# Stylish-TTS/stylish-tts

Measured on AMD Instinct MI355X. Metric: audio frames/sec/GPU (24 kHz) forward+backward; DDP scaling 1/2/4/8 MI355X, higher is better.
Workload: dtype bf16 GEMM operands, f32 accumulation/storage; 1 GPU; c3: B=32/GPU T=520 frames (6.5 s) L=100

## Files before the change

### include/stylish_hip.h

```cpp
#ifndef STYLISH_HIP_H
#define STYLISH_HIP_H

#include <stddef.h>
#include <stdint.h>

#ifdef __cplusplus
extern "C" {
#endif

typedef enum {
  STY_OK = 0,
  STY_EINVAL = -1,
  STY_ESHAPE = -2,
  STY_EHIP = -3,
  STY_ENOMEM = -4,
  STY_ESTATE = -5
} sty_status;

typedef struct sty_model sty_model;

int sty_version(void);
const char *sty_last_error(void);

int sty_model_create(const char *kind, sty_model **out);
// ... 30 lines not shown
  float *audio;
  float *tap_text_encoding;
  float *tap_decoder_out;
  sty_vocoder_io voc_taps;
  void *style_stream;
} sty_speech_io;
int sty_speech_workspace_bytes(const sty_model *m, int B, int L, int T, size_t *bytes);
int sty_speech_fwd(sty_model *m, const sty_speech_io *io, void *workspace, size_t ws_bytes, void *stream);

int sty_style_workspace_bytes(const sty_model *m, int B, int T, size_t *bytes);
int sty_style_fwd(sty_model *m, int B, int T, const float *mel, float *style, void *workspace, size_t ws_bytes,
                  void *stream);

int sty_mel_workspace_bytes(int B, int N, int n_fft, int hop, size_t *bytes);
int sty_mel_fwd(int B, int N, const float *audio, int n_fft, int win_length, int hop, float mean, float std,
                float *mel, float *energy, void *workspace, size_t ws_bytes, void *stream);

int sty_multispec_workspace_bytes(int B, int N, size_t *bytes);
int sty_multispec_fwd(int B, int N, const float *audio, float *const *mag, float *const *phase,
                      float *const *fft_mag, void *workspace, size_t ws_bytes, void *stream);

int sty_alignment_fwd(int B, int L, int T, const float *durations, float *alignment, void *stream);

int sty_duration_workspace_bytes(const sty_model *m, int B, int L, size_t *bytes);
int sty_duration_fwd(sty_model *m, int B, int L, const int64_t *texts, const int64_t *text_lengths, const float *style,
                     float *dur_pred, void *workspace, size_t ws_bytes, void *stream);
int sty_pitch_energy_workspace_bytes(const sty_model *m, int B, int L, int T, size_t *bytes);
int sty_pitch_energy_fwd(sty_model *m, int B, int L, int T, const int64_t *texts, const int64_t *text_lengths,
                         const float *alignment, const float *style, float *pitch, float *energy, void *workspace,
                         size_t ws_bytes, void *stream);

int sty_pitch_style_workspace_bytes(const sty_model *m, int B, int T, size_t *bytes);
int sty_pitch_style_fwd(sty_model *m, int B, int T, const float *mel, const float *pitch, const float *energy,
                        float *style, void *workspace, size_t ws_bytes, void *stream);

int sty_aligner_workspace_bytes(const sty_model *m, int B, int T, size_t *bytes);
int sty_aligner_fwd(sty_model *m, int B, int T, const float *mel, const int64_t *mel_lengths, float *log_probs,
                    void *workspace, size_t ws_bytes, void *stream);
int sty_forced_align_workspace_bytes(int B, int T, int U, size_t *bytes);
int sty_forced_align(int B, int T, int V1, int U, const float *log_probs, const int64_t *targets,
                     const int64_t *input_lengths, const int64_t *target_lengths, int blank, int32_t *labels,
                     float *scores, int32_t *status, void *workspace, size_t ws_bytes, void *stream);

void sty_rmvpe_resample_kernel_host(float *out);
void sty_rmvpe_mel_basis_host(float *out);
int sty_rmvpe_mel_workspace_bytes(int B, int N, size_t *bytes);
int sty_rmvpe_mel_fwd(int B, int N, const float *audio, float *logmel, void *workspace, size_t ws_bytes, void *stream);
int sty_rmvpe_workspace_bytes(const sty_model *m, int B, int n, size_t *bytes);
int sty_rmvpe_fwd(sty_model *m, int B, int n, const float *logmel, float *salience, void *workspace, size_t ws_bytes,
                  void *stream);
int sty_rmvpe_decode(int B, int n, const float *salience, float thred, float *f0, void *stream);

int sty_aligner_train_workspace_bytes(sty_model *m, int B, int T, size_t *bytes);
int sty_aligner_fwd_train(sty_model *m, int B, int T, const float *mel, const int64_t *mel_lengths, float drop_p,
                          unsigned drop_seed, float *log_probs, void *workspace, size_t ws_bytes, void *stream);
int sty_aligner_bwd(sty_model *m, const float *d_logits, void *stream);
int sty_ctc_loss_workspace_bytes(int B, int T, int V1, int U, size_t *bytes);
int sty_ctc_loss_fwd_bwd(int B, int T, int V1, int U, const float *log_probs, const float *log_priors, float prior_scale,
                         const int64_t *targets, const int64_t *input_lengths, const int64_t *target_lengths, int blank,
                         float weight, double *nll, float *loss, int32_t *status, float *d_logits, void *workspace,
                         size_t ws_bytes, void *stream);

int sty_convnext_fwd(sty_model *m, const char *prefix, int B, int C, int T, const float *x, const float *style,
                     float *y, void *workspace, size_t ws_bytes, void *stream);
int sty_resblock_fwd(sty_model *m, const char *prefix, int B, int T, const float *x, const float *style, float *y,
                     void *workspace, size_t ws_bytes, void *stream);
int sty_block_train_workspace_bytes(sty_model *m, const char *kind, const char *prefix, int B, int C, int T,
                                    size_t *bytes);
int sty_block_fwd_bwd(sty_model *m, const char *kind, const char *prefix, int B, int C, int T, const float *x,
                      const float *style, const float *gy, float *y, float *gx, float *d_style, void *workspace,
                      size_t ws_bytes, void *stream);
int sty_attention_workspace_bytes(int B, int H, int T, size_t *bytes);
int sty_attention_fwd_bwd(int B, int H, int DH, int T, const float *q, const float *k, const float *v,
                          const int64_t *lengths, const float *d_o, float *o, float *dq, float *dk, float *dv,
                          void *workspace, size_t ws_bytes, void *stream);
int sty_stft64_fwd(int B, int N, const float *wave, float *spec, float *phase, void *stream);
void sty_stft64_bases_host(float *out);
int sty_istft64_fwd(int B, int F, const float *logamp, const float *real, const float *imag, float *audio,
                    void *stream);
int sty_source_fwd(int B, int T, const float *pitch, const float *voiced, const float *noise, uint64_t seed,
                   const float *lin_w, const float *lin_b, float *prior, void *workspace, size_t ws_bytes,
                   void *stream);
int sty_source_workspace_bytes(int B, int T, size_t *bytes);
int sty_grn_bwd_workspace_bytes(int B, int C4, int T, size_t *bytes);
int sty_grn_bwd(int B, int C4, int T, const float *h, const float *ds, const float *gamma, int from_gx, float *coef,
                float *dgamma, void *workspace, size_t ws_bytes, void *stream);
int sty_act_bwd(int kind, int B, int C, int T, const float *x, float *dy, const float *alpha, const float *h,
                const float *coef, int fused, float *dx, int accumulate, float *dalpha, void *stream);
int sty_adain_finalize(int B, int C, int T, int nseg, const double *part, const float *gb, float eps, float *a, float *s,
                       float *mean, float *rstd, void *stream);

int sty_model_enable_training(sty_model *m);
typedef struct {
  int bn_batch_stats;
  int sn_power_iter;
  int f0_smooth;
  int energy_smooth;
  float bn_momentum;
  unsigned dropout_seed;
  float text_dropout;
  int compute_bf16;
  int frozen;
  float block_dropout;
} sty_train_opts;
int sty_model_set_train_opts(sty_model *m, const sty_train_opts *opts);

typedef void (*sty_grad_hook)(void *user, int segment);
int sty_model_set_grad_hook(sty_model *m, sty_grad_hook hook, void *user);
int sty_model_bind_grad(sty_model *m, const char *key, float *grad);
int sty_vocoder_train_workspace_bytes(sty_model *m, int B, int T, size_t *bytes);
int sty_vocoder_fwd_train(sty_model *m, const sty_vocoder_io *io, void *workspace, size_t ws_bytes, void *stream);
int sty_vocoder_bwd(sty_model *m, const float *d_audio, float *d_mel, float *d_style, void *stream);
int sty_speech_train_workspace_bytes(sty_model *m, int B, int L, int T, size_t *bytes);
int sty_speech_fwd_train(sty_model *m, const sty_speech_io *io, void *workspace, size_t ws_bytes, void *stream);
int sty_speech_bwd(sty_model *m, const float *d_audio, float *d_style, float *d_energy, void *stream);
int sty_speech_prepare_train(sty_model *m, void *stream);
int sty_speech_bwd_pe(sty_model *m, const float *d_audio, float *d_style, float *d_pitch, float *d_energy, void *stream);
int sty_speech_d_style_ready(sty_model *m, void *stream);
int sty_speech_branch_stream(sty_model *m, void **stream);
int sty_style_train_workspace_bytes(sty_model *m, int B, int T, size_t *bytes);
int sty_style_fwd_train(sty_model *m, int B, int T, const float *mel, float *style, void *workspace, size_t ws_bytes,
                        void *stream);
int sty_style_bwd(sty_model *m, const float *d_style, void *stream);
int sty_style_prepare_train(sty_model *m, void *stream);
int sty_style_tap(sty_model *m, int index, int grad, float *dst, int *C, int *H, int *W, void *stream);
int sty_pitch_loss_fwd_bwd(int B, int T, const float *target, const float *pred, float weight, int normalize,
                           float *loss, float *d_pred, void *workspace, size_t ws_bytes, void *stream);
int sty_prediction_to_duration(int B, int L, int NC, const float *pred, const int64_t *text_lengths,
                               const float *class_table, float *duration, void *stream);
int sty_duration_loss_fwd_bwd(int B, int L, int NC, const float *pred, const int64_t *text_lengths,
                              const float *target_dur, const int64_t *target_class, const float *class_table,
                              const float *ce_weight, float w_duration, float w_ce, const float *d_duration_extra,
                              float *losses, float *d_pred, void *workspace, size_t ws_bytes, void *stream);
int sty_duration_train_workspace_bytes(sty_model *m, int B, int L, size_t *bytes);
int sty_duration_fwd_train(sty_model *m, int B, int L, const int64_t *texts, const int64_t *text_lengths,
                           const float *style, float *out, void *workspace, size_t ws_bytes, void *stream);
int sty_duration_bwd(sty_model *m, const float *d_out, float *d_style, void *stream);
int sty_pitch_energy_train_workspace_bytes(sty_model *m, int B, int L, int T, size_t *bytes);
int sty_pitch_energy_fwd_train(sty_model *m, int B, int L, int T, const int64_t *texts, const int64_t *text_lengths,
                               const float *alignment, const float *style, float *pitch, float *energy, void *workspace,
                               size_t ws_bytes, void *stream);
int sty_pitch_energy_bwd(sty_model *m, const float *d_pitch, const float *d_energy, float *d_style, void *stream);
int sty_pitch_style_train_workspace_bytes(sty_model *m, int B, int T, size_t *bytes);
int sty_pitch_style_fwd_train(sty_model *m, int B, int T, const float *mel, const float *pitch, const float *energy,
                              float *style, void *workspace, size_t ws_bytes, void *stream);

int sty_conv1d_workspace_bytes(int Cout, int Cin, int K, size_t *bytes);
int sty_conv1d_fwd(int B, int Cin, int Cout, int K, int dil, int T, const float *x, const float *w, const float *bias,
                   float *y, void *workspace, size_t ws_bytes, int compute_bf16, void *stream);
int sty_conv1d_fwd_ex(int B, int Cin, int Cout, int K, int dil, int T, const float *x, const float *w, const float *bias,
                      const float *in_mask, const float *residual, const float *out_mask, int out_mask_post, int relu,
                      float *y, void *workspace, size_t ws_bytes, int compute_bf16, void *stream);
enum { STY_ROUTE_IN_MASK = 1, STY_ROUTE_RESIDUAL = 2, STY_ROUTE_OUT_MASK = 4, STY_ROUTE_RELU = 8, STY_ROUTE_TWO_BYTE_X = 16,
       STY_ROUTE_STATS = 32, STY_ROUTE_Y16 = 64, STY_ROUTE_X16 = 128 };
enum { STY_CONV_STEM2D = 0, STY_CONV_32P, STY_CONV_SC, STY_CONV_K1, STY_CONV_Q, STY_CONV_P16, STY_CONV_TILED };
int sty_conv1d_route(int B, int Cin, int Cout, int K, int dil, int T, int compute_bf16, int flags, int *kernel);
int sty_conv1d_bwd_workspace_bytes(int B, int Cin, int Cout, int K, int T, size_t *bytes);
int sty_conv1d_bwd(int B, int Cin, int Cout, int K, int dil, int T, const float *x, const float *w, const float *gy,
                   float *dw, float *dbias, float *dx, void *workspace, size_t ws_bytes, int compute_bf16,
                   void *stream);
int sty_partial_sum(int dw_form, const float *part, int C, int K, int nblk, float *dw, float *db, void *stream);

int sty_adamw_step(size_t n, float *p, const float *g, float *m, float *v, float lr, float beta1, float beta2,
                   float eps, float weight_decay, int step, float grad_scale, void *stream);
int sty_adamw_step_scaled(size_t n, float *p, const float *g, float *m, float *v, double lr, const double *lr_mult,
                          float beta1, float beta2, float eps, float weight_decay, int step, float grad_scale,
                          void *stream);
int sty_disc_lr_track(double *state, const float *loss, double ideal_loss, double f_max, double h_min, double x_max,
                      double x_min, void *stream);

int sty_acoustic_loss_workspace_bytes(int B, int N, size_t *bytes);
int sty_acoustic_loss_target(int B, int N, const float *audio_gt, void *workspace, size_t ws_bytes, void *stream);
int sty_acoustic_loss_fwd_bwd(int B, int N, const float *audio_gt, const float *audio_pred, float w_mel,
                              float w_phase, float *losses, float *d_audio_pred, void *workspace, size_t ws_bytes,
                              void *stream);

typedef struct {
  const float *g[10];
  const float *v[10];
  const float *bias[10];
} sty_specdisc_params;
typedef struct {
  float *g[10];
  float *v[10];
  float *bias[10];
} sty_specdisc_grads;
int sty_specdisc_workspace_bytes(int B, int H, int W, int with_grads, size_t *bytes);
int sty_specdisc_forward(const sty_specdisc_params *p, int B, int H, int W, const float *x, float *scores,
                         int compute_bf16, void *workspace, size_t ws_bytes, void *stream);
int sty_specdisc_losses(const sty_specdisc_params *p, int B, int H, int W, const float *target, const float *pred,
                        float gen_scale, float *gen_loss, float *d_pred, float disc_scale, float *disc_loss,
                        const sty_specdisc_grads *grads, int compute_bf16, void *workspace, size_t ws_bytes,
                        void *stream);

int sty_pitchdisc_workspace_bytes(int B, int dim_in, int kernel, int T, int with_grads, size_t *bytes);
int sty_pitchdisc_forward(const sty_specdisc_params *p, int B, int dim_in, int kernel, int T, const float *x,
                          float *scores, void *workspace, size_t ws_bytes, void *stream);
int sty_pitchdisc_losses(const sty_specdisc_params *p, int B, int dim_in, int kernel, int T, const float *target,
                         const float *pred, float gen_scale, float *gen_loss, float *d_pred, float disc_scale,
                         float *disc_loss, const sty_specdisc_grads *grads, void *workspace, size_t ws_bytes,
                         void *stream);

typedef struct {
  const float *conv_w[12];
  const float *conv_b[12];
  const float *bn_w[9];
  const float *bn_b[9];
  float *bn_rm[9];
  float *bn_rv[9];
} sty_cfdisc_params;
typedef struct {
  float *conv_w[12];
  float *conv_b[12];
  float *bn_w[9];
  float *bn_b[9];
} sty_cfdisc_grads;
int sty_cfdisc_workspace_bytes(int B, int N, int with_grads, size_t *bytes);
int sty_cfdisc_forward(const sty_cfdisc_params *p, int B, int N, const float *x, float *scores, float bn_momentum,
                       int compute_bf16, void *workspace, size_t ws_bytes, void *stream);
int sty_cfdisc_losses(const sty_cfdisc_params *p, int B, int N, const float *target, const float *pred, float gen_scale,
                      float *gen_loss, float *d_pred, float disc_scale, float *disc_loss, const sty_cfdisc_grads *grads,
                      float bn_momentum, int compute_bf16, void *workspace, size_t ws_bytes, void *stream);

int sty_acoustic_gan_workspace_bytes(int B, int N, int with_grads, size_t *bytes);
int sty_acoustic_gan_loss_fwd_bwd(int B, int N, const float *audio_gt, const float *audio_pred, float w_mel,
                                  float w_phase, float w_gen, const sty_specdisc_params *mrd, float disc_scale,
                                  const sty_specdisc_grads *mrd_grads, int step_mask, float *losses, float *gan_losses,
                                  float *d_audio_pred, void *workspace, size_t ws_bytes, void *gan_workspace,
                                  size_t gan_ws_bytes, int compute_bf16, void *stream);

typedef struct sty_comm sty_comm;
int sty_comm_unique_id(void *id128);
int sty_comm_init(const void *id128, int rank, int world, int stream_priority, sty_comm **out);
int sty_comm_allreduce_bucket(sty_comm *c, float *buf, size_t n, void *producer_stream);
int sty_comm_wait(sty_comm *c, void *consumer_stream);
int sty_comm_set_stream(sty_comm *c, void *stream);
int sty_comm_stats(sty_comm *c, uint64_t *buckets, uint64_t *reduce_scatter_all_gather, double *bytes);
int sty_comm_destroy(sty_comm *c);

int sty_pack_accumulate(int n, int D, int rows, const float *styles, const int64_t *text_lengths, double *sums,
                        int64_t *counts, void *stream);
int sty_pack_finalize(int rows, int D, const double *sums, const int64_t *counts, const int32_t *lo, const int32_t *hi,
                      float *pack, void *stream);

typedef struct {
  char name[48];
  char inst[144];
  uint64_t launches;
  double ms;
  double flops;
  double bytes;
} sty_prof_row;
int sty_prof_enable(int on);
int sty_prof_only(const char *family);
int sty_set_single_stream(int on);
int sty_prof_report(sty_prof_row *rows, int cap);

#ifdef __cplusplus
}
#endif
#endif
```

### stylish_tts_amd/csrc/api.hip

```cpp
#include <math.h>
#include <stdarg.h>
#include <string.h>
#include <stdlib.h>
#include <cxxabi.h>

#include <map>
#include <string>

#include "model.h"

namespace sty {

static thread_local char g_err[1024] = "";
void set_error(const char* fmt, ...) {
  va_list ap;
  va_start(ap, fmt);
  vsnprintf(g_err, sizeof(g_err), fmt, ap);
  va_end(ap);
}
int hip_fail(hipError_t e, const char* what) {
  set_error("HIP error %d (%s) at %s", (int)e, hipGetErrorString(e), what);
  return STY_EHIP;
}

// ... 2666 lines not shown
}
int sty_style_tap(sty_model* m, int index, int grad, float* dst, int* C, int* H, int* W, void* stream) {
  int rc = model_ready(m, "mel_style_encoder", "pitch_style_encoder");
  if (rc) return rc;
  if (!m->trainer) {
    set_error("sty_style_tap: no recorded forward");
    return STY_ESTATE;
  }
  return trainer_style_tap(m->trainer, index, grad, dst, C, H, W, S(stream));
}
int sty_conv1d_workspace_bytes(int Cout, int Cin, int K, size_t* bytes) {
  if (!bytes || Cout <= 0 || Cin <= 0 || K <= 0) {
    set_error("sty_conv1d_workspace_bytes: bad argument");
    return STY_EINVAL;
  }
  *bytes = ((size_t)K * align_up(Cin, CI_CHUNK) * align_up(Cout, 128) + align_up(Cout, 128)) * sizeof(float) + 512;
  return STY_OK;
}
int sty_conv1d_fwd(int B, int Cin, int Cout, int K, int dil, int T, const float* x, const float* w, const float* bias,
                   float* y, void* workspace, size_t ws_bytes, int compute_bf16, void* stream) {
  size_t need = 0;
  int rc = sty_conv1d_workspace_bytes(Cout, Cin, K, &need);
  if (rc) return rc;
  if (!x || !w || !y || !workspace || B <= 0 || T <= 0 || dil <= 0 || (K - 1) * dil > 128 || ws_bytes < need) {
    set_error("sty_conv1d_fwd: bad argument, halo > 128 or workspace too small");
    return STY_EINVAL;
  }
  PackedConv pc;
  pc.Cin = Cin;
  pc.Cout = Cout;
  pc.K = K;
  pc.CinP = (int)align_up(Cin, CI_CHUNK);
  pc.CoutP = (int)align_up(Cout, 32);
  float* wp = reinterpret_cast<float*>(align_up(reinterpret_cast<size_t>(workspace), 256));
  float* bp = wp + (size_t)K * pc.CinP * pc.CoutP;
  STY_HIP(hipMemsetAsync(wp, 0, ((size_t)K * pc.CinP * pc.CoutP + pc.CoutP) * sizeof(float), S(stream)));
  rc = launch_pack_conv(w, nullptr, nullptr, bias, Cout, Cin, K, wp, bp, pc.CinP, pc.CoutP, S(stream));
  if (rc) return rc;
  pc.wp = wp;
  pc.bias = bias ? bp : nullptr;
  ConvArgs a;
  a.x[0] = x;
  a.xc[0] = Cin;
  a.nsrc = 1;
  a.B = B;
  a.T = T;
  a.w = pc;
  a.dil = dil;
  a.pad = (K - 1) * dil / 2;
  a.y = y;
  a.bf16 = compute_bf16 != 0;
  if (compute_bf16 == 2) {
    const size_t tw = ((size_t)B * (Cin + Cout) * T) * sizeof(__bf16) + 512;
    if (ws_bytes < need + tw) {
      set_error("sty_conv1d_fwd: compute_bf16 = 2 needs %zu more workspace bytes for the operand twins", tw);
      return STY_EINVAL;
    }
    __bf16* x16 = reinterpret_cast<__bf16*>(align_up(reinterpret_cast<size_t>(static_cast<char*>(workspace) + need), 256));
    if ((rc = launch_twin_cast(x, nullptr, PRO_NONE, B, Cin, T, x16, S(stream)))) return rc;
    a.x16 = x16;
    a.y16 = x16 + (size_t)B * Cin * T;
    a.y16_act = PRO_LRELU;
  }
  return launch_conv1d(a, S(stream));
}
static PackedConv unit_conv_dims(int Cin, int Cout, int K) {
  PackedConv pc;
  pc.Cin = Cin;
  pc.Cout = Cout;
  pc.K = K;
  pc.CinP = (int)align_up(Cin, CI_CHUNK);
  pc.CoutP = (int)align_up(Cout, 32);
  return pc;
}
int sty_conv1d_fwd_ex(int B, int Cin, int Cout, int K, int dil, int T, const float* x, const float* w, const float* bias,
                      const float* in_mask, const float* residual, const float* out_mask, int out_mask_post, int relu, float* y,
                      void* workspace, size_t ws_bytes, int compute_bf16, void* stream) {
  size_t need = 0;
  int rc = sty_conv1d_workspace_bytes(Cout, Cin, K, &need);
  if (rc) return rc;
  if (!x || !w || !y || !workspace || B <= 0 || T <= 0 || dil <= 0 || (K - 1) * dil > 128 || ws_bytes < need ||
      !(compute_bf16 == 0 || compute_bf16 == 1)) {
    set_error("sty_conv1d_fwd_ex: bad argument, halo > 128, a compute mode other than 0 / 1 or workspace too small");
    return STY_EINVAL;
  }
  PackedConv pc;
  pc.Cin = Cin;
  pc.Cout = Cout;
  pc.K = K;
  pc.CinP = (int)align_up(Cin, CI_CHUNK);
  pc.CoutP = (int)align_up(Cout, 32);
  float* wp = reinterpret_cast<float*>(align_up(reinterpret_cast<size_t>(workspace), 256));
  float* bp = wp + (size_t)K * pc.CinP * pc.CoutP;
  STY_HIP(hipMemsetAsync(wp, 0, ((size_t)K * pc.CinP * pc.CoutP + pc.CoutP) * sizeof(float), S(stream)));
  rc = launch_pack_conv(w, nullptr, nullptr, bias, Cout, Cin, K, wp, bp, pc.CinP, pc.CoutP, S(stream));
  if (rc) return rc;
  pc.wp = wp;
  pc.bias = bias ? bp : nullptr;
  ConvArgs a;
  a.x[0] = x;
  a.xc[0] = Cin;
  a.nsrc = 1;
  a.B = B;
  a.T = T;
  a.w = pc;
  a.dil = dil;
  a.pad = (K - 1) * dil / 2;
  a.y = y;
  a.bf16 = compute_bf16;
  if (in_mask) {
    a.pro = PRO_MASK;
    a.mask = in_mask;
  }
  a.act = relu ? ACT_RELU : ACT_NONE;
  a.residual = residual;
  a.out_mask = out_mask;
  a.out_mask_post = out_mask ? out_mask_post : 0;
  return launch_conv1d(a, S(stream));
}
int sty_conv1d_route(int B, int Cin, int Cout, int K, int dil, int T, int compute_bf16, int flags, int* kernel) {
  if (!kernel || B <= 0 || Cin <= 0 || Cout <= 0 || K <= 0 || T <= 0 || dil <= 0) {
    set_error("sty_conv1d_route: bad argument");
    return STY_EINVAL;
  }
  static_assert(STY_CONV_STEM2D == CONV_STEM2D && STY_CONV_32P == CONV_32P && STY_CONV_SC == CONV_SC && STY_CONV_K1 == CONV_K1 &&
                    STY_CONV_Q == CONV_Q && STY_CONV_P16 == CONV_P16 && STY_CONV_TILED == CONV_TILED,
                "stylish_hip.h lists the families in the order of ConvKernel");
  static float dummy_f[4];
  static double dummy_d[4];
  static __bf16 dummy_h[4];
  ConvArgs a;
  a.x[0] = dummy_f;
  a.xc[0] = Cin;
  a.nsrc = 1;
  a.B = B;
  a.T = T;
  a.w = unit_conv_dims(Cin, Cout, K);
  a.w.wp = dummy_f;
  a.dil = dil;
  a.pad = (K - 1) * dil / 2;
  a.y = dummy_f;
  a.bf16 = compute_bf16 != 0;
  if (flags & STY_ROUTE_IN_MASK) {
    a.pro = PRO_MASK;
    a.mask = dummy_f;
  }
  if (flags & STY_ROUTE_RESIDUAL) a.residual = dummy_f;
  if (flags & STY_ROUTE_OUT_MASK) a.out_mask = dummy_f;
  if (flags & STY_ROUTE_RELU) a.act = ACT_RELU;
  if (flags & STY_ROUTE_TWO_BYTE_X) a.xh = 1;
  if (flags & STY_ROUTE_STATS) a.stat_part = dummy_d;
  if (flags & STY_ROUTE_Y16) a.y16 = dummy_h;
  if (flags & STY_ROUTE_X16) a.x16 = dummy_h;
  const ConvRoute r = conv1d_route(a);
  *kernel = r.refusal == CONV_OK ? (int)r.kernel : -1;
  return STY_OK;
}
int sty_conv1d_bwd_workspace_bytes(int B, int Cin, int Cout, int K, int T, size_t* bytes) {
  if (!bytes || B <= 0 || Cin <= 0 || Cout <= 0 || K <= 0 || T <= 0) {
    set_error("sty_conv1d_bwd_workspace_bytes: bad argument");
    return STY_EINVAL;
  }
  const PackedConv pc = unit_conv_dims(Cin, Cout, K);
  const size_t plane = (size_t)K * pc.CinP * pc.CoutP + pc.CoutP;
  *bytes = (3 * plane + wgrad_partial_floats(pc, B, T)) * sizeof(float) + 1024;
  *bytes += (size_t)B * (Cin + Cout) * T * sizeof(__bf16) + 512;
  return STY_OK;
}
int sty_conv1d_bwd(int B, int Cin, int Cout, int K, int dil, int T, const float* x, const float* w, const float* gy,
                   float* dw, float* dbias, float* dx, void* workspace, size_t ws_bytes, int compute_bf16,
                   void* stream) {
  size_t need = 0;
  int rc = sty_conv1d_bwd_workspace_bytes(B, Cin, Cout, K, T, &need);
  if (rc) return rc;
  if (!x || !w || !gy || !dw || !workspace || dil <= 0 || (K - 1) * dil > 128 || ws_bytes < need) {
    set_error("sty_conv1d_bwd: bad argument, halo > 128 or workspace too small");
    return STY_EINVAL;
  }
  hipStream_t st = S(stream);
  PackedConv pc = unit_conv_dims(Cin, Cout, K);
  const size_t plane = (size_t)K * pc.CinP * pc.CoutP;
  float* wp = reinterpret_cast<float*>(align_up(reinterpret_cast<size_t>(workspace), 256));
  float* bp = wp + plane;
  float* gwp = bp + pc.CoutP;
  float* gbp = gwp + plane;
  PackedConv pd;
  pd.Cin = Cout;
  pd.Cout = Cin;
  pd.K = K;
  pd.CinP = pc.CoutP;
  pd.CoutP = pc.CinP;
  float* wd = gbp + pc.CoutP;
  float* partial = wd + plane + pc.CoutP;
  STY_HIP(hipMemsetAsync(wp, 0, (size_t)(partial - wp) * sizeof(float), st));
  rc = launch_pack_conv(w, nullptr, nullptr, nullptr, Cout, Cin, K, wp, bp, pc.CinP, pc.CoutP, st);
  if (rc) return rc;
  pc.wp = wp;
  pc.bias = dbias ? bp : nullptr;
  ConvArgs a;
  a.x[0] = x;
  a.xc[0] = Cin;
  a.nsrc = 1;
  a.B = B;
  a.T = T;
  a.w = pc;
  a.dil = dil;
  a.pad = (K - 1) * dil / 2;
  a.bf16 = compute_bf16 != 0;
  if (compute_bf16 == 3) {
    if (dx || T % 2) {
      set_error("sty_conv1d_bwd: a two-byte x (compute_bf16 = 3) is for dw / dbias only (dx == NULL), T even");
      return STY_EINVAL;
    }
    a.xh = 1;
  }
  if (compute_bf16 == 2) {
    __bf16* x16 = reinterpret_cast<__bf16*>(align_up(reinterpret_cast<size_t>(partial + wgrad_partial_floats(pc, B, T)), 256));
    __bf16* g16 = x16 + (size_t)B * Cin * T;
    if ((rc = launch_twin_cast(x, nullptr, PRO_NONE, B, Cin, T, x16, st))) return rc;
    if ((rc = launch_twin_cast(gy, nullptr, PRO_NONE, B, Cout, T, g16, st))) return rc;
    a.x16 = x16;
    a.g16 = g16;
  }
  bool bias_done = false;
  rc = launch_conv1d_wgrad(a, gy, nullptr, 1.0f, gwp, partial, dbias ? gbp : nullptr, &bias_done, st);
  if (rc) return rc;
  if (dbias && !bias_done) {
    set_error("sty_conv1d_bwd: this conv's bias gradient is a separate pass (launch_bias_grad), not wired here");
    return STY_EINVAL;
  }
  STY_HIP(hipMemsetAsync(dw, 0, (size_t)Cout * Cin * K * sizeof(float), st));
  rc = launch_unpack_grad(gwp, nullptr, nullptr, Cout, Cin, K, pc.CinP, pc.CoutP, dw, nullptr, nullptr, st);
  if (rc) return rc;
  if (dbias) STY_HIP(hipMemcpyAsync(dbias, gbp, (size_t)Cout * sizeof(float), hipMemcpyDeviceToDevice, st));
  if (dx) {
    PackedConv pdm = pd;
    rc = launch_pack_dgrad(wp, K, pc.CinP, pc.CoutP, wd, st);
    if (rc) return rc;
    pdm.wp = wd;
    pdm.bias = nullptr;
    ConvArgs d;
    d.x[0] = gy;
    d.xc[0] = Cout;
    d.nsrc = 1;
    d.B = B;
    d.T = T;
    d.w = pdm;
    d.dil = dil;
    d.pad = (K - 1) * dil - a.pad;
    d.bf16 = a.bf16;
    d.y = dx;
    d.x16 = a.g16;
    rc = launch_conv1d(d, st);
  }
  return rc;
}
int sty_partial_sum(int dw_form, const float* part, int C, int K, int nblk, float* dw, float* db, void* stream) {
  if (!part || !db || C <= 0 || nblk <= 0 || (dw_form && (!dw || K <= 0))) {
    set_error("sty_partial_sum: bad argument");
    return STY_EINVAL;
  }
  return launch_partial_sum(dw_form, part, C, K, nblk, dw, db, S(stream));
}
static size_t grn_bwd_ws_bytes(int B, int C4, int T) {
  return (size_t)B * C4 * row_stats_nseg(T) * 2 * sizeof(double) + (size_t)2 * B * C4 * sizeof(float);
}
int sty_grn_bwd_workspace_bytes(int B, int C4, int T, size_t* bytes) {
  if (!bytes || B <= 0 || C4 <= 0 || T <= 0) {
    set_error("sty_grn_bwd_workspace_bytes: bad argument");
    return STY_EINVAL;
  }
  *bytes = grn_bwd_ws_bytes(B, C4, T);
  return STY_OK;
}
int sty_grn_bwd(int B, int C4, int T, const float* h, const float* ds, const float* gamma, int from_gx, float* coef,
                float* dgamma, void* workspace, size_t ws_bytes, void* stream) {
  if (!h || !ds || !gamma || !coef || !dgamma || !workspace || B <= 0 || C4 <= 0 || T <= 0) {
    set_error("sty_grn_bwd: bad argument");
    return STY_EINVAL;
  }
  if (ws_bytes < grn_bwd_ws_bytes(B, C4, T)) {
    set_error("sty_grn_bwd: workspace too small");
    return STY_ENOMEM;
  }
  hipStream_t st = S(stream);
  const int nseg = row_stats_nseg(T);
  double* part = (double*)workspace;
  float* scale = (float*)(part + (size_t)B * C4 * nseg * 2);
  float* gx = scale + (size_t)B * C4;
  int rc = launch_row_stats(h, B * C4, T, part, st);
  if (rc) return rc;
  if ((rc = launch_grn_finalize(part, nseg, gamma, B, C4, scale, st, gx))) return rc;
  return launch_grn_bwd(from_gx ? gx : nullptr, part, nseg, gamma, ds, B, C4, coef, dgamma, st);
}
int sty_act_bwd(int kind, int B, int C, int T, const float* x, float* dy, const float* alpha, const float* h,
                const float* coef, int fused, float* dx, int accumulate, float* dalpha, void* stream) {
  if (!x || !dy || !dx || B <= 0 || C <= 0 || T <= 0 || (kind == ACT_SNAKE && !alpha) || ((h != nullptr) != (coef != nullptr))) {
    set_error("sty_act_bwd: bad argument");
    return STY_EINVAL;
  }
  hipStream_t st = S(stream);
  if (h && !fused) {
    const int rc = launch_row_scale_add(h, coef, 0.f, B * C, T, dy, st);
    if (rc) return rc;
    h = coef = nullptr;
  }
  return launch_act_bwd(kind, x, dy, alpha, B, C, T, dx, accumulate, dalpha, st, h, coef);
}
int sty_adain_finalize(int B, int C, int T, int nseg, const double* part, const float* gb, float eps, float* a, float* s,
// ... 145 lines not shown
```

### stylish_tts_amd/csrc/bwd.hip

```cpp
#include "sty_common.h"

namespace sty {

__device__ __forceinline__ double wave_sum(double v) {
  for (int o = 32; o > 0; o >>= 1) v += __shfl_xor(v, o);
  return v;
}

template <int N>
__device__ __forceinline__ void block_sum(double (&v)[N], double (*red)[4]) {
  const int lane = threadIdx.x & 63, wave = threadIdx.x >> 6;
#pragma unroll
  for (int i = 0; i < N; ++i) {
    v[i] = wave_sum(v[i]);
    if (lane == 0) red[i][wave] = v[i];
  }
  __syncthreads();
  if (threadIdx.x == 0) {
#pragma unroll
    for (int i = 0; i < N; ++i) v[i] = red[i][0] + red[i][1] + red[i][2] + red[i][3];
  }
}

__global__ __launch_bounds__(256) void pro_bwd_kernel(int mode_, const float* __restrict__ u, int Cu, int cu0,
// ... 592 lines not shown
  STY_LAUNCH_CHECK();
  return STY_OK;
}
bool chan_ln32_eligible(int B, int C, int T, int relu) {
  return C == 32 && !relu && (size_t)B * T >= 65536 && getenv("STY_NO_LN32_BWD") == nullptr;
}
int launch_chan_ln_bwd(const float* x, const float* dy, const float* y, int B, int C, int T, float eps, int ada,
                       const float* w, const float* gb, int relu, const float* out_mask, float* dx, int accumulate,
                       float* mu_tmp, float* r_tmp, float* dgb, float* dw, float* db, hipStream_t st, int h16) {
  const bool no32 = getenv("STY_NO_LN32_BWD") != nullptr;
  if (C == 32 && !relu && (size_t)B * T >= 65536 && !no32) {
    const int nblk = cdiv(T, 256);
    if ((h16 & 4) && accumulate) {
      set_error("chan_ln_bwd: a two-byte dx cannot be accumulated into");
      return STY_EINVAL;
    }
    hipLaunchKernelGGL(chan_ln32_bwd_kernel, dim3(nblk, B), dim3(256), 0, st, x, dy, T, eps, ada, w, gb, out_mask, dx, accumulate,
                       mu_tmp, h16);
    hipLaunchKernelGGL(chan_ln32_param_sum_kernel, dim3(ada ? B * 64 : 64), dim3(64), 0, st, mu_tmp, B, nblk, ada, dgb, dw, db);
    STY_LAUNCH_CHECK();
    return STY_OK;
  }
  if (h16) {
    set_error("chan_ln_bwd: two-byte tensors only on the C = 32 long-row kernel (chan_ln32_eligible)");
    return STY_EINVAL;
  }
  if ((size_t)B * T < 65536 && C <= 256)
    hipLaunchKernelGGL((chan_ln_bwd_dx_reg_kernel<16, 16>), dim3(cdiv(T, 16), B), dim3(256), 0, st, x, dy, y, C, T, eps, ada, w,
                       gb, relu, out_mask, dx, accumulate, mu_tmp, r_tmp);
  else if ((size_t)B * T >= 65536)
    hipLaunchKernelGGL(chan_ln_bwd_dx_kernel<64>, dim3(cdiv(T, 64), B), dim3(256), 0, st, x, dy, y, C, T, eps, ada, w, gb,
                       relu, out_mask, dx, accumulate, mu_tmp, r_tmp);
  else
    hipLaunchKernelGGL(chan_ln_bwd_dx_kernel<16>, dim3(cdiv(T, 16), B), dim3(256), 0, st, x, dy, y, C, T, eps, ada, w, gb,
                       relu, out_mask, dx, accumulate, mu_tmp, r_tmp);
  hipLaunchKernelGGL(chan_ln_bwd_param_kernel, dim3(C, B), dim3(256), 0, st, x, dy, y, mu_tmp, r_tmp, C, T, ada, relu,
                     out_mask, dgb, dw, db);
  STY_LAUNCH_CHECK();
  return STY_OK;
}

__global__ __launch_bounds__(256) void grn_bwd_kernel(const float* __restrict__ gx, const double* __restrict__ part, int nseg,
                                                      const float* __restrict__ gamma,
                                                      const float* __restrict__ ds, int C4,
                                                      float* __restrict__ coef, float* __restrict__ dgamma) {
  __shared__ float gxs[1024];
  __shared__ double red[2][4];
  const int b = blockIdx.x;
  if (gx) {
    for (int c = threadIdx.x; c < C4; c += 256) gxs[c] = gx[(size_t)b * C4 + c];
  } else if (nseg < 32) {
    for (int c = threadIdx.x; c < C4; c += 256) {
      double sq = 0.0;
      for (int k = 0; k < nseg; ++k) sq += part[(((size_t)b * C4 + c) * nseg + k) * 2 + 1];
      gxs[c] = (float)sqrt(sq);
    }
  } else {
    const int lane = threadIdx.x & 63, wave = threadIdx.x >> 6;
    for (int c = wave; c < C4; c += 4) {
      const double* pp = part + ((size_t)b * C4 + c) * nseg * 2 + 1;
      double sq = 0.0;
      for (int k = lane; k < nseg; k += 64) sq += pp[(size_t)k * 2];
      for (int o = 32; o > 0; o >>= 1) sq += __shfl_xor(sq, o);
      if (lane == 0) gxs[c] = (float)sqrt(sq);
    }
  }
  __syncthreads();
  double acc[1] = {0.0};
  for (int c = threadIdx.x; c < C4; c += 256) acc[0] += gxs[c];
  __shared__ float mean_s, dot_s;
  block_sum<1>(acc, red);
  if (threadIdx.x == 0) mean_s = (float)(acc[0] / C4);
  __syncthreads();
  const float m = mean_s + 1e-6f;
  double d2[1] = {0.0};
  for (int c = threadIdx.x; c < C4; c += 256) {
    const float dnx = ds[(size_t)b * C4 + c] * gamma[c];
    d2[0] += (double)dnx * gxs[c];
    atomicAdd(&dgamma[c], ds[(size_t)b * C4 + c] * (gxs[c] / m));
  }
  __syncthreads();
  block_sum<1>(d2, red);
  if (threadIdx.x == 0) dot_s = (float)d2[0];
  __syncthreads();
  for (int c = threadIdx.x; c < C4; c += 256) {
    const float dnx = ds[(size_t)b * C4 + c] * gamma[c];
    const float dgx = dnx / m - dot_s / (m * m) / (float)C4;
    coef[(size_t)b * C4 + c] = gxs[c] > 0.f ? dgx / gxs[c] : 0.f;
  }
}
int launch_grn_bwd(const float* gx, const double* part, int nseg, const float* gamma, const float* ds, int B, int C4,
                   float* coef, float* dgamma, hipStream_t st) {
  if (C4 > 1024) {
    set_error("grn_bwd: 4C > 1024");
    return STY_EINVAL;
  }
  if (!gx && !part) {
    set_error("grn_bwd: neither the forward's norms nor its partials");
    return STY_EINVAL;
  }
  ProfScope prof("grn_bwd_kernel", 0.0, 4.0 * B * C4 * 4, st, gx ? "gx" : "part");
  hipLaunchKernelGGL(grn_bwd_kernel, dim3(B), dim3(256), 0, st, gx, part, nseg, gamma, ds, C4, coef, dgamma);
  STY_LAUNCH_CHECK();
  return STY_OK;
}

__global__ void act_fwd_kernel(int kind, const float* __restrict__ x, const float* __restrict__ alpha, int C, int T,
                               float* __restrict__ y) {
  const int t = blockIdx.x * 256 + threadIdx.x, c = blockIdx.y, b = blockIdx.z;
  if (t >= T) return;
  if (kind == ACT_GLU) {
    const float a = x[((size_t)b * 2 * C + c) * T + t], g = x[((size_t)b * 2 * C + C + c) * T + t];
    y[((size_t)b * C + c) * T + t] = a / (1.f + expf(-g));
    return;
  }
  const size_t o = ((size_t)b * C + c) * T + t;
  const float v = x[o];
  float r = v;
  if (kind == ACT_RELU) r = fmaxf(v, 0.f);
  else if (kind == ACT_SWISH) r = v / (1.f + expf(-v));
  else if (kind == ACT_SNAKE) r = sty_snake(v, alpha[c], 1.f / alpha[c]);
  else if (kind == 100) r = tanhf(v);
  else if (kind == ACT_GELU) r = 0.5f * v * (1.0f + erff(v * 0.70710678118654752f));
  y[o] = r;
}
__device__ __forceinline__ float act_apply1(int kind, float v, float al, float ral) {
  float r = v;
  if (kind == ACT_RELU) r = fmaxf(v, 0.f);
  else if (kind == ACT_SWISH) r = v / (1.f + expf(-v));
  else if (kind == ACT_SNAKE) r = sty_snake(v, al, ral);
  else if (kind == 100) r = tanhf(v);
  else if (kind == ACT_GELU) r = 0.5f * v * (1.0f + erff(v * 0.70710678118654752f));
  return r;
}
__global__ __launch_bounds__(256) void act_fwd4_kernel(int kind, const float* __restrict__ x, const float* __restrict__ alpha,
                                                       unsigned C, unsigned T4, unsigned n4, float* __restrict__ y) {
  const unsigned idx = blockIdx.x * 256u + threadIdx.x;
  if (idx >= n4) return;
  float al = 1.f, ral = 1.f;
  if (kind == ACT_SNAKE) {
    al = alpha[(idx / T4) % C];
    ral = 1.f / al;
  }
  const float4 v = reinterpret_cast<const float4*>(x)[idx];
  float4 r;
  r.x = act_apply1(kind, v.x, al, ral);
  r.y = act_apply1(kind, v.y, al, ral);
  r.z = act_apply1(kind, v.z, al, ral);
  r.w = act_apply1(kind, v.w, al, ral);
  reinterpret_cast<float4*>(y)[idx] = r;
}
int launch_act_fwd(int kind, const float* x, const float* alpha, int B, int C, int T, float* y, hipStream_t st) {
  const size_t n4 = (size_t)B * C * (T / 4);
  if (kind != ACT_GLU && T % 4 == 0 && n4 < ((size_t)1 << 31) && ((((size_t)x | (size_t)y) & 15) == 0)) {
    hipLaunchKernelGGL(act_fwd4_kernel, dim3((unsigned)((n4 + 255) / 256)), dim3(256), 0, st, kind, x, alpha, (unsigned)C,
                       (unsigned)(T / 4), (unsigned)n4, y);
    STY_LAUNCH_CHECK();
    return STY_OK;
  }
  hipLaunchKernelGGL(act_fwd_kernel, dim3(cdiv(T, 256), C, B), dim3(256), 0, st, kind, x, alpha, C, T, y);
  STY_LAUNCH_CHECK();
  return STY_OK;
}
__global__ __launch_bounds__(256) void act_bwd_kernel(int kind, const float* __restrict__ x,
                                                      const float* __restrict__ dy, const float* __restrict__ alpha,
                                                      int C, int T, float* __restrict__ dx, int accumulate,
                                                      float* __restrict__ dalpha, const float* __restrict__ h,
                                                      const float* __restrict__ coef) {
  __shared__ double red[1][4];
  const int c = blockIdx.x, b = blockIdx.y;
  double acc[1] = {0.0};
  if (kind == ACT_GLU) {
    const size_t ra = ((size_t)b * 2 * C + c) * T, rg = ((size_t)b * 2 * C + C + c) * T, ro = ((size_t)b * C + c) * T;
    for (int t = threadIdx.x; t < T; t += 256) {
      const float a = x[ra + t], g = x[rg + t], d = dy[ro + t];
      const float sg = 1.f / (1.f + expf(-g));
      const float da = d * sg, dg = d * a * sg * (1.f - sg);
      dx[ra + t] = accumulate ? dx[ra + t] + da : da;
      dx[rg + t] = accumulate ? dx[rg + t] + dg : dg;
    }
    return;
  }
  const size_t row = ((size_t)b * C + c) * T;
  const float al = kind == ACT_SNAKE ? alpha[c] : 1.f;
  const float cf = h ? coef[(size_t)b * C + c] : 0.f;
  auto one = [&](float v, float d) -> float {
    float g = d;
    if (kind == ACT_RELU) g = v > 0.f ? d : 0.f;
    else if (kind == ACT_SWISH) {
      const float sg = 1.f / (1.f + expf(-v));
      g = d * (sg + v * sg * (1.f - sg));
    } else if (kind == ACT_SNAKE) {
      float sn, cs;
      sty_sincos(al * v, sn, cs);
      const float s2 = sn * sn, s2a = 2.f * sn * cs;
      g = d * (1.f + s2a);
      acc[0] += (double)(d * (v * s2a - s2 / al) / al);
    } else if (kind == 100) {
      const float th = tanhf(v);
      g = d * (1.f - th * th);
    } else if (kind == ACT_GELU) {
      g = d * (0.5f * (1.0f + erff(v * 0.70710678118654752f)) + v * 0.3989422804014327f * expf(-0.5f * v * v));
    }
    return g;
  };
  if ((T & 3) == 0 && ((((size_t)(x + row) | (size_t)(dy + row) | (size_t)(dx + row) | (size_t)(h ? h + row : nullptr)) & 15) == 0)) {
    const float4* x4 = reinterpret_cast<const float4*>(x + row);
    const float4* d4 = reinterpret_cast<const float4*>(dy + row);
    float4* o4 = reinterpret_cast<float4*>(dx + row);
    const float4* h4 = h ? reinterpret_cast<const float4*>(h + row) : nullptr;
    for (int t = threadIdx.x; t < T / 4; t += 256) {
      const float4 v = x4[t];
      float4 d = d4[t];
      if (h) {
        const float4 hv = h4[t];
        d = make_float4(fmaf(hv.x, cf, d.x), fmaf(hv.y, cf, d.y), fmaf(hv.z, cf, d.z), fmaf(hv.w, cf, d.w));
      }
      float4 g;
      g.x = one(v.x, d.x);
      g.y = one(v.y, d.y);
      g.z = one(v.z, d.z);
      g.w = one(v.w, d.w);
      if (accumulate) {
        const float4 o = o4[t];
        g = make_float4(o.x + g.x, o.y + g.y, o.z + g.z, o.w + g.w);
      }
      o4[t] = g;
    }
  } else
  for (int t = threadIdx.x; t < T; t += 256) {
    const float v = x[row + t];
    float d = dy[row + t];
    if (h) d = fmaf(h[row + t], cf, d);
    float g = d;
    if (kind == ACT_RELU) g = v > 0.f ? d : 0.f;
    else if (kind == ACT_SWISH) {
      const float sg = 1.f / (1.f + expf(-v));
      g = d * (sg + v * sg * (1.f - sg));
    } else if (kind == ACT_SNAKE) {
      float sn, cs;
      sty_sincos(al * v, sn, cs);
      const float s2 = sn * sn, s2a = 2.f * sn * cs;
      g = d * (1.f + s2a);
      acc[0] += (double)(d * (v * s2a - s2 / al) / al);
    } else if (kind == 100) {
      const float th = tanhf(v);
      g = d * (1.f - th * th);
    } else if (kind == ACT_GELU) {
      g = d * (0.5f * (1.0f + erff(v * 0.70710678118654752f)) + v * 0.3989422804014327f * expf(-0.5f * v * v));
    }
    dx[row + t] = accumulate ? dx[row + t] + g : g;
  }
  if (kind == ACT_SNAKE && dalpha) {
    block_sum<1>(acc, red);
    if (threadIdx.x == 0) atomicAdd(&dalpha[c], (float)acc[0]);
  }
}
int launch_act_bwd(int kind, const float* x, const float* dy, const float* alpha, int B, int C, int T, float* dx,
                   int accumulate, float* dalpha, hipStream_t st, const float* h, const float* coef) {
  if (h && (kind == ACT_GLU || !coef)) {
    set_error("act_bwd: a row term needs its coefficients and a one-to-one activation");
    return STY_EINVAL;
  }
  ProfScope prof("act_bwd_kernel", 0.0, 4.0 * B * C * T * (3.0 + (accumulate ? 1 : 0) + (h ? 1 : 0)), st, h ? "row term" : nullptr);
  hipLaunchKernelGGL(act_bwd_kernel, dim3(C, B), dim3(256), 0, st, kind, x, dy, alpha, C, T, dx, accumulate, dalpha, h, coef);
  STY_LAUNCH_CHECK();
  return STY_OK;
}

__global__ void row_scale_add_kernel(const float* __restrict__ src, const float* __restrict__ coef, float k, int T,
                                     float* __restrict__ dst) {
  const int t = blockIdx.x * 256 + threadIdx.x, row = blockIdx.y;
  if (t >= T) return;
  const size_t o = (size_t)row * T + t;
  dst[o] += src[o] * (coef ? coef[row] : k);
}
__global__ __launch_bounds__(256) void row_scale_add4_kernel(const float* __restrict__ src, const float* __restrict__ coef,
                                                             float k, unsigned T4, unsigned n4, float* __restrict__ dst) {
  const unsigned idx = blockIdx.x * 256u + threadIdx.x;
  if (idx >= n4) return;
  const float f = coef ? coef[idx / T4] : k;
  const float4 sv = reinterpret_cast<const float4*>(src)[idx];
  float4 d = reinterpret_cast<float4*>(dst)[idx];
  d.x += sv.x * f;
  d.y += sv.y * f;
  d.z += sv.z * f;
  d.w += sv.w * f;
  reinterpret_cast<float4*>(dst)[idx] = d;
}
int launch_row_scale_add(const float* src, const float* coef, float k, int rows, int T, float* dst, hipStream_t st) {
  ProfScope prof(coef ? "row_scale_add_kernel[coef]" : "row_scale_add_kernel", 0.0, 12.0 * rows * T, st);
  const size_t n4 = (size_t)rows * (T / 4);
  if (vec4_ok(n4, T, src, dst)) {
    hipLaunchKernelGGL(row_scale_add4_kernel, dim3((unsigned)((n4 + 255) / 256)), dim3(256), 0, st, src, coef, k,
                       (unsigned)(T / 4), (unsigned)n4, dst);
    STY_LAUNCH_CHECK();
    return STY_OK;
  }
  hipLaunchKernelGGL(row_scale_add_kernel, dim3(cdiv(T, 256), rows), dim3(256), 0, st, src, coef, k, T, dst);
  STY_LAUNCH_CHECK();
  return STY_OK;
}

__global__ void dwconv_fwd_kernel(const float* __restrict__ x, const float* __restrict__ w,
                                  const float* __restrict__ bias, int C, int T, int K, int pad,
                                  float* __restrict__ y) {
// ... 640 lines not shown
```

### stylish_tts_amd/csrc/conv1d.hip

```cpp
#include <stdlib.h>

#include "sty_common.h"

namespace sty {

__device__ __forceinline__ float sigmoidf_(float v) { return 1.0f / (1.0f + expf(-v)); }

}

#include "conv_stage.h"

namespace sty {

template <int ACT>
__device__ __forceinline__ float act_apply(float x, float alpha) {
  if constexpr (ACT == ACT_RELU) return fmaxf(x, 0.f);
  if constexpr (ACT == ACT_SWISH) return x * sigmoidf_(x);
  if constexpr (ACT == ACT_SNAKE) return sty_snake(x, alpha, 1.0f / alpha);
  if constexpr (ACT == ACT_GELU) return 0.5f * x * (1.0f + erff(x * 0.70710678118654752f));
  return x;
}

constexpr int STY_MINW = 2;
template <int WM, int WN, int MT, int NT, int KS = 1, bool BF = false>
// ... 213 lines not shown
    }
    return;
  }
#define STY_EPI_ACT(ACT)                                                                 \
  _Pragma("clang loop unroll(full)") for (int m = 0; m < MT; ++m)                        \
  _Pragma("clang loop unroll(full)") for (int n = 0; n < NT; ++n)                        \
  _Pragma("unroll") for (int r = 0; r < 16; ++r) {                                       \
    const int co = co0 + m * 32 + (r & 3) + 8 * (r >> 2) + 4 * hi;                       \
    float x = acc[m][n][r] + (a.w.bias ? a.w.bias[co] : 0.f);                            \
    float al = 1.f;                                                                      \
    if constexpr (ACT == ACT_SNAKE) al = a.act_alpha[co < Cout ? co : 0];                \
    acc[m][n][r] = act_apply<ACT>(x, al) * a.out_scale;                                  \
  }
  switch (a.act) {
    case ACT_RELU: { STY_EPI_ACT(ACT_RELU) } break;
    case ACT_SWISH: { STY_EPI_ACT(ACT_SWISH) } break;
    case ACT_SNAKE: { STY_EPI_ACT(ACT_SNAKE) } break;
    case ACT_GELU: { STY_EPI_ACT(ACT_GELU) } break;
    default: { STY_EPI_ACT(ACT_NONE) } break;
  }
#undef STY_EPI_ACT
#pragma clang loop unroll(full)
  for (int m = 0; m < MT; ++m) {
#pragma clang loop unroll(full)
    for (int n = 0; n < NT; ++n) {
      const int t = t0 + tw + n * 32 + l31;
      const bool tin = t < T;
      float v[16];
      const float om_pre = (a.out_mask && !a.out_mask_post && tin) ? a.out_mask[(size_t)b * T + t] : 1.f;
#pragma unroll
      for (int r = 0; r < 16; ++r) {
        const int co = co0 + m * 32 + (r & 3) + 8 * (r >> 2) + 4 * hi;
        float x = acc[m][n][r] * om_pre;
        if (a.residual && co < Cout && tin) x += a.residual[((size_t)b * Cout + co) * T + t];
        v[r] = x;
      }
      if (a.ln_out) {
        float s = 0.f;
#pragma unroll
        for (int r = 0; r < 16; ++r) s += v[r];
        s += __shfl_xor(s, 32);
        const float mean = s * (1.0f / 32.0f);
        float q = 0.f;
#pragma unroll
        for (int r = 0; r < 16; ++r) {
          float d = v[r] - mean;
          q += d * d;
        }
        q += __shfl_xor(q, 32);
        const float rstd = 1.0f / sqrtf(q * (1.0f / 32.0f) + a.ln_eps);
#pragma unroll
        for (int r = 0; r < 16; ++r) {
          const int co = co0 + m * 32 + (r & 3) + 8 * (r >> 2) + 4 * hi;
          v[r] = (v[r] - mean) * rstd * a.ln_w[co] + a.ln_b[co];
        }
      }
      if (tin) {
        const float om = (a.out_mask && a.out_mask_post) ? a.out_mask[(size_t)b * T + t] : 1.f;
        if (a.shuffle == 1) {
#pragma unroll
          for (int r = 0; r < 16; ++r) {
            const int co = co0 + m * 32 + (r & 3) + 8 * (r >> 2) + 4 * hi;
            if (co < Cout) a.y[((size_t)b * Cout + co) * T + t] = v[r] * om;
          }
        } else {
          const int s = a.shuffle;
#pragma unroll
          for (int r = 0; r < 16; ++r) {
            const int co = co0 + m * 32 + (r & 3) + 8 * (r >> 2) + 4 * hi;
            if (co < Cout)
              a.y[((size_t)b * (Cout / s) + co / s) * ((size_t)T * s) + (size_t)t * s + co % s] = v[r] * om;
          }
        }
      }
    }
  }
}

template <int WM, int WN, int MT, int NT, int KS = 1, bool BF = false>
static int launch_cfg(const ConvArgs& a, hipStream_t st) {
  if constexpr (!BF) {
    if (a.bf16) return launch_cfg<WM, WN, MT, NT, KS, true>(a, st);
  }
  constexpr int CO_BLK = 32 * MT * WM;
  constexpr int TT_BLK = 32 * NT * WN;
  const int halo = (a.w.K - 1) * a.dil;
  size_t lds = (size_t)KS * CI_CHUNK * (TT_BLK + halo) * sizeof(float);
  if (KS > 1 && lds < (size_t)MT * NT * 16 * 64 * WM * WN * sizeof(float)) lds = (size_t)MT * NT * 16 * 64 * WM * WN * sizeof(float);
  if (halo > 128) {
    set_error("conv1d: receptive-field halo %d > 128 not built", halo);
    return STY_EINVAL;
  }
  if (lds > 64 * 1024) {
    static bool raised = false;
    if (!raised) {
      STY_HIP(hipFuncSetAttribute(reinterpret_cast<const void*>(&conv1d_mfma_kernel<WM, WN, MT, NT, KS, BF>),
                                  hipFuncAttributeMaxDynamicSharedMemorySize, 80 * 1024));
      raised = true;
    }
    if (lds > 80 * 1024) {
      set_error("conv1d: LDS tile %zu B exceeds 80 KiB (K=%d dil=%d)", lds, a.w.K, a.dil);
      return STY_EINVAL;
    }
  }
  if (a.w.CoutP % CO_BLK != 0) {
    set_error("conv1d: CoutP %d not a multiple of block tile %d", a.w.CoutP, CO_BLK);
    return STY_EINVAL;
  }
  dim3 grid(cdiv(a.T, TT_BLK), a.w.CoutP / CO_BLK, a.B);
  const double outs = (double)a.B * a.w.Cout * a.T;
  const double flops = 2.0 * a.w.Cin * a.w.K * outs;
  const double in_elems = (double)a.B * (a.flatW ? a.Cin2d : a.w.Cin) * a.T;
  const double bytes = 4.0 * (in_elems + outs * (a.residual ? 2.0 : 1.0) + (double)a.w.Cout * a.w.Cin * a.w.K);
  char fam[48];
  snprintf(fam, sizeof(fam), BF ? "conv1d_mfma_kernel<%d,%d,%d,%d,%d,true>" : "conv1d_mfma_kernel<%d,%d,%d,%d,%d,false>", WM,
           WN, MT, NT, KS);
  char detail[40];
  snprintf(detail, sizeof(detail), "ci%d co%d k%d T%d W%d", a.w.Cin, a.w.Cout, a.w.K, a.T, a.flatW);
  ProfScope prof(fam, flops, bytes, st, detail);
  hipLaunchKernelGGL((conv1d_mfma_kernel<WM, WN, MT, NT, KS, BF>), grid, dim3(64 * WM * WN * KS), lds, st, a);
  STY_LAUNCH_CHECK();
  return STY_OK;
}

static int launch_tiled(const ConvArgs& a, hipStream_t st) {
  const long tiles128 = (long)cdiv(a.T, 128) * (a.w.CoutP / 128) * a.B;
  const long t128_min = a.bf16 ? 256 : 512;
  const long t64_min = a.bf16 ? 256 : 512;
  constexpr long t32_min = 512;
  if (a.act == ACT_GLU) {
    if (a.w.CoutP % 128 == 0 && tiles128 >= t128_min) return launch_cfg<2, 2, 2, 2>(a, st);
    return launch_cfg<1, 4, 2, 1>(a, st);
  }
  if (a.w.CoutP % 128 == 0 && tiles128 >= t128_min) return launch_cfg<2, 2, 2, 2>(a, st);
  if (a.w.CoutP % 64 == 0) {
    const long tiles64 = (long)cdiv(a.T, 256) * (a.w.CoutP / 64) * a.B;
    if (tiles64 >= t64_min) return launch_cfg<1, 4, 2, 2>(a, st);
    const long wgs = (long)cdiv(a.T, 64) * (a.w.CoutP / 64) * a.B;
    constexpr int ks4_wgs = 64;
    if (wgs <= ks4_wgs && a.ksplit_max >= 4 && a.w.CinP >= 8 * CI_CHUNK && a.pro != PRO_LN_AFFINE)
      return launch_cfg<2, 2, 1, 1, 4>(a, st);
    constexpr int ks2_wgs = 256;
    if (wgs <= ks2_wgs && a.w.CinP >= 4 * CI_CHUNK && a.pro != PRO_LN_AFFINE) return launch_cfg<2, 2, 1, 1, 2>(a, st);
    return launch_cfg<2, 2, 1, 1>(a, st);
  }
  if ((long)cdiv(a.T, 512) * (a.w.CoutP / 32) * a.B >= t32_min) return launch_cfg<1, 8, 1, 2>(a, st);
  return launch_cfg<1, 4, 1, 2>(a, st);
}

bool stem2d_eligible(const ConvArgs& a);
bool conv32p_eligible(const ConvArgs& a);
bool convsc_eligible(const ConvArgs& a);
bool convk1_eligible(const ConvArgs& a);
bool convp16_eligible(const ConvArgs& a);
bool convq_eligible(const ConvArgs& a);
int launch_stem2d(const ConvArgs& a, hipStream_t st);
int launch_conv32p(const ConvArgs& a, hipStream_t st);
int launch_convsc(const ConvArgs& a, hipStream_t st);
int launch_convk1(const ConvArgs& a, hipStream_t st);
int launch_convq(const ConvArgs& a, hipStream_t st);
int launch_convp16(const ConvArgs& a, hipStream_t st);

ConvRoute conv1d_route(const ConvArgs& a) {
  ConvRoute r;
  if (stem2d_eligible(a))
    r.kernel = CONV_STEM2D;
  else if (conv32p_eligible(a))
    r.kernel = CONV_32P;
  else if (a.xh || a.yh || a.rh)
    r.refusal = CONV_NO_TWO_BYTE;
  else if (a.stat_part)
    r.refusal = CONV_NO_STATS;
  else if (convsc_eligible(a))
    r.kernel = CONV_SC;
  else if (convk1_eligible(a))
    r.kernel = CONV_K1;
  else if (convp16_eligible(a))
    r.kernel = a.x16 && convq_eligible(a) ? CONV_Q : CONV_P16;
  r.x16_only = (r.kernel == CONV_Q || r.kernel == CONV_P16) && a.x16 && a.act != ACT_LRELU01;
  r.up_stage = r.kernel == CONV_Q && a.flatW && a.act == ACT_NONE && !a.out_mask && !a.residual &&
               !(a.up_g && (!a.up_gate16 || !a.up_mask || a.up_H <= 0 || a.up_H * a.flatW != a.T)) &&
               (long)a.w.Cout * a.T < (1l << 26);
  if (a.up_g && !r.up_stage) r.refusal = CONV_NO_UP_STAGE;
  return r;
}

int launch_conv1d(const ConvArgs& a, hipStream_t st) {
  const ConvRoute r = conv1d_route(a);
  if (r.refusal == CONV_NO_UP_STAGE) {
    set_error("conv1d: up-sample + gate output stage asked of a conv that does not run on convq_kernel");
    return STY_EINVAL;
  }
  int cin = 0;
  for (int i = 0; i < a.nsrc; ++i) cin += a.xc[i];
  if (a.flatW) cin = a.w.Cin;
  if (cin != a.w.Cin) {
    set_error("conv1d: input channels %d != weight Cin %d", cin, a.w.Cin);
    return STY_ESHAPE;
  }
  if (a.pro == PRO_LN_AFFINE && a.w.CinP != CI_CHUNK) {
    set_error("conv1d: LN prologue needs Cin <= %d", CI_CHUNK);
    return STY_EINVAL;
  }
  if (a.ln_out && a.w.Cout != 32) {
    set_error("conv1d: LN epilogue needs Cout == 32");
    return STY_EINVAL;
  }
  if (r.refusal == CONV_NO_TWO_BYTE) {
    set_error("conv1d: bf16-stored operand (xh %d yh %d rh %d) on a conv the persistent 32-channel kernel does not take", a.xh,
              a.yh, a.rh);
    return STY_EINVAL;
  }
  if (r.refusal == CONV_NO_STATS) {
    set_error("conv1d: output statistics requested for a conv the persistent 32-channel kernel does not take");
    return STY_EINVAL;
  }
  int rc = STY_OK;
  switch (r.kernel) {
    case CONV_STEM2D: rc = launch_stem2d(a, st); break;
    case CONV_32P: rc = launch_conv32p(a, st); break;
    case CONV_SC: rc = launch_convsc(a, st); break;
    case CONV_K1: rc = launch_convk1(a, st); break;
    case CONV_Q: rc = launch_convq(a, st); break;
    case CONV_P16: rc = launch_convp16(a, st); break;
    case CONV_TILED: rc = launch_tiled(a, st); break;
  }
  if (rc == STY_OK && a.y16 && !r.writes_y16()) {
    if (a.shuffle > 1) {
      set_error("conv1d: no output twin for a pixel-shuffled store");
      return STY_EINVAL;
    }
    rc = launch_twin_cast(a.y, nullptr, a.y16_act, a.B, a.w.Cout, a.T, a.y16, st);
  }
  return rc;
}

}
```

### stylish_tts_amd/csrc/convk1.hip

```cpp
#include <stdlib.h>

#include "sty_common.h"
#include "conv_stage.h"

namespace sty {

constexpr int G_KC = 64;
constexpr int G_PITCH = 160;

typedef short g_s4 __attribute__((ext_vector_type(4)));

__device__ __forceinline__ unsigned g_pk(float a, float b) {
  typedef __bf16 b2 __attribute__((ext_vector_type(2)));
  b2 r;
  r[0] = (__bf16)a;
  r[1] = (__bf16)b;
  return __builtin_bit_cast(unsigned, r);
}

template <int PRO, int RELU>
__global__ __launch_bounds__(256, 2) void convk1_kernel(ConvArgs a, int tiles_per_row, int ncot, int ntiles, int per_xcd) {
  extern __shared__ __attribute__((aligned(16))) __bf16 g_lds[];
  const int tid = threadIdx.x, lane = tid & 63, wave = __builtin_amdgcn_readfirstlane(tid >> 6), l31 = lane & 31, hi = lane >> 5;
  const int wm = wave >> 1, wn = wave & 1;
  const int tile = ((int)blockIdx.x & 7) * per_xcd + ((int)blockIdx.x >> 3);
  if (tile >= ntiles) return;
  const int cot = tile % ncot, n0 = (tile / ncot) * 128;
  const int T = a.T, Cin = a.w.Cin, Cout = a.w.Cout;
  const int NT = a.B * T;
  const int nch = a.w.CinP / G_KC;
  const int NMB = a.w.CoutP / 32;

  const int cg = tid & 31, r0 = tid >> 5;
  const __amdgpu_buffer_rsrc_t rx =
      __builtin_amdgcn_make_buffer_rsrc(const_cast<float*>(a.x[0]), 0, (unsigned)((size_t)a.B * Cin * T * 4), 0x00020000);
  const int ns = n0 + 4 * cg;
  const int b = ns < NT ? ns / T : 0, ts = ns - b * T;
  const __amdgpu_buffer_rsrc_t rw = __builtin_amdgcn_make_buffer_rsrc(
      const_cast<void*>(a.w.wf), 0, a.w.CinP * a.w.CoutP * 2, 0x00020000);
  const int xoff = ns < NT ? ((b * Cin + r0) * T + ts) * 4 : 0x7FFFFF00;
  float mk[4] = {1.f, 1.f, 1.f, 1.f};
  if constexpr (PRO == PRO_MASK) {
#pragma unroll
    for (int e = 0; e < 4; ++e) mk[e] = ns < NT ? a.mask[(size_t)ns + e] : 0.f;
  }
  float4 xv[8];
  float pa[8];
  bf16x8 av[2][2][2];
  auto issue = [&](int c) {
#pragma unroll
    for (int i = 0; i < 8; ++i) {
      xv[i] = c * G_KC + r0 + 8 * i < Cin
                  ? __builtin_bit_cast(float4, __builtin_amdgcn_raw_buffer_load_b128(rx, xoff + (c * G_KC + 8 * i) * T * 4, 0, 0))
                  : make_float4(0.f, 0.f, 0.f, 0.f);
      if constexpr (PRO == PRO_SCALE) {
        const int ci = c * G_KC + r0 + 8 * i;
        pa[i] = ci < Cin ? a.pa[(size_t)b * Cin + ci] : 0.f;
      }
    }
#pragma unroll
    for (int h = 0; h < 2; ++h)
#pragma unroll
      for (int s_ = 0; s_ < 2; ++s_)
#pragma unroll
        for (int m = 0; m < 2; ++m) {
          const int f = ((2 * c + h) * 2 + s_) * NMB + cot * 4 + wm * 2 + m;
          av[h][s_][m] = __builtin_bit_cast(bf16x8, __builtin_bit_cast(float4, __builtin_amdgcn_raw_buffer_load_b128(
                                                        rw, cot * 4 + wm * 2 + m < NMB ? lane * 16 : 0x7FFFFF00, f * 1024, 0)));
        }
  };
  auto commit = [&](int buf) {
    __bf16* dst = g_lds + buf * G_KC * G_PITCH + r0 * G_PITCH + 4 * cg;
#pragma unroll
    for (int i = 0; i < 8; ++i) {
      float v[4] = {xv[i].x, xv[i].y, xv[i].z, xv[i].w};
#pragma unroll
      for (int e = 0; e < 4; ++e) {
        if constexpr (PRO == PRO_MASK) v[e] *= mk[e];
        if constexpr (PRO == PRO_SCALE) v[e] *= pa[i];
      }
      uint2 pk;
      pk.x = g_pk(v[0], v[1]);
      pk.y = g_pk(v[2], v[3]);
      *reinterpret_cast<uint2*>(dst + 8 * i * G_PITCH) = pk;
    }
  };

  f32x16 acc[2][2];
#pragma unroll
  for (int m = 0; m < 2; ++m)
#pragma unroll
    for (int n = 0; n < 2; ++n)
#pragma unroll
      for (int r = 0; r < 16; ++r) acc[m][n][r] = 0.f;

  const int i16 = lane & 15, nh = (lane >> 4) & 1;
  const int trow = 8 * hi + (i16 >> 2), tcol = wn * 64 + 16 * nh + 4 * (i16 & 3);

  issue(0);
  for (int c = 0; c < nch; ++c) {
    const int buf = c & 1;
    commit(buf);
    bf16x8 ac[2][2][2];
#pragma unroll
    for (int h = 0; h < 2; ++h)
#pragma unroll
      for (int s_ = 0; s_ < 2; ++s_)
#pragma unroll
        for (int m = 0; m < 2; ++m) ac[h][s_][m] = av[h][s_][m];
    __syncthreads();
    if (c + 1 < nch) issue(c + 1);
    const __bf16* xb = g_lds + buf * G_KC * G_PITCH;
#pragma unroll
    for (int ks = 0; ks < 4; ++ks) {
      bf16x8 bfrag[2];
#pragma unroll
      for (int n = 0; n < 2; ++n) {
        const __bf16* p = xb + (ks * 16 + trow) * G_PITCH + tcol + n * 32;
        const g_s4 lo = __builtin_amdgcn_ds_read_tr16_b64_v4i16((__attribute__((address_space(3))) g_s4*)(p));
        const g_s4 hi4 = __builtin_amdgcn_ds_read_tr16_b64_v4i16((__attribute__((address_space(3))) g_s4*)(p + 4 * G_PITCH));
        typedef short s8 __attribute__((ext_vector_type(8)));
        s8 q;
        q[0] = lo[0];
        q[1] = lo[1];
        q[2] = lo[2];
        q[3] = lo[3];
        q[4] = hi4[0];
        q[5] = hi4[1];
        q[6] = hi4[2];
        q[7] = hi4[3];
        bfrag[n] = __builtin_bit_cast(bf16x8, q);
      }
#pragma unroll
      for (int m = 0; m < 2; ++m)
#pragma unroll
        for (int n = 0; n < 2; ++n)
          acc[m][n] = __builtin_amdgcn_mfma_f32_32x32x16_bf16(ac[ks >> 1][ks & 1][m], bfrag[n], acc[m][n], 0, 0, 0);
    }
  }

  __syncthreads();
  float* stg = reinterpret_cast<float*>(g_lds) + wave * 32 * 68;
  const unsigned ybytes = (unsigned)((size_t)a.B * Cout * T * 4);
  const __amdgpu_buffer_rsrc_t ry = __builtin_amdgcn_make_buffer_rsrc(a.y, 0, ybytes, 0x00020000);
  const __amdgpu_buffer_rsrc_t rres = __builtin_amdgcn_make_buffer_rsrc(
      const_cast<float*>(a.residual ? a.residual : a.y), 0, a.residual ? ybytes : 0, 0x00020000);
  const bool post = a.out_mask && a.out_mask_post;
  const int c4 = lane & 15, rq = lane >> 4;
  const int nq = n0 + wn * 64 + 4 * c4;
  const bool qin = nq < NT;
  const int bq = qin ? nq / T : 0, tq = nq - bq * T;
  float om[4] = {1.f, 1.f, 1.f, 1.f};
  if (a.out_mask && qin) {
#pragma unroll
    for (int e = 0; e < 4; ++e) om[e] = a.out_mask[(size_t)nq + e];
  }
#pragma unroll
  for (int m = 0; m < 2; ++m) {
#pragma unroll
    for (int n = 0; n < 2; ++n)
#pragma unroll
      for (int r = 0; r < 16; ++r) stg[((r & 3) + 8 * (r >> 2) + 4 * hi) * 68 + n * 32 + l31] = acc[m][n][r];
    __syncthreads();
    const int cobase = cot * 128 + (wm * 2 + m) * 32;
#pragma unroll
    for (int i = 0; i < 8; ++i) {
      const int row = rq + 4 * i, co = cobase + row;
      if (co < Cout && qin) {
        const int yo = ((bq * Cout + co) * T + tq) * 4;
        const float4 sv = *reinterpret_cast<const float4*>(stg + row * 68 + 4 * c4);
        const float bi = a.w.bias ? a.w.bias[co] : 0.f;
        float v[4] = {sv.x + bi, sv.y + bi, sv.z + bi, sv.w + bi};
        float al = 1.f, ral = 1.f;
        if (RELU == 2) {
          al = a.act_alpha[co];
          ral = 1.0f / al;
        }
        float4 res = make_float4(0.f, 0.f, 0.f, 0.f);
        if (a.residual) res = __builtin_bit_cast(float4, __builtin_amdgcn_raw_buffer_load_b128(rres, yo, 0, 0));
        const float rr[4] = {res.x, res.y, res.z, res.w};
#pragma unroll
        for (int e = 0; e < 4; ++e) {
          if (RELU == 1) v[e] = fmaxf(v[e], 0.f);
          if (RELU == 2) v[e] = sty_snake(v[e], al, ral);
          if (RELU == 3) v[e] = 0.5f * v[e] * (1.0f + erff(v[e] * 0.70710678118654752f));
          v[e] *= a.out_scale;
          if (a.out_mask && !post) v[e] *= om[e];
          v[e] += rr[e];
          if (post) v[e] *= om[e];
        }
        const float4 o4 = make_float4(v[0], v[1], v[2], v[3]);
        __builtin_amdgcn_raw_buffer_store_b128(
            __builtin_bit_cast(__attribute__((__vector_size__(4 * sizeof(unsigned)))) unsigned, o4), ry, yo, 0, 0);
      }
    }
    __syncthreads();
  }
}

int convp16_frags(const ConvArgs& a, hipStream_t st, const void** out);

bool convk1_eligible(const ConvArgs& a) {
  if (!a.bf16 || getenv("STY_NO_CONVK1")) return false;
  if (a.w.K != 1 || a.flatW || a.nsrc != 1 || a.in_shuffle > 1 || a.shuffle != 1 || a.ln_out || a.Tin || a.y_split) return false;
  if (!(a.act == ACT_NONE || a.act == ACT_RELU || (a.act == ACT_SNAKE && a.act_alpha) || a.act == ACT_GELU)) return false;
  if (!(a.pro == PRO_NONE || a.pro == PRO_MASK || a.pro == PRO_SCALE)) return false;
  if (a.T % 4 || a.w.CinP % G_KC || a.w.CinP < 64 || a.w.CoutP < 64) return false;
  if ((size_t)a.B * a.w.CinP * a.T * 4 >= (size_t)1 << 31 || (size_t)a.B * a.w.CoutP * a.T * 4 >= (size_t)1 << 31) return false;
  const char* mt = getenv("STY_CONVK1_MIN_TILES");
  return (long)cdiv(a.B * a.T, 128) * cdiv(a.w.CoutP, 128) >= (mt ? atoi(mt) : 24);
}

template <int PRO>
static void g_launch(const ConvArgs& a, dim3 grid, size_t lds, int tpr, int ncot, int ntiles, int per, hipStream_t st) {
  if (a.act == ACT_RELU)
    hipLaunchKernelGGL((convk1_kernel<PRO, 1>), grid, dim3(256), lds, st, a, tpr, ncot, ntiles, per);
  else if (a.act == ACT_SNAKE)
    hipLaunchKernelGGL((convk1_kernel<PRO, 2>), grid, dim3(256), lds, st, a, tpr, ncot, ntiles, per);
  else if (a.act == ACT_GELU)
    hipLaunchKernelGGL((convk1_kernel<PRO, 3>), grid, dim3(256), lds, st, a, tpr, ncot, ntiles, per);
  else
    hipLaunchKernelGGL((convk1_kernel<PRO, 0>), grid, dim3(256), lds, st, a, tpr, ncot, ntiles, per);
}

int launch_convk1(const ConvArgs& a0, hipStream_t st) {
  ConvArgs a = a0;
  int rc = convp16_frags(a0, st, &a.w.wf);
  if (rc) return rc;
  const int tpr = cdiv(a.B * a.T, 128), ncot = cdiv(a.w.CoutP, 128);
  const int ntiles = tpr * ncot, per = cdiv(ntiles, 8);
  const size_t lds = (size_t)2 * G_KC * G_PITCH * sizeof(__bf16);
  const double outs = (double)a.B * a.w.Cout * a.T;
  char detail[40];
  snprintf(detail, sizeof(detail), "ci%d co%d k1 T%d", a.w.Cin, a.w.Cout, a.T);
  ProfScope prof("convk1_kernel<true>", 2.0 * a.w.Cin * outs,
                 4.0 * ((double)a.B * a.w.Cin * a.T + outs * (a.residual ? 2.0 : 1.0)) + 2.0 * a.w.Cout * a.w.Cin, st, detail);
  const dim3 grid(per * 8);
  switch (a.pro) {
    case PRO_MASK: g_launch<PRO_MASK>(a, grid, lds, tpr, ncot, ntiles, per, st); break;
    case PRO_SCALE: g_launch<PRO_SCALE>(a, grid, lds, tpr, ncot, ntiles, per, st); break;
    default: g_launch<PRO_NONE>(a, grid, lds, tpr, ncot, ntiles, per, st); break;
  }
  STY_LAUNCH_CHECK();
  return STY_OK;
}

}
```

### stylish_tts_amd/csrc/norms.hip

```cpp
#include "sty_common.h"

namespace sty {

__global__ __launch_bounds__(256) void style_fc_kernel(const StyleFcDesc* __restrict__ descs, int style_dim,
                                                       const float* __restrict__ style, float* __restrict__ gb_base,
                                                       int B) {
  __shared__ float s[256];
  const StyleFcDesc d = descs[blockIdx.x];
  const int b = blockIdx.y;
  for (int i = threadIdx.x; i < style_dim; i += 256) s[i] = style[(size_t)b * style_dim + i];
  __syncthreads();
  for (int j = threadIdx.x; j < d.n; j += 256) {
    const float* w = d.W + (size_t)j * style_dim;
    float acc = 0.f;
    for (int k = 0; k < style_dim; ++k) acc = fmaf(s[k], w[k], acc);
    gb_base[d.off * B + (size_t)b * d.n + j] = acc + d.b[j];
  }
}

int launch_style_fc(const StyleFcDesc* descs_dev, int nlayers, int B, int style_dim, const float* style,
                    float* gb_base, hipStream_t st) {
  if (style_dim > 256) {
    set_error("style_fc: style_dim %d > 256", style_dim);
    return STY_EINVAL;
  }
  hipLaunchKernelGGL(style_fc_kernel, dim3(nlayers, B), dim3(256), 0, st, descs_dev, style_dim, style, gb_base, B);
  STY_LAUNCH_CHECK();
  return STY_OK;
}

constexpr int SEG = 4096;
int row_stats_nseg(int T) { return cdiv(T, SEG); }

__global__ __launch_bounds__(256) void row_stats_kernel(const float* __restrict__ x, int T, int nseg,
                                                        double* __restrict__ part) {
  __shared__ double rs[8], rq[8];
  const int seg = blockIdx.x, row = blockIdx.y;
  const float* p = x + (size_t)row * T;
  const int beg = seg * SEG, end = min(beg + SEG, T);
  double s = 0.0, q = 0.0;
  for (int i = beg + threadIdx.x; i < end; i += 256) {
    const double v = (double)p[i];
    s += v;
    q += v * v;
  }
  for (int o = 32; o > 0; o >>= 1) {
    s += __shfl_xor(s, o);
    q += __shfl_xor(q, o);
  }
  const int wave = threadIdx.x >> 6;
  if ((threadIdx.x & 63) == 0) {
    rs[wave] = s;
    rq[wave] = q;
  }
  __syncthreads();
  if (threadIdx.x == 0) {
    double ts = rs[0] + rs[1] + rs[2] + rs[3], tq = rq[0] + rq[1] + rq[2] + rq[3];
    part[((size_t)row * nseg + seg) * 2 + 0] = ts;
    part[((size_t)row * nseg + seg) * 2 + 1] = tq;
  }
}

int launch_row_stats(const float* x, int rows, int T, double* part, hipStream_t st) {
  const int nseg = row_stats_nseg(T);
  hipLaunchKernelGGL(row_stats_kernel, dim3(nseg, rows), dim3(256), 0, st, x, T, nseg, part);
  STY_LAUNCH_CHECK();
  return STY_OK;
}

__global__ __launch_bounds__(256) void adain_finalize_kernel(const double* __restrict__ part, int nseg,
                                                             const float* __restrict__ gb, int B, int C, int T, float eps,
                                                             float* __restrict__ a, float* __restrict__ s,
                                                             float* __restrict__ mean_out, float* __restrict__ rstd_out) {
  const int i = blockIdx.x * 4 + (threadIdx.x >> 6), lane = threadIdx.x & 63;
  if (i >= B * C) return;
  const int b = i / C, c = i % C;
  double sum = 0.0, sq = 0.0;
  for (int k = lane; k < nseg; k += 64) {
    sum += part[((size_t)i * nseg + k) * 2];
    sq += part[((size_t)i * nseg + k) * 2 + 1];
  }
  for (int o = 32; o > 0; o >>= 1) {
    sum += __shfl_xor(sum, o);
    sq += __shfl_xor(sq, o);
  }
  if (lane) return;
  const double mean = sum / T;
  double var = sq / T - mean * mean;
  if (var < 0.0) var = 0.0;
  const float rstd = (float)(1.0 / sqrt(var + (double)eps));
  const float g = 1.f + gb[(size_t)b * 2 * C + c], be = gb[(size_t)b * 2 * C + C + c];
  const float av = g * rstd;
  a[i] = av;
  s[i] = be - av * (float)mean;
  if (mean_out) {
    mean_out[i] = (float)mean;
    rstd_out[i] = rstd;
  }
}

int launch_adain_finalize(const double* part, int nseg, const float* gb, int B, int C, int T, float eps, float* a,
                          float* s, hipStream_t st, float* mean, float* rstd) {
  hipLaunchKernelGGL(adain_finalize_kernel, dim3(cdiv(B * C, 4)), dim3(256), 0, st, part, nseg, gb, B, C, T, eps, a, s, mean,
                     rstd);
  STY_LAUNCH_CHECK();
  return STY_OK;
}

__global__ __launch_bounds__(1024) void grn_finalize_kernel(const double* __restrict__ part, int nseg, int G,
                                                            const float* __restrict__ gamma, int C4,
                                                            float* __restrict__ scale, float* __restrict__ gx_out) {
  __shared__ float red[16];
  __shared__ float gxs[1024];
  const int b = blockIdx.x, wave = threadIdx.x >> 6, lane = threadIdx.x & 63;
  const int cpw = 64 / G, sub = lane / G, gl = lane % G;
  float loc = 0.f;
  for (int c0 = wave * cpw; c0 < C4; c0 += 16 * cpw) {
    const int c = c0 + sub;
    double sq = 0.0;
    if (c < C4) {
      const double* p = part + ((size_t)b * C4 + c) * nseg * 2 + 1;
      for (int k = gl; k < nseg; k += G) sq += p[(size_t)k * 2];
    }
    for (int o = G >> 1; o > 0; o >>= 1) sq += __shfl_xor(sq, o);
    if (gl == 0 && c < C4) {
      const float gx = (float)sqrt(sq);
      gxs[c] = gx;
      if (gx_out) gx_out[(size_t)b * C4 + c] = gx;
      loc += gx;
    }
  }
  for (int o = 32; o > 0; o >>= 1) loc += __shfl_xor(loc, o);
  if (lane == 0) red[wave] = loc;
  __syncthreads();
  float tot = 0.f;
#pragma unroll
  for (int i = 0; i < 16; ++i) tot += red[i];
  const float mean = tot / (float)C4;
  for (int c = threadIdx.x; c < C4; c += 1024) scale[(size_t)b * C4 + c] = 1.f + gamma[c] * (gxs[c] / (mean + 1e-6f));
}

int launch_grn_finalize(const double* part, int nseg, const float* gamma, int B, int C4, float* scale,
                        hipStream_t st, float* gx) {
  if (C4 > 1024) {
    set_error("grn_finalize: 4C = %d > 1024", C4);
    return STY_EINVAL;
  }
  int G = 1;
  while (G < 64 && G < nseg) G <<= 1;
  hipLaunchKernelGGL(grn_finalize_kernel, dim3(B), dim3(1024), 0, st, part, nseg, G, gamma, C4, scale, gx);
  STY_LAUNCH_CHECK();
  return STY_OK;
}

__global__ __launch_bounds__(64) void chan_layernorm_kernel(const float* __restrict__ x, float* __restrict__ y, int C,
                                                            int T, float eps, int ada, const float* __restrict__ w,
                                                            const float* __restrict__ bvec,
                                                            const float* __restrict__ gb, int relu,
                                                            const float* __restrict__ out_mask) {
  const int t = blockIdx.x * 64 + threadIdx.x;
  const int b = blockIdx.y;
  if (t >= T) return;
  const float* p = x + (size_t)b * C * T + t;
  float mean = 0.f;
  for (int c = 0; c < C; ++c) mean += p[(size_t)c * T];
  mean /= (float)C;
  float var = 0.f;
  for (int c = 0; c < C; ++c) {
    const float d = p[(size_t)c * T] - mean;
    var += d * d;
  }
  const float rstd = 1.0f / sqrtf(var / (float)C + eps);
  float* q = y + (size_t)b * C * T + t;
  for (int c = 0; c < C; ++c) {
    const float n = (p[(size_t)c * T] - mean) * rstd;
    float sc, sh;
    if (ada) {
      sc = 1.f + gb[(size_t)b * 2 * C + c];
      sh = gb[(size_t)b * 2 * C + C + c];
    } else {
      sc = w[c];
      sh = bvec[c];
    }
    float o = n * sc + sh;
    if (relu) o = fmaxf(o, 0.f);
    if (out_mask) o *= out_mask[(size_t)b * T + t];
    q[(size_t)c * T] = o;
  }
}

template <int CPT>
__global__ __launch_bounds__(256) void chan_layernorm_reg_kernel(const float* __restrict__ x, float* __restrict__ y,
                                                                 int T, float eps, int ada,
                                                                 const float* __restrict__ w,
                                                                 const float* __restrict__ bvec,
                                                                 const float* __restrict__ gb, int relu,
                                                                 const float* __restrict__ out_mask) {
  constexpr int C = 4 * CPT;
  __shared__ float red[4][64];
  const int lane = threadIdx.x & 63, wave = threadIdx.x >> 6;
  const int t = blockIdx.x * 64 + lane, b = blockIdx.y;
  const bool in = t < T;
  const float* p = x + (size_t)b * C * T + t;
  float v[CPT];
  float s = 0.f;
#pragma unroll
  for (int i = 0; i < CPT; ++i) {
    v[i] = in ? p[(size_t)(wave + 4 * i) * T] : 0.f;
    s += v[i];
  }
  red[wave][lane] = s;
  __syncthreads();
  const float mean = (red[0][lane] + red[1][lane] + red[2][lane] + red[3][lane]) * (1.0f / C);
  __syncthreads();
  float q = 0.f;
#pragma unroll
  for (int i = 0; i < CPT; ++i) {
    const float d = v[i] - mean;
    q += d * d;
  }
  red[wave][lane] = q;
  __syncthreads();
  const float rstd = 1.0f / sqrtf((red[0][lane] + red[1][lane] + red[2][lane] + red[3][lane]) * (1.0f / C) + eps);
  if (!in) return;
  const float om = out_mask ? out_mask[(size_t)b * T + t] : 1.f;
  float* o = y + (size_t)b * C * T + t;
#pragma unroll
  for (int i = 0; i < CPT; ++i) {
    const int c = wave + 4 * i;
    float sc, sh;
    if (ada) {
      sc = 1.f + gb[(size_t)b * 2 * C + c];
      sh = gb[(size_t)b * 2 * C + C + c];
    } else {
      sc = w[c];
      sh = bvec[c];
    }
    float r = (v[i] - mean) * rstd * sc + sh;
    if (relu) r = fmaxf(r, 0.f);
    o[(size_t)c * T] = r * om;
  }
}

int launch_chan_layernorm(const float* x, float* y, int B, int C, int T, float eps, int ada, const float* w,
                          const float* bvec, const float* gb, int relu, const float* out_mask, hipStream_t st) {
  const dim3 grid(cdiv(T, 64), B);
#define STY_LN_CASE(CPT)                                                                                          \
  case 4 * CPT:                                                                                                    \
    hipLaunchKernelGGL(chan_layernorm_reg_kernel<CPT>, grid, dim3(256), 0, st, x, y, T, eps, ada, w, bvec, gb, relu, \
                       out_mask);                                                                                  \
    break;
  switch (C) {
    STY_LN_CASE(8)
    STY_LN_CASE(16)
    STY_LN_CASE(32)
    STY_LN_CASE(64)
    STY_LN_CASE(80)
    STY_LN_CASE(96)
    STY_LN_CASE(128)
    default:
      hipLaunchKernelGGL(chan_layernorm_kernel, grid, dim3(64), 0, st, x, y, C, T, eps, ada, w, bvec, gb, relu,
                         out_mask);
  }
#undef STY_LN_CASE
  STY_LAUNCH_CHECK();
  return STY_OK;
}

template <int KT>
__global__ __launch_bounds__(256) void dwconv_adaln_kernel(const float* __restrict__ x, const float* __restrict__ w,
                                                           const float* __restrict__ bias, int C, int T, int K,
                                                           float eps, const float* __restrict__ gb,
                                                           float* __restrict__ y, int TT) {
  extern __shared__ __attribute__((aligned(16))) float u[];
  float* smean = u + (size_t)C * TT;
  float* srstd = smean + TT;
  float* part = srstd + TT;
  const int b = blockIdx.y, t0 = blockIdx.x * TT;
  const int pad = K / 2;
  const int tid = threadIdx.x;
  const int lane = tid % TT, grp = tid / TT, ngrp = 256 / TT;
  const int t = t0 + lane;
  float psum = 0.f;
  for (int c = grp; c < C; c += ngrp) {
    const float* p = x + ((size_t)b * C + c) * T;
    float acc = bias[c];
    if constexpr (KT > 0) {
      float xv[KT];
#pragma unroll
      for (int k = 0; k < KT; ++k) {
        const int tt = t - KT / 2 + k;
        xv[k] = (tt >= 0 && tt < T) ? p[tt] : 0.f;
      }
#pragma unroll
      for (int k = 0; k < KT; ++k) acc = fmaf(w[c * KT + k], xv[k], acc);
    } else {
      for (int k = 0; k < K; ++k) {
        const int tt = t - pad + k;
        if (tt >= 0 && tt < T) acc = fmaf(w[c * K + k], p[tt], acc);
      }
    }
    u[c * TT + lane] = acc;
    psum += acc;
// ... 90 lines not shown
```

### stylish_tts_amd/csrc/sty_common.h

```cpp
#pragma once
#include <hip/hip_runtime.h>
#include <stdint.h>
#include <stdio.h>

#include "../../include/stylish_hip.h"

namespace sty {

void set_error(const char* fmt, ...);
int hip_fail(hipError_t e, const char* what);

#define STY_HIP(expr)                                      \
  do {                                                     \
    hipError_t _e = (expr);                                \
    if (_e != hipSuccess) return sty::hip_fail(_e, #expr); \
  } while (0)

#define STY_LAUNCH_CHECK() STY_HIP(hipGetLastError())

extern thread_local const void* g_last_kernel;
template <class R, class... A>
inline const void* kernel_handle(R (*f)(A...)) {
  return reinterpret_cast<const void*>(f);
}
#undef hipLaunchKernelGGL
#define hipLaunchKernelGGL(kernelName, numBlocks, numThreads, memPerBlock, streamId, ...)        \
  do {                                                                                             \
    sty::g_last_kernel = sty::kernel_handle(kernelName);                                           \
    (kernelName)<<<(numBlocks), (numThreads), (memPerBlock), (streamId)>>>(__VA_ARGS__);           \
  } while (0)

struct ProfScope {
  int slot = -1;
  hipStream_t st;
  ProfScope(const char* family, double flops, double bytes, hipStream_t s, const char* detail = nullptr);
  ~ProfScope();
};

typedef float f32x16 __attribute__((ext_vector_type(16)));
typedef float f32x4 __attribute__((ext_vector_type(4)));
typedef __bf16 bf16x8 __attribute__((ext_vector_type(8)));

constexpr int WAVE = 64;

#ifdef __HIPCC__
__device__ __forceinline__ bf16x8 sty_pack_bf16(float v0, float v1, float v2, float v3, float v4, float v5, float v6,
                                                float v7) {
  bf16x8 r;
  r[0] = (__bf16)v0;
  r[1] = (__bf16)v1;
  r[2] = (__bf16)v2;
  r[3] = (__bf16)v3;
  r[4] = (__bf16)v4;
  r[5] = (__bf16)v5;
  r[6] = (__bf16)v6;
  r[7] = (__bf16)v7;
  return r;
}
#endif

#ifdef __HIPCC__
typedef __bf16 bf16x2 __attribute__((ext_vector_type(2)));
__device__ __forceinline__ float sty_bf_lo(unsigned u) { return __builtin_bit_cast(float, u << 16); }
__device__ __forceinline__ float sty_bf_hi(unsigned u) { return __builtin_bit_cast(float, u & 0xffff0000u); }
__device__ __forceinline__ unsigned sty_pack2_bf16(float lo, float hi) {
  bf16x2 r;
  r[0] = (__bf16)lo;
  r[1] = (__bf16)hi;
  return __builtin_bit_cast(unsigned, r);
}
__device__ __forceinline__ float sty_round_bf16(float v) {
  return __builtin_bit_cast(float, (unsigned)__builtin_bit_cast(unsigned short, (__bf16)v) << 16);
}
__device__ __forceinline__ float sty_ld_any(const void* p, size_t i, bool h) {
  return h ? sty_bf_lo(reinterpret_cast<const unsigned short*>(p)[i]) : reinterpret_cast<const float*>(p)[i];
}
__device__ __forceinline__ void sty_st_any(void* p, size_t i, float v, bool h) {
  if (h)
    reinterpret_cast<unsigned short*>(p)[i] = __builtin_bit_cast(unsigned short, (__bf16)v);
  else
    reinterpret_cast<float*>(p)[i] = v;
}
__device__ __forceinline__ float4 sty_ld4_any(const void* p, size_t i4, bool h) {
  if (h) {
    const uint2 u = reinterpret_cast<const uint2*>(p)[i4];
    return make_float4(sty_bf_lo(u.x), sty_bf_hi(u.x), sty_bf_lo(u.y), sty_bf_hi(u.y));
  }
  return reinterpret_cast<const float4*>(p)[i4];
}
__device__ __forceinline__ void sty_st4_any(void* p, size_t i4, float4 v, bool h) {
  if (h)
    reinterpret_cast<uint2*>(p)[i4] = make_uint2(sty_pack2_bf16(v.x, v.y), sty_pack2_bf16(v.z, v.w));
  else
    reinterpret_cast<float4*>(p)[i4] = v;
}
#endif

static inline int cdiv(int a, int b) { return (a + b - 1) / b; }
#ifdef __HIPCC__
__device__ __forceinline__ int wg_chunks(int mode, int split, int nsplit, int total, int& first, int& end) {
  if (mode == 1) {
    first = (int)(((long long)split * total) / nsplit);
    end = (int)(((long long)(split + 1) * total) / nsplit);
    return 1;
  }
  end = total;
  if (mode == 2) {
    const int k = split & 7, q = nsplit >> 3, r = nsplit & 7;
    first = k * q + (k < r ? k : r) + (split >> 3);
  } else {
    first = split;
  }
  return nsplit;
}
#endif

static inline size_t align_up(size_t v, size_t a) { return (v + a - 1) / a * a; }

struct PackedConv {
  const float* wp = nullptr;
  const float* bias = nullptr;
  int Cin = 0, Cout = 0, K = 1, CinP = 0, CoutP = 0;
  const void* wf = nullptr;
};

constexpr int CI_CHUNK = 32;

enum ConvPro : int {
  PRO_NONE = 0,
  PRO_AFFINE = 1,
  PRO_AFFINE_SNAKE = 2,
  PRO_AFFINE_LRELU = 3,
  PRO_LN_AFFINE = 4,
  PRO_MASK = 5,
  PRO_SCALE = 6,
  PRO_LRELU = 7,
};
enum ConvAct : int { ACT_NONE = 0, ACT_RELU = 1, ACT_SWISH = 2, ACT_SNAKE = 3, ACT_GLU = 4, ACT_GELU = 5,
                     ACT_LRELU01 = 6 };

struct ConvArgs {
  const float* x[3] = {nullptr, nullptr, nullptr};
  int xc[3] = {0, 0, 0};
  int nsrc = 1;
  int B = 0, T = 0;
  int Tin = 0;
  int dil = 1, pad = 0;
  int hpad = 0, Cin2d = 0;
  int flatW = 0;
  int ksplit_max = 4;
  int bf16 = 0;
  int in_shuffle = 0;
  PackedConv w;
  int pro = PRO_NONE;
  const float* pa = nullptr;
  const float* ps = nullptr;
  const float* palpha = nullptr;
  const float* pbeta = nullptr;
  float ln_eps = 1e-6f;
  const float* mask = nullptr;
  int act = ACT_NONE;
  const float* act_alpha = nullptr;
  float out_scale = 1.f;
  const float* residual = nullptr;
  const float* out_mask = nullptr;
  int out_mask_post = 0;
  int shuffle = 1;
  int ln_out = 0;
  const float* ln_w = nullptr;
  const float* ln_b = nullptr;
  float* y = nullptr;
  float* y_split = nullptr;
  double* stat_part = nullptr;
  const __bf16* x16 = nullptr;
  const __bf16* g16 = nullptr;
  __bf16* y16 = nullptr;
  int y16_act = PRO_NONE;
  const float* up_g = nullptr;
  const __bf16* up_gate16 = nullptr;
  const float* up_mask = nullptr;
  float up_scale = 1.f;
  int up_H = 0;
  int xh = 0, yh = 0, rh = 0, gh = 0;
  int w_row = 0, w_tap = 0;
};
int launch_twin_cast(const float* x, const float* mask, int pro, int B, int C, int T, __bf16* y16, hipStream_t st);
int launch_wgradb16(const ConvArgs& fwd, int nsplit, float* partial, int want_bias, hipStream_t st);

enum ConvKernel : int {
  CONV_STEM2D,
  CONV_32P,
  CONV_SC,
  CONV_K1,
  CONV_Q,
  CONV_P16,
  CONV_TILED,
};
enum ConvRefusal : int { CONV_OK = 0, CONV_NO_UP_STAGE, CONV_NO_TWO_BYTE, CONV_NO_STATS };
struct ConvRoute {
  ConvKernel kernel = CONV_TILED;
  ConvRefusal refusal = CONV_OK;
  bool x16_only = false;
  bool up_stage = false;
  bool writes_y16() const { return kernel == CONV_STEM2D || kernel == CONV_Q || kernel == CONV_P16; }
  bool stats() const { return kernel == CONV_32P; }
  bool two_byte() const { return kernel == CONV_32P; }
};
ConvRoute conv1d_route(const ConvArgs& a);
int launch_conv1d(const ConvArgs& a, hipStream_t st);
int conv32p_stat_nseg(int T);
inline int num_cus() {
  static int n = 0;
  if (!n) {
    int dev = 0;
    if (hipGetDevice(&dev) != hipSuccess || hipDeviceGetAttribute(&n, hipDeviceAttributeMultiprocessorCount, dev) != hipSuccess || n <= 0)
      n = 256;
  }
  return n;
}
enum WgradKernel : int {
  WGRAD_B,
  WGRAD_B16,
  WGRAD_K1,
  WGRAD_64,
  WGRAD_ROWS32,
  WGRAD_STEM,
  WGRAD_P32,
  WGRAD_TILED,
};
struct WgradRoute {
  WgradKernel kernel = WGRAD_TILED;
  int nsplit = 1;
  size_t plane = 0;
  bool fuses_bias = true;
  bool twins_only = false;
  bool refused = false;
};
WgradRoute conv1d_wgrad_route(const ConvArgs& fwd, const float* g, const float* gmask);
bool wgrad_fuses_bias(const ConvArgs& fwd);
int launch_conv1d_wgrad(const ConvArgs& fwd, const float* g, const float* gmask, float scale, float* gwp,
                        float* partial, float* gbias, bool* bias_done, hipStream_t st);
int launch_wgradb(const ConvArgs& ax, const ConvArgs& ag, int nsplit, float* partial, int want_bias, hipStream_t st);
int wgradb_chunks(const PackedConv& w, int B, int T, int dil);
int wgradp32_chunks(const ConvArgs& fwd);
int launch_wgradp32(const ConvArgs& ax, const ConvArgs& ag, int nsplit, float* partial, int want_bias, hipStream_t st);
int wgrad_cnx_nsplit(int B, int T);
int launch_conv_wgrad_cnx(int x_wide, const void* wide, const float* narrow, int B, int T, float* gwp, float* partial,
                          float* gbias, hipStream_t st, int narrow16 = 0);
int wgrad_cnx_per_b(int B, int T);
int launch_wgrad_cnx(int x_wide, const void* wide, const float* narrow, int B, int T, float* partial, int want_bias,
                     hipStream_t st, int per_b = 0, int narrow16 = 0);
int convp16_repack_range(const void* lo, const void* hi, hipStream_t st);
void convp16_forget_range(const void* lo, const void* hi);


struct StyleFcDesc {
  const float* W;
  const float* b;
  size_t off;
  int n;
  int pad;
};
int launch_style_fc(const StyleFcDesc* descs_dev, int nlayers, int B, int style_dim, const float* style,
                    float* gb_base, hipStream_t st);
struct StyleFcBwdDesc {
  const float* W;
  float* dW;
  float* db;
  size_t off;
  int n;
  int pad;
};
int row_stats_nseg(int T);
int launch_row_stats(const float* x, int rows, int T, double* part, hipStream_t st);
int launch_adain_finalize(const double* part, int nseg, const float* gb, int B, int C, int T, float eps, float* a,
                          float* s, hipStream_t st, float* mean = nullptr, float* rstd = nullptr);
int launch_grn_finalize(const double* part, int nseg, const float* gamma, int B, int C4, float* scale, hipStream_t st,
                        float* gx = nullptr);
int launch_chan_layernorm(const float* x, float* y, int B, int C, int T, float eps, int ada, const float* w,
                          const float* bvec, const float* gb, int relu, const float* out_mask, hipStream_t st);
int launch_embedding(const int64_t* tokens, const float* emb, int B, int L, int H, int ntok, float scale, float* y,
                     hipStream_t st);
int launch_length_mask(const int64_t* lengths, int B, int L, float* mask, hipStream_t st);
int launch_bmm_ct(const float* enc, const float* ali, int B, int C, int L, int T, float* y, hipStream_t st);
int launch_concat(const float* const* src, const int* ch, int nsrc, int B, int T, float* y, hipStream_t st);
int launch_fnv(const float* pitch, const float* energy, const float* voiced, const float* w34, int B, int T, float* y,
               hipStream_t st);
int launch_prep_fnv(const float* g0, const float* v0, const float* b0, const float* g1, const float* v1,
                    const float* b1, const float* g2, const float* v2, const float* b2, float* w34, hipStream_t st);
int launch_alignment(const float* dur, int B, int L, int T, float* ali, hipStream_t st);
int launch_axpy(const float* x, float a, float* y, size_t n, hipStream_t st);
int launch_dwconv_adaln(const float* x, const float* w, const float* bias, int B, int C, int T, int K, float eps,
                        const float* gb, float* y, hipStream_t st);
int launch_dwconv_bn_swish(const float* x, const float* w, const float* bias, const float* bn_w, const float* bn_b,
                           const float* bn_rm, const float* bn_rv, float bn_eps, int B, int C, int T, int K,
                           float* y, hipStream_t st);
}

namespace sty {
struct Cnx32Args {
  const float* x;
  const float* dw_w;
  const float* dw_b;
  const float* gb;
  const float* w1p;
  const float* b1;
  const float* alpha;
  const float* w2a;
  const float* b2eff;
  const float* scale;
  double* part;
  float* y;
  int T, ntiles;
  int bf16 = 0;
  void* h16 = nullptr;
};

struct Cnx32BwdArgs {
  const float* x;
  const float* gy;
  const float *dw_w, *dw_b;
  const float* gb;
  const float* w1p;
  const float* w1;
  const float* w2;
  const float *b1, *alpha;
  const float* scale;
  const float* coef;
  double* part;
  double* part_gb;
  float *hs, *gh0;
  float *xn, *gu;
  int T, ntiles;
  int bf16 = 0;
  int out_bf16 = 0;
  int lean = 0;
  const void* wfrag = nullptr;
  float* gx = nullptr;
  int xn16 = 0;
  int gy16 = 0, gx16 = 0, gu16 = 0;
  int x16 = 0;
};
constexpr int CNX_BWD_FUSED_STRIDE = 248;
int convnext32_bwd_ntiles(int T, int fused);
constexpr size_t CNX_FRAG_HALFS = 3 * 4 * 2 * 64 * 8;
int launch_cnx_frag_pack(const float* w1p, const float* w2raw, const float* w1raw, void* wfrag, hipStream_t st);
int launch_cnx_m_finish(float* partial, int B, int SB, const float* w2raw, const float* scale, float* ds, float* gw2,
                        float* gb2, hipStream_t st);
int launch_cnx_dalpha(const float* w1raw, const float* b1, const float* alpha, const float* gw1, const float* gb1,
                      const float* scale, const float* ds, const float* coef, const double* part, int nseg, int B,
                      float* dalpha, hipStream_t st);
int launch_convnext32_bwd(const Cnx32BwdArgs& a, int B, int pass, hipStream_t st);
int launch_cnx_partial_sum(const double* part, int B, int C, int ntiles, int mode, float* out, hipStream_t st);

constexpr int W2A_MAXJ = 16;
struct W2aJobs {
  const float* w2[W2A_MAXJ];
  const float* b2[W2A_MAXJ];
  const float* gb[W2A_MAXJ];
  float* w2a[W2A_MAXJ];
  float* b2eff[W2A_MAXJ];
  int C[W2A_MAXJ];
  int n = 0;
};
int launch_pack_w2a_multi(const W2aJobs& jobs, hipStream_t st);
struct AttnArgs {
  const float* q;
  const float* k;
  const float* v;
  float* o;
  size_t qbs, kbs, vbs, obs;
  int T, H;
  float scale;
  const int64_t* lengths;
  float drop_p = 0.f;
  unsigned drop_seed = 0, drop_site = 0;
  float* lse = nullptr;
  int bf16 = 0;
};
bool attention16_eligible(const AttnArgs& a, int DH);
int launch_attention16(const AttnArgs& a, int B, hipStream_t st);
int launch_attention16_bwd(const AttnArgs& a, const float* dO, float* dQ, float* dK, float* dV, size_t dqbs, size_t dkbs,
                           size_t dvbs, size_t dobs, int B, float* ws, hipStream_t st);
}

#ifdef __HIPCC__
namespace sty {
__device__ __forceinline__ float sty_hash_u(unsigned seed, unsigned site, unsigned idx) {
  unsigned x = idx * 0x9E3779B1u + site * 0x85EBCA77u + seed * 0xC2B2AE3Du;
  x ^= x >> 16;
  x *= 0x7FEB352Du;
  x ^= x >> 15;
  x *= 0x846CA68Bu;
  x ^= x >> 16;
  return (float)(x >> 8) * (1.0f / 16777216.0f);
}
__device__ __forceinline__ void sty_unit_vec(float re, float im, float& c, float& s) {
  const float h2 = re * re + im * im;
  if (h2 > 0.f && h2 < 3.0e38f) {
    const float r = 1.0f / sqrtf(h2);
    c = re * r;
    s = im * r;
  } else {
    const float ph = atan2f(im, re);
    c = cosf(ph);
    s = sinf(ph);
  }
}
static __device__ __attribute__((noinline)) float sty_sinf_slow(float x) { return sinf(x); }
__device__ __forceinline__ float sty_sinf(float x) {
  if (__builtin_expect(fabsf(x) > 8192.0f, 0)) return sty_sinf_slow(x);
  const float kf = rintf(x * 0.636619772f);
  const int k = (int)kf;
  float r = fmaf(-kf, 1.57079637050628662109375f, x);
  r = fmaf(-kf, -4.37113900018624283e-8f, r);
  r = fmaf(-kf, -1.71512449e-15f, r);
  const float r2 = r * r;
  const float ps = fmaf(r2, fmaf(r2, -1.9515295891e-4f, 8.3321608736e-3f), -1.6666654611e-1f);
  const float s = fmaf(r * r2, ps, r);
  const float pc = fmaf(r2, fmaf(r2, 2.443315711809948e-5f, -1.388731625493765e-3f), 4.166664568298827e-2f);
  const float c = fmaf(r2 * r2, pc, fmaf(r2, -0.5f, 1.0f));
  const float res = (k & 1) ? c : s;
  return (k & 2) ? -res : res;
}
__device__ __forceinline__ float sty_sin2_fast(float x) {
  const float kf = rintf(x * 0.636619772f);
  float r = fmaf(-kf, 1.57079637050628662109375f, x);
  r = fmaf(-kf, -4.37113900018624283e-8f, r);
  const float z = r * r;
  float p = fmaf(z, -4.27556050e-6f, 1.41093474e-4f);
  p = fmaf(p, z, -3.17460317e-3f);
// ... 110 lines not shown
```

### stylish_tts_amd/csrc/train.hip

```cpp
#include <stdlib.h>
#include <string.h>

#include <map>
#include <memory>
#include <unordered_map>

#include "model.h"

namespace sty {

struct Trainer {
  sty_model* m = nullptr;
  hipStream_t st = nullptr;
  int B = 0, T = 0;
  Bump ws;
  int rc = STY_OK;
  float* gb = nullptr;
  float* dgb = nullptr;
  const float* style = nullptr;
  float* audio = nullptr;
  std::vector<std::function<void()>> tape;
  std::unordered_map<const float*, float*> gmap;
  std::unordered_set<const float*> nograd;
  float* scratch_param = nullptr;
// ... 303 lines not shown
    gmap[act] = g;
    return true;
  }
  const float* gbp(const AdaFc& a) const { return gb ? gb + a.off * B : nullptr; }
  float* dgbp(const AdaFc& a) const { return dgb ? dgb + a.off * B : nullptr; }

  template <typename Tp>
  Tp* take(size_t n) {
    Tp* p = ws.take<Tp>(n);
    peak = ws.off > peak ? ws.off : peak;
    return p;
  }
  bool keep_temps = false;
  void release(size_t mark) {
    if (!keep_temps) ws.off = mark;
  }
  std::unordered_set<const void*> half_;
  bool act16_env = getenv("STY_NO_ACT16") == nullptr;
  bool act16_on() const { return act16_env && m->topts.compute_bf16 != 0; }
  bool is16(const void* p) const { return p && !half_.empty() && half_.count(p) != 0; }
  float* take_act(size_t n, bool h) {
    if (!h) return take<float>(n);
    float* p = reinterpret_cast<float*>(take<__bf16>((n + 7) & ~size_t(7)));
    half_.insert(p);
    return p;
  }
  std::unordered_set<const float*> g16_ok;
  bool grad16_env = getenv("STY_NO_GRAD16") == nullptr && getenv("STY_NO_CNX_GX") == nullptr;
  bool grad16_on() const { return grad16_env && act16_on(); }
  bool grad16_stream_env = getenv("STY_GRAD16_STREAM") != nullptr && atoi(getenv("STY_GRAD16_STREAM")) != 0;
  bool grad16_stream_on() const { return grad16_stream_env && grad16_on(); }
  float* G16(const float* act, size_t n) {
    auto it = gmap.find(act);
    if (it != gmap.end() && is16(it->second)) return it->second;
    return G(act, n);
  }
  std::map<const float*, std::pair<int, int>> ungated;
  bool gate_pending(const float* act) const { return !ungated.empty() && ungated.count(act) != 0; }
  void gate_flush(const float* act) {
    auto it = ungated.find(act);
    if (it == ungated.end()) return;
    const int C = it->second.first, n = it->second.second;
    ungated.erase(it);
    auto gi = gmap.find(act);
    if (gi == gmap.end() || !live()) return;
    float* g = gi->second;
    chk(launch_pro_bwd(PRO_LRELU, g, C, 0, act, B, C, n, nullptr, nullptr, C, 0, nullptr, nullptr, g, 0, nullptr, nullptr,
                       nullptr, st));
  }
  struct PendRow {
    const float* coef;
    int rows, T;
  };
  std::unordered_map<const float*, PendRow> pend_row;
  void row_flush(const float* act) {
    auto it = pend_row.find(act);
    if (it == pend_row.end()) return;
    const PendRow p = it->second;
    pend_row.erase(it);
    float* g = G(act, (size_t)p.rows * p.T);
    if (live()) chk(launch_row_scale_add(act, p.coef, 0.f, p.rows, p.T, g, st));
  }
  const float* take_row(const float* act) {
    auto it = pend_row.find(act);
    if (it == pend_row.end()) return nullptr;
    const float* coef = it->second.coef;
    pend_row.erase(it);
    return coef;
  }
  float* G(const float* act, size_t n, bool raw = false, bool keep_lazy = false, bool keep_row = false) {
    if (!pend_up.empty()) up_flush(act);
    if (!keep_row && !pend_row.empty()) row_flush(act);
    if (!raw && !ungated.empty()) gate_flush(act);
    if (!keep_lazy && !lazy_mask.empty()) mask_flush(act);
    auto it = gmap.find(act);
    if (it != gmap.end() && is16(it->second)) {
      set_error("a two-byte gradient buffer reached a consumer without a two-byte form");
      rc = STY_ESTATE;
    }
    if (it != gmap.end()) return side_cow(act, it->second, n);
    float* g = take<float>(n);
    if (live()) {
      hipError_t e = hipMemsetAsync(g, 0, n * sizeof(float), st);
      if (e != hipSuccess) rc = hip_fail(e, "grad memset");
    }
    gmap[act] = g;
    return g;
  }
  float* Gw(const float* act, size_t n, int& acc) {
    if (!pend_up.empty()) up_flush(act);
    if (!pend_row.empty()) row_flush(act);
    if (!ungated.empty()) gate_flush(act);
    if (mask_pending(act)) {
      tw_g.erase(lazy_mask[act].dst);
      mask_flush(act);
    }
    auto it = gmap.find(act);
    if (it != gmap.end() && is16(it->second)) {
      set_error("a two-byte gradient buffer reached a second writer");
      rc = STY_ESTATE;
    }
    if (it != gmap.end()) {
      acc = 1;
      return side_cow(act, it->second, n);
    }
    float* g = take<float>(n);
    gmap[act] = g;
    acc = 0;
    return g;
  }
  bool wants(const float* act) const { return !nograd.count(act); }
  float* PGpacked(const float* packed) const {
    if (!packed || !m->garena) return nullptr;
    return reinterpret_cast<float*>(m->garena + (reinterpret_cast<const char*>(packed) - m->arena));
  }
  float* PG(const float* param, size_t n) {
    auto it = m->pgrad.find(param);
    if (it != m->pgrad.end()) return it->second;
    if (n > scratch_param_n) return nullptr;
    return scratch_param;
  }

  ConvArgs base(const PackedConv& w, const float* x, int Tt, float* y) {
    ConvArgs a;
    a.x[0] = x;
    a.xc[0] = w.Cin;
    a.nsrc = 1;
    a.B = B;
    a.T = Tt;
    a.w = w;
    a.pad = (w.K - 1) / 2;
    a.y = y;
    a.bf16 = m->topts.compute_bf16;
    return a;
  }

  void conv(const ConvArgs& a0) {
    ConvArgs a = a0;
    a.bf16 = m->topts.compute_bf16;
    a.xh = is16(a.x[0]);
    a.yh = is16(a.y);
    a.rh = is16(a.residual);
    if (a.nsrc > 1 && (is16(a.x[1]) || is16(a.x[2]))) {
      set_error("training: a bf16-stored tensor as source 1 / 2 of a channel-concatenated conv");
      rc = STY_ESTATE;
      return;
    }
    const size_t pn = wgrad_partial_floats(a.w, B, a.T);
    side_need = pn > side_need ? pn : side_need;
    wg_need(pn);
    bias_pass_sizing(a);
    if (live()) chk(launch_conv1d(a, st));
    ConvArgs f = a;
    tape.push_back([this, f]() { conv_bwd(f); });
  }
  void bias_pass_sizing(const ConvArgs& a) {
    if (!a.w.bias || wgrad_fuses_bias(a)) return;
    const size_t bn = bias_grad_scratch_floats(B, a.w.Cout, a.T);
    side_need = bn > side_need ? bn : side_need;
    wg_need(bn);
  }
  void conv_wgrad(const ConvArgs& f, float* gY, const float* gmask, int shuffle) {
    const PackedConv& w = f.w;
    const int Tt = f.T;
    bool bias_done = false;
    float* gbias = w.bias ? PGpacked(w.bias) : nullptr;
    if (m->topts.frozen) {
      bias_done = true;
    } else if (side_ready()) {
      float* sp = deferring() ? wg_take(wgrad_partial_floats(w, B, Tt)) : side_partial;
      float* gwp = PGpacked(w.wp);
      const float osc = f.out_scale;
      side_push(gY, [=](hipStream_t s) { chk(launch_conv1d_wgrad(f, gY, gmask, osc, gwp, sp, gbias, nullptr, s)); });
      bias_done = wgrad_fuses_bias(f);
      if (w.bias && !bias_done) {
        float* bs = deferring() ? wg_take(bias_grad_scratch_floats(B, w.Cout, Tt)) : side_partial;
        side_push(gY, [=](hipStream_t s) { chk(launch_bias_grad(gY, gmask, B, w.Cout, Tt, shuffle, osc, gbias, bs, s)); });
        bias_done = true;
      }
    } else {
      const size_t pn = wgrad_partial_floats(w, B, Tt);
      float* partial = deferring() ? wg_take(pn) : take<float>(pn);
      DeferScope ds(this);
      if (live()) chk(launch_conv1d_wgrad(f, gY, gmask, f.out_scale, PGpacked(w.wp), partial, gbias, &bias_done, st));
    }
    if (w.bias && !bias_done) {
      float* bs = take<float>(bias_grad_scratch_floats(B, w.Cout, Tt));
      if (live()) chk(launch_bias_grad(gY, gmask, B, w.Cout, Tt, shuffle, f.out_scale, PGpacked(w.bias), bs, st));
    }
  }
  void conv_bwd(const ConvArgs& f) {
    const PackedConv& w = f.w;
    const int Tt = f.T;
    const size_t ny = (size_t)B * w.Cout * Tt;
    float* gY = G(f.y, ny);
    float* gR = nullptr;
    if (f.residual && wants(f.residual)) {
      if (!gmap.count(f.residual) && !(f.out_mask && f.out_mask_post) && f.shuffle <= 1)
        gmap[f.residual] = gY;
      else
        gR = G(f.residual, ny);
    }
    float* gX[3] = {nullptr, nullptr, nullptr};
    int accX[3] = {1, 1, 1};
    bool any = false;
    const float* gX_src = nullptr;
    if (f.nsrc == 1 && f.pro == PRO_AFFINE_SNAKE && Tt % 8 == 0 && wants(f.x[0]) && !side_reads.empty()) {
      auto ia = adain_of.find(f.pa);
      auto ig = gmap.find(f.x[0]);
      if (ia != adain_of.end() && ia->second.x == f.x[0] && ia->second.s == f.ps && !*ia->second.done && ig != gmap.end() &&
          side_reads.count(ig->second) && !is16(ig->second) && (ungated.empty() || !ungated.count(f.x[0]))) {
        gX_src = ig->second;
        gX[0] = take<float>((size_t)B * f.xc[0] * Tt);
        gmap[f.x[0]] = gX[0];
        accX[0] = 1;
        any = true;
      }
    }
    for (int i = 0; i < f.nsrc; ++i)
      if (wants(f.x[i]) && !(i == 0 && gX_src)) {
        gX[i] = Gw(f.x[i], (size_t)B * f.xc[i] * Tt, accX[i]);
        any = true;
      }
    for (int i = 1; i < f.nsrc; ++i)
      for (int j = 0; j < i; ++j)
        if (gX[i] && gX[i] == gX[j]) accX[i] = 1;
    if (side_ready())
      for (int i = 0; i < f.nsrc; ++i)
        if (gX[i] && gX[i] == gY) gX[i] = fresh_copy(f.x[i], gY, (size_t)B * f.xc[i] * Tt);
    float* dpa = nullptr;
    float* dps = nullptr;
    float* dal = nullptr;
    AdainInfo* fuse = nullptr;
    if (any && f.pro == PRO_AFFINE_SNAKE && f.nsrc == 1 && Tt % 8 == 0) {
      auto it = adain_of.find(f.pa);
      if (it != adain_of.end() && it->second.x == f.x[0] && it->second.s == f.ps && !*it->second.done) fuse = &it->second;
    }
    if (any && fuse) {
      dal = PG(f.palpha, w.Cin);
    } else if (any) {
      if (f.pro == PRO_AFFINE_SNAKE || f.pro == PRO_AFFINE_LRELU || f.pro == PRO_AFFINE) {
        int dummy;
        dpa = Gw(f.pa, (size_t)B * w.Cin, dummy);
        dps = Gw(f.ps, (size_t)B * w.Cin, dummy);
      } else if (f.pro == PRO_SCALE) {
        int dummy;
        dpa = Gw(f.pa, (size_t)B * w.Cin, dummy);
      }
      if (f.pro == PRO_AFFINE_SNAKE) dal = PG(f.palpha, w.Cin);
    }
    const size_t mark = ws.off;
    const float* gmask = f.out_mask;
    if (gR && live()) {
      if (f.out_mask && f.out_mask_post)
        chk(launch_pro_bwd(PRO_MASK, gY, w.Cout, 0, gY, B, w.Cout, Tt, nullptr, nullptr, w.Cout, 0, nullptr, f.out_mask,
                           gR, 1, nullptr, nullptr, nullptr, st));
      else
        chk(launch_row_scale_add(gY, nullptr, 1.0f, B * w.Cout, Tt, gR, st));
    }
    conv_wgrad(f, gY, gmask, f.shuffle);
    if (any) {
      auto it = m->dgrad.find(w.wp);
      if (it == m->dgrad.end()) {
        set_error("training: no input-gradient weights for a conv (model not finalized for training?)");
        rc = STY_ESTATE;
        return;
      }
      const bool u16 = f.xh && f.nsrc == 1 && act16_on();
      float* U = take_act((size_t)B * w.Cin * Tt, u16);
      struct UGuard {
        Trainer* t;
        float* U;
        size_t mark;
        ~UGuard() {
          t->half_.erase(U);
          t->release(mark);
        }
      } u_guard{this, U, mark};
      ConvArgs d;
      d.x[0] = gY;
      d.xc[0] = w.Cout;
      d.nsrc = 1;
      d.B = B;
      d.T = Tt;
      d.w = it->second;
      d.dil = f.dil;
      d.bf16 = f.bf16;
      d.pad = (w.K - 1) * f.dil - f.pad;
      d.out_scale = f.out_scale;
      d.in_shuffle = f.shuffle > 1 ? f.shuffle : 0;
      if (gmask) {
        d.pro = PRO_MASK;
        d.mask = gmask;
      }
      d.y = U;
      d.yh = u16;
      d.xh = is16(gY);
      if (f.nsrc == 1 && (f.pro == PRO_NONE || f.pro == PRO_MASK) && gX[0] != gY) {
        d.y = gX[0];
        d.yh = is16(gX[0]);
        d.rh = d.yh;
        d.residual = accX[0] ? gX[0] : nullptr;
        if (f.pro == PRO_MASK) {
          d.out_mask = f.mask;
          d.out_mask_post = 0;
        }
        if (live()) chk(launch_conv1d(d, st));
        release(mark);
        return;
      }
      if (live()) chk(launch_conv1d(d, st));
      if (fuse) {
        *fuse->done = true;
        if (live())
          chk(launch_pro_bwd_adain(U, u16, f.x[0], f.xh, B, w.Cin, Tt, f.pa, f.ps, f.palpha, fuse->mean, fuse->rstd, fuse->gbl,
                                   gX[0], is16(gX[0]), accX[0], fuse->dgl, dal, f.bf16 ? 1 : 0, st, gX_src));
        half_.erase(U);
        release(mark);
        return;
      }
      if (gX_src) {
        set_error("training: out-of-place prologue backward planned without the fused kernel");
        rc = STY_ESTATE;
        return;
      }
      if (u16 || f.xh) {
        half_.erase(U);
        set_error("training: bf16-stored conv input without the fused prologue backward");
        rc = STY_ESTATE;
        return;
      }
      int c0 = 0;
      for (int i = 0; i < f.nsrc; ++i) {
        if (gX[i] && live())
          chk(launch_pro_bwd(f.pro | (f.bf16 ? 0x100 : 0), U, w.Cin, c0, f.x[i], B, f.xc[i], Tt, f.pa, f.ps, w.Cin, c0, f.palpha, f.mask, gX[i],
                             accX[i], dpa, dps, dal, st));
        c0 += f.xc[i];
      }
    }
    release(mark);
  }

  float* act(int kind, const float* x, const float* alpha, int C, int Tt) {
    float* y = take<float>((size_t)B * C * Tt);
    if (live()) chk(launch_act_fwd(kind, x, alpha, B, C, Tt, y, st));
    tape.push_back([=]() {
      const int Cin = kind == ACT_GLU ? 2 * C : C;
      float* gY = G(y, (size_t)B * C * Tt, false, false, kind != ACT_GLU);
      const float* row = take_row(y);
      int acc = 1;
      float* gX = Gw(x, (size_t)B * Cin * Tt, acc);
      float* dal = kind == ACT_SNAKE ? PG(alpha, C) : nullptr;
      if (live()) chk(launch_act_bwd(kind, x, gY, alpha, B, C, Tt, gX, acc, dal, st, row ? y : nullptr, row));
    });
    return y;
  }

  unsigned drop_site = 0;
  const unsigned* drop_seed_arg = nullptr;
  unsigned drop_seed_val = 0;
  bool dropout_on() const { return m->topts.dropout_seed != 0; }
  float* dropout(const float* x, float p, int C, int Tt, const float* residual, size_t group = 1) {
    const size_t n = (size_t)B * C * Tt;
    float* y = take<float>(n);
    const unsigned seed = drop_seed_arg ? *drop_seed_arg : m->topts.dropout_seed, site = drop_site++;
    if (live()) chk(launch_dropout(x, residual, n, p, seed, site, y, 0, st, group));
    tape.push_back([=]() {
      float* gY = G(y, n);
      if (residual && wants(residual)) {
        if (!gmap.count(residual)) {
          gmap[residual] = gY;
        } else {
          float* gR = G(residual, n);
          if (live()) chk(launch_row_scale_add(gY, nullptr, 1.0f, 1, (int)n, gR, st));
        }
      }
      int acc = 1;
      float* gX = Gw(x, n, acc);
      if (gX == gY) {
        set_error("dropout backward: aliased gradient buffers");
        rc = STY_ESTATE;
        return;
      }
      if (live()) chk(launch_dropout(gY, nullptr, n, p, seed, site, gX, acc, st, group));
    });
    return y;
  }

  float* layernorm(const float* x, int C, int Tt, float eps, const AdaFc* fc, const float* w, const float* bvec,
                   int relu = 0, const float* omask = nullptr) {
    float* y = take<float>((size_t)B * C * Tt);
    const float* gbl = fc ? gbp(*fc) : nullptr;
    float* dgl = fc ? dgbp(*fc) : nullptr;
    if (live()) chk(launch_chan_layernorm(x, y, B, C, Tt, eps, fc ? 1 : 0, w, bvec, gbl, relu, omask, st));
    const bool ln32 = grad16_on() && chan_ln32_eligible(B, C, Tt, relu);
    if (ln32 && grad16_stream_on()) g16_ok.insert(y);
    tape.push_back([=]() {
      const size_t nel = (size_t)B * C * Tt;
      float* gY = ln32 ? G16(y, nel) : G(y, nel);
      int acc = 1, h16 = is16(gY) ? 2 : 0;
      float* gX;
      if (ln32 && g16_ok.count(x) && !gmap.count(x)) {
        gX = take_act(nel, true);
        gmap[x] = gX;
        acc = 0;
        h16 |= 4;
      } else {
        gX = Gw(x, nel, acc);
      }
      const size_t mark = ws.off;
      float* mu = take<float>((size_t)B * Tt);
      float* r = take<float>((size_t)B * Tt);
      float* dw = fc ? nullptr : PG(w, C);
      float* db = fc ? nullptr : PG(bvec, C);
      if (live())
        chk(launch_chan_ln_bwd(x, gY, y, B, C, Tt, eps, fc ? 1 : 0, w, gbl, relu, omask, gX, acc, mu, r, dgl, dw, db, st, h16));
      ws.off = mark;
    });
    return y;
  }

  struct AdainInfo {
    const float *x, *s, *mean, *rstd, *gbl;
    float* dgl;
    std::shared_ptr<bool> done;
  };
  std::unordered_map<const float*, AdainInfo> adain_of;
  void adain(const float* x, int C, int Tt, const AdaFc& fc, float*& a, float*& s, const double* have_part = nullptr,
             int have_nseg = 0) {
    a = take<float>((size_t)B * C);
    s = take<float>((size_t)B * C);
    float* mean = take<float>((size_t)B * C);
    float* rstd = take<float>((size_t)B * C);
    const int nseg = have_part ? have_nseg : row_stats_nseg(Tt);
    const double* part = have_part;
    if (!have_part) {
      double* p2 = take<double>((size_t)B * C * nseg * 2);
      if (live()) chk(launch_row_stats(x, B * C, Tt, p2, st));
      part = p2;
    }
    if (live()) chk(launch_adain_finalize(part, nseg, gbp(fc), B, C, Tt, 1e-5f, a, s, st, mean, rstd));
    const float* gbl = gbp(fc);
    float* dgl = dgbp(fc);
    float* aa = a;
    float* ss = s;
    auto done = std::make_shared<bool>(false);
    adain_of[aa] = AdainInfo{x, ss, mean, rstd, gbl, dgl, done};
    if (!have_part && is16(x)) {
      set_error("training: instance-norm statistics pass over a bf16-stored tensor (the producing conv leaves them behind)");
      rc = STY_ESTATE;
    }
    tape.push_back([=]() {
      if (*done) return;
      if (is16(x)) {
        set_error("training: AdaIN backward over a bf16-stored tensor outside the fused prologue backward");
        rc = STY_ESTATE;
        return;
      }
      float* da = G(aa, (size_t)B * C);
      float* ds = G(ss, (size_t)B * C);
      float* gX = G(x, (size_t)B * C * Tt);
      const size_t mark = ws.off;
      float* c0 = take<float>((size_t)B * C);
      float* c1 = take<float>((size_t)B * C);
      if (live()) {
        chk(launch_adain_fold_bwd(da, ds, mean, rstd, gbl, B, C, Tt, dgl, c0, c1, st));
        chk(launch_row_axpb(x, c0, c1, B * C, Tt, gX, st));
      }
      release(mark);
    });
  }

  float* dwconv(const float* x, const float* w, const float* bias, int C, int Tt, int K, int pad) {
    float* y = take<float>((size_t)B * C * Tt);
    if (live()) chk(launch_dwconv_fwd(x, w, bias, B, C, Tt, K, pad, y, st));
    tape.push_back([=]() {
      float* gY = G(y, (size_t)B * C * Tt);
      int acc = 1;
      float* gX = wants(x) ? Gw(x, (size_t)B * C * Tt, acc) : nullptr;
      float* gw = PG(w, (size_t)C * K);
      float* gb = PG(bias, C);
      if (side_ready() && gX != gY) {
        float* sc = take<float>(dwconv_bwd_scratch_floats(B, C, Tt, K));
        side_push(gY, [=](hipStream_t s2) {
          chk(launch_dwconv_bwd(x, gY, w, B, C, Tt, K, pad, nullptr, 0, gw, gb, sc, s2));
        });
        if (live() && gX) chk(launch_dwconv_bwd(x, gY, w, B, C, Tt, K, pad, gX, acc, nullptr, nullptr, nullptr, st));
        return;
      }
      const size_t mark = ws.off;
      float* sc = take<float>(dwconv_bwd_scratch_floats(B, C, Tt, K));
      if (live()) chk(launch_dwconv_bwd(x, gY, w, B, C, Tt, K, pad, gX, acc, gw, gb, sc, st));
      ws.off = mark;
    });
    return y;
  }

  size_t cnx_partial_floats(const PackedConv& w, int Tt) const {
    const size_t a = wgrad_partial_floats(w, B, Tt), b = (size_t)wgrad_cnx_nsplit(B, Tt) * (4096 + 128);
    return a > b ? a : b;
  }
  float* convnext32_fused(const ConvNeXt& c, const float* x, int Tt) {
    const int nt = convnext32_ntiles(Tt);
    const size_t n32 = (size_t)B * 32 * Tt, n128 = (size_t)B * 128 * Tt;
    double* part = take<double>((size_t)B * 128 * nt * 2);
    float* scale = take<float>((size_t)B * 128);
    float* gxn = take<float>((size_t)B * 128);
    float* y = take<float>(n32);
// ... 51 lines not shown
      }
      if (!gmap.count(x)) {
        if (side || fuse_gx) {
          gX = take_act(n32, gx16);
          gmap[x] = gX;
          gx_src = gY;
        } else {
          gmap[x] = gY;
          gX = gY;
        }
      } else {
        gX = G(x, n32);
        if (live()) chk(launch_row_scale_add(gY, nullptr, 1.0f, 1, (int)n32, gX, st));
      }
      const int nt_b = convnext32_bwd_ntiles(Tt, fuse_gx);
      float* hs_p = side && !lean ? take<float>(n128) : nullptr;
      float* gh0_p = side ? take<float>(lean ? n128 / 2 : n128) : nullptr;
      float* ds_p = (side || deferring()) && lean ? take<float>((size_t)B * 128) : nullptr;
      float* coef_p = (side || deferring()) && lean ? take<float>((size_t)B * 128) : nullptr;
      float* xn_p = side ? take<float>(xn16 ? n32 / 2 : n32) : nullptr;
      float* gu_p = side ? take<float>(gu16 ? n32 / 2 : n32) : nullptr;
      float* dsc_p = side ? take<float>(dwconv_bwd_scratch_floats(B, 32, Tt, 7)) : nullptr;
      const size_t mark = ws.off;
      double* pds = take<double>((size_t)B * 128 * nt_b);
      double* pgb = take<double>((size_t)B * 64 * nt_b);
      float* ds = ds_p ? ds_p : take<float>((size_t)B * 128);
      float* coef = coef_p ? coef_p : take<float>((size_t)B * 128);
      float* hs = lean ? nullptr : (side ? hs_p : take<float>(n128));
      float* gh0 = side ? gh0_p : take<float>(lean ? n128 / 2 : n128);
      float* xn = side ? xn_p : take<float>(xn16 ? n32 / 2 : n32);
      float* gu = side ? gu_p : take<float>(gu16 ? n32 / 2 : n32);
      Cnx32BwdArgs a;
      a.x = x;
      a.gy = gY;
      a.dw_w = c.dw_w;
      a.dw_b = c.dw_b;
      a.gb = gbl;
      a.w1p = c.w1p;
      a.w1 = c.w1_raw;
      a.w2 = c.w2_raw;
      a.b1 = c.b1;
      a.alpha = c.alpha;
      a.scale = scale;
      a.coef = coef;
      a.part = pds;
      a.part_gb = pgb;
      a.hs = hs;
      a.gh0 = gh0;
      a.xn = xn;
      a.gu = gu;
      a.T = Tt;
      a.ntiles = nt_b;
      a.gx = fuse_gx ? gX : nullptr;
      a.xn16 = xn16;
      a.gy16 = gy16;
      a.gx16 = gx16;
      a.gu16 = gu16;
      a.bf16 = m->topts.compute_bf16;
      a.wfrag = wfrag;
      const bool cnx16 = a.bf16 && Tt % 8 == 0 && getenv("STY_NO_WGRADB") == nullptr;
      a.out_bf16 = cnx16;
      ConvArgs f2 = base(c.pw2, hs, Tt, nullptr);
      ConvArgs f1 = base(c.pw1, xn, Tt, nullptr);
      const size_t p1n_ = cnx_partial_floats(c.pw1, Tt), p2n_ = cnx_partial_floats(c.pw2, Tt);
      float* p2 = deferring() ? wg_take(p2n_) : side ? side_partial : take<float>(p2n_);
      float* p1 = deferring() ? wg_take(p1n_) : side ? side_partial : take<float>(p1n_);
      float* dsc = side ? dsc_p : take<float>(dwconv_bwd_scratch_floats(B, 32, Tt, 7));
      float* gw2 = PGpacked(c.pw2.wp);
      float* gb2 = PGpacked(c.pw2.bias);
      float* gw1 = PGpacked(c.pw1.wp);
      float* gb1 = PGpacked(c.pw1.bias);
      const bool frozen = m->topts.frozen;
      float* dal = PG(c.alpha, 128);
      if (lean) {
        const int SB = wgrad_cnx_per_b(B, Tt);
        float* pM = take<float>((size_t)B * SB * (4096 + 32));
        a.lean = 1;
        if (live()) {
          chk(launch_wgrad_cnx(1, h16, gY, B, Tt, pM, 1, st, 1, gy16));
          chk(launch_cnx_m_finish(pM, B, SB, c.w2_raw, scale, ds, frozen ? nullptr : gw2, frozen ? nullptr : gb2, st));
          chk(launch_grn_bwd(gxn, nullptr, 0, c.grn_gamma, ds, B, 128, coef, PG(c.grn_gamma, 128), st));
          chk(launch_convnext32_bwd(a, B, 2, st));
          chk(launch_cnx_partial_sum(pgb, B, 64, nt_b, 2, dgl, st));
        }
      } else if (live()) {
        Cnx32BwdArgs a1 = a;
        a1.gx = nullptr;
        a1.ntiles = nt;
        chk(launch_convnext32_bwd(a1, B, 1, st));
        chk(launch_cnx_partial_sum(pds, B, 128, nt, 0, ds, st));
        chk(launch_grn_bwd(gxn, nullptr, 0, c.grn_gamma, ds, B, 128, coef, PG(c.grn_gamma, 128), st));
        chk(launch_convnext32_bwd(a, B, 2, st));
        chk(launch_cnx_partial_sum(pds, B, 128, nt_b, 1, dal, st));
        chk(launch_cnx_partial_sum(pgb, B, 64, nt_b, 2, dgl, st));
      }
      const float *w1r = c.w1_raw, *b1p = c.b1, *alp = c.alpha;
      auto lean_w1 = [=](hipStream_t s_) {
        chk(launch_conv_wgrad_cnx(0, gh0, xn, B, Tt, gw1, p1, gb1, s_, xn16));
        auto dalpha = [=](hipStream_t s3) {
          chk(launch_cnx_dalpha(w1r, b1p, alp, gw1, gb1, scale, ds, coef, part, nt, B, dal, s3));
        };
        if (deferring())
          after_reduce.push_back(dalpha);
        else
          dalpha(s_);
      };
      float* gdw = PG(c.dw_w, 32 * 7);
      float* gdb = PG(c.dw_b, 32);
      const float* dww = c.dw_w;
      if (m->topts.frozen) {
        if (live() && !fuse_gx) chk(launch_dwconv_bwd(x, gu, dww, B, 32, Tt, 7, 3, gX, 1, nullptr, nullptr, nullptr, st, gx_src));
      } else if (side) {
        side_push(gY, [=](hipStream_t s2) {
          if (lean) {
            lean_w1(s2);
          } else if (cnx16) {
            chk(launch_conv_wgrad_cnx(1, hs, gY, B, Tt, gw2, p2, gb2, s2));
            chk(launch_conv_wgrad_cnx(0, gh0, xn, B, Tt, gw1, p1, gb1, s2));
          } else {
            chk(launch_conv1d_wgrad(f2, gY, nullptr, 1.0f, gw2, p2, gb2, nullptr, s2));
            chk(launch_conv1d_wgrad(f1, gh0, nullptr, 1.0f, gw1, p1, gb1, nullptr, s2));
          }
          chk(launch_dwconv_bwd(x, gu, dww, B, 32, Tt, 7, 3, nullptr, 0, gdw, gdb, dsc, s2, nullptr, 0, gu16));
        });
        if (live() && !fuse_gx) chk(launch_dwconv_bwd(x, gu, dww, B, 32, Tt, 7, 3, gX, 1, nullptr, nullptr, nullptr, st, gx_src));
      } else if (live()) {
        bool done = false;
        DeferScope dsc_(this);
        if (lean) {
          lean_w1(st);
        } else if (cnx16) {
          chk(launch_conv_wgrad_cnx(1, hs, gY, B, Tt, gw2, p2, gb2, st));
          chk(launch_conv_wgrad_cnx(0, gh0, xn, B, Tt, gw1, p1, gb1, st));
        } else {
          chk(launch_conv1d_wgrad(f2, gY, nullptr, 1.0f, gw2, p2, gb2, &done, st));
          chk(launch_conv1d_wgrad(f1, gh0, nullptr, 1.0f, gw1, p1, gb1, &done, st));
        }
        if (fuse_gx)
          chk(launch_dwconv_bwd(x, gu, dww, B, 32, Tt, 7, 3, nullptr, 0, gdw, gdb, dsc, st, nullptr, 0, gu16));
        else
          chk(launch_dwconv_bwd(x, gu, dww, B, 32, Tt, 7, 3, gX, 1, gdw, gdb, dsc, st));
      }
      ws.off = mark;
    });
    return y;
  }

  float* convnext(const ConvNeXt& c, const float* x, int Tt, bool branch_only = false) {
    const int C = c.C;
    if (C == 32 && c.w2a && c.w1_raw && c.w2_raw) return convnext32_fused(c, x, Tt);
    float* u = dwconv(x, c.dw_w, c.dw_b, C, Tt, 7, 3);
    float* xn = layernorm(u, C, Tt, 1e-6f, &c.norm, nullptr, nullptr);
    float* h0 = take<float>((size_t)B * 4 * C * Tt);
    conv(base(c.pw1, xn, Tt, h0));
    float* h = c.alpha ? act(ACT_SNAKE, h0, c.alpha, 4 * C, Tt)
                       : act(ACT_GELU, h0, nullptr, 4 * C, Tt);
    const int nseg = row_stats_nseg(Tt);
    double* part = take<double>((size_t)B * 4 * C * nseg * 2);
    float* scale = take<float>((size_t)B * 4 * C);
    float* gxn = take<float>((size_t)B * 4 * C);
    if (live()) {
      chk(launch_row_stats(h, B * 4 * C, Tt, part, st));
      chk(launch_grn_finalize(part, nseg, c.grn_gamma, B, 4 * C, scale, st, gxn));
    }
    const float* gamma = c.grn_gamma;
    tape.push_back([=]() {
      float* dsc = G(scale, (size_t)B * 4 * C);
      G(h, (size_t)B * 4 * C * Tt);
      float* coef = take<float>((size_t)B * 4 * C);
      if (live()) chk(launch_grn_bwd(gxn, nullptr, 0, gamma, dsc, B, 4 * C, coef, PG(gamma, 4 * C), st));
      pend_row[h] = PendRow{coef, B * 4 * C, Tt};
    });
    float* y = take<float>((size_t)B * C * Tt);
    ConvArgs b2 = base(c.pw2, h, Tt, y);
    b2.pro = PRO_SCALE;
    b2.pa = scale;
    if (!branch_only) b2.residual = x;
    conv(b2);
    return y;
  }

  static ConvArgs cat3_slice(const ConvArgs& a3, const PackedConv& w, int i, bool dgrad) {
    ConvArgs s = a3;
    s.nsrc = 1;
    s.xc[0] = 32;
    s.x[1] = s.x[2] = nullptr;
    s.xc[1] = s.xc[2] = 0;
    s.w = w;
    s.w.Cin = s.w.CinP = 32;
    s.w.Cout = s.w.CoutP = 32;
    if (dgrad) {
      s.w.wp = w.wp + 32 * i;
      s.w_row = w.CoutP;
      s.w_tap = w.CinP * w.CoutP;
    } else {
      s.w.wp = w.wp + (size_t)32 * i * w.CoutP;
      s.w_row = w.CoutP;
      s.w_tap = w.CinP * w.CoutP;
    }
    return s;
  }
  bool cat3_ok(const ConvArgs& a3) const {
    if (!m->topts.compute_bf16 || getenv("STY_NO_CAT3") || a3.nsrc != 3 || a3.w.CinP != 96 || a3.w.CoutP != 32) return false;
    for (int i = 0; i < 3; ++i)
      if (a3.xc[i] != 32 || is16(a3.x[i])) return false;
    if (a3.pro != PRO_NONE || a3.residual || a3.out_mask || a3.act != ACT_NONE || a3.shuffle != 1) return false;
    auto it = m->dgrad.find(a3.w.wp);
    if (it == m->dgrad.end()) return false;
    ConvArgs f = cat3_slice(a3, a3.w, 0, false), d = cat3_slice(a3, it->second, 0, true);
    d.pad = (a3.w.K - 1) * a3.dil - a3.pad;
    return plan_route(m, f).kernel == CONV_32P && plan_route(m, d).kernel == CONV_32P;
  }
  void conv_cat3(const ConvArgs& a0) {
    ConvArgs a3 = a0;
    a3.bf16 = m->topts.compute_bf16;
    const size_t pn = wgrad_partial_floats(a3.w, B, a3.T);
    side_need = pn > side_need ? pn : side_need;
    wg_need(pn);
    bias_pass_sizing(a3);
    for (int i = 0; i < 3 && live(); ++i) {
      ConvArgs s = cat3_slice(a3, a3.w, i, false);
      s.x[0] = a3.x[i];
      if (i) {
        s.w.bias = nullptr;
        s.residual = a3.y;
      }
      chk(launch_conv1d(s, st));
    }
    tape.push_back([this, a3]() {
      const PackedConv& w = a3.w;
      const int Tt = a3.T;
      const size_t ny = (size_t)B * 32 * Tt;
      float* gY = G(a3.y, ny);
      float* gX[3];
      int accX[3] = {1, 1, 1};
      for (int i = 0; i < 3; ++i) gX[i] = wants(a3.x[i]) ? Gw(a3.x[i], ny, accX[i]) : nullptr;
      const size_t mark = ws.off;
      conv_wgrad(a3, gY, nullptr, 1);
      const PackedConv& wd = m->dgrad.find(w.wp)->second;
      for (int i = 0; i < 3; ++i) {
        if (!gX[i] || !live()) continue;
        ConvArgs d = cat3_slice(a3, wd, i, true);
        d.x[0] = gY;
        d.w.bias = nullptr;
        d.pad = (w.K - 1) * a3.dil - a3.pad;
        d.y = gX[i];
        d.residual = accX[i] ? gX[i] : nullptr;
        chk(launch_conv1d(d, st));
      }
      ws.off = mark;
    });
  }
  bool resblock16(const ResBlock32& r, int Tt) const {
    if (!act16_on() || Tt % 8 != 0) return false;
    const int dil[3] = {1, 3, 5};
    for (int i = 0; i < 3; ++i) {
      ConvArgs c1, c2;
      c1.B = c2.B = B, c1.T = c2.T = Tt, c1.nsrc = c2.nsrc = 1, c1.w = r.c1[i], c2.w = r.c2[i];
      c1.xc[0] = c2.xc[0] = 32;
      c1.dil = dil[i], c1.pad = 5 * dil[i], c2.pad = 5;
      c1.pro = c2.pro = PRO_AFFINE_SNAKE;
      c1.xh = c1.yh = c2.xh = c2.yh = c2.rh = 1;
      if (!plan_route(m, c1).two_byte() || !plan_route(m, c2).two_byte()) return false;
    }
    return true;
  }
  float* resblock(const ResBlock32& r, float* x, int Tt, const double* part_x = nullptr) {
    const int dil[3] = {1, 3, 5};
    const int nseg_p = conv32p_stat_nseg(Tt);
    const bool h16 = resblock16(r, Tt);
    if (is16(x) && (!h16 || !part_x)) {
      set_error("training: bf16-stored resblock input without the two-byte path");
      rc = STY_ESTATE;
      return x;
    }
    for (int i = 0; i < 3; ++i) {
      float *a, *s;
      adain(x, 32, Tt, r.n1[i], a, s, part_x, nseg_p);
      float* xt = take_act((size_t)B * 32 * Tt, h16);
      ConvArgs c1 = base(r.c1[i], x, Tt, xt);
      c1.dil = dil[i];
      c1.pad = 5 * dil[i];
      c1.pro = PRO_AFFINE_SNAKE;
      c1.pa = a;
      c1.ps = s;
      c1.palpha = r.a1[i];
      double* part_t = nullptr;
      if (plan_route(m, c1).stats()) c1.stat_part = part_t = take<double>((size_t)B * 32 * nseg_p * 2);
      conv(c1);
      adain(xt, 32, Tt, r.n2[i], a, s, part_t, nseg_p);
      float* xn = take_act((size_t)B * 32 * Tt, h16 && i + 1 < 3);
      ConvArgs c2 = base(r.c2[i], xt, Tt, xn);
      c2.pro = PRO_AFFINE_SNAKE;
      c2.pa = a;
      c2.ps = s;
      c2.palpha = r.a2[i];
      c2.residual = x;
      part_x = nullptr;
      if (plan_route(m, c2).stats() && i + 1 < 3) {
        double* p = take<double>((size_t)B * 32 * nseg_p * 2);
        c2.stat_part = p;
        part_x = p;
      }
      conv(c2);
      x = xn;
    }
    return x;
  }

  float* attention(const float* q, const float* kv, int inner, int Tt) {
    float* o = take<float>((size_t)B * inner * Tt);
    AttnArgs at;
    at.q = q;
    at.k = kv;
    at.v = kv + (size_t)inner * Tt;
    at.o = o;
// ... 1566 lines not shown
```

### stylish_tts_amd/lib.py

```python
import ctypes as C
import os

os.environ.setdefault("GPU_MAX_HW_QUEUES", "2")

HERE = os.path.dirname(os.path.abspath(__file__))
LIB_PATH = os.path.join(HERE, "libstylish_hip.so")


class StyError(RuntimeError):
    pass


class VocoderIO(C.Structure):
    _fields_ = [("B", C.c_int), ("T", C.c_int)] + [
        (n, C.c_void_p) for n in ("mel", "style", "pitch", "voiced", "noise", "prior_override")
    ] + [("seed", C.c_uint64), ("audio", C.c_void_p)] + [
        (n, C.c_void_p) for n in ("tap_conformer_out", "tap_prior", "tap_har_spec", "tap_har_phase",
                                  "tap_logamp_prior", "tap_phase_prior", "tap_trunk", "tap_logamp")
    ]


class SpeechIO(C.Structure):
    _fields_ = [("B", C.c_int), ("L", C.c_int), ("T", C.c_int)] + [
        (n, C.c_void_p) for n in ("texts", "text_lengths", "alignment", "pitch", "energy", "voiced", "style",
                                  "denormal_pitch", "noise", "prior_override")
    ] + [("seed", C.c_uint64), ("audio", C.c_void_p), ("tap_text_encoding", C.c_void_p),
         ("tap_decoder_out", C.c_void_p), ("voc_taps", VocoderIO), ("style_stream", C.c_void_p)]


class TrainOpts(C.Structure):
    _fields_ = [("bn_batch_stats", C.c_int), ("sn_power_iter", C.c_int), ("f0_smooth", C.c_int),
                ("energy_smooth", C.c_int), ("bn_momentum", C.c_float), ("dropout_seed", C.c_uint),
                ("text_dropout", C.c_float), ("compute_bf16", C.c_int), ("frozen", C.c_int),
                ("block_dropout", C.c_float)]


class SpecDiscPtrs(C.Structure):
    _fields_ = [("g", C.c_void_p * 10), ("v", C.c_void_p * 10), ("bias", C.c_void_p * 10)]


class CfDiscParams(C.Structure):
    _fields_ = [("conv_w", C.c_void_p * 12), ("conv_b", C.c_void_p * 12), ("bn_w", C.c_void_p * 9), ("bn_b", C.c_void_p * 9),
                ("bn_rm", C.c_void_p * 9), ("bn_rv", C.c_void_p * 9)]


class CfDiscGrads(C.Structure):
    _fields_ = [("conv_w", C.c_void_p * 12), ("conv_b", C.c_void_p * 12), ("bn_w", C.c_void_p * 9), ("bn_b", C.c_void_p * 9)]


_P, _I, _SZP = C.c_void_p, C.c_int, C.POINTER(C.c_size_t)
SYMBOLS = {
    "sty_version": (C.c_int, []),
    "sty_last_error": (C.c_char_p, []),
    "sty_stft64_bases_host": (None, [_P]),
    "sty_model_create": (C.c_int, [C.c_char_p, C.POINTER(_P)]),
    "sty_model_destroy": (None, [_P]),
    "sty_model_bind": (C.c_int, [_P, C.c_char_p, _P, _I, C.POINTER(C.c_int64)]),
    "sty_model_finalize": (C.c_int, [_P]),
    "sty_model_num_keys": (C.c_int, [_P]),
    "sty_model_key": (C.c_char_p, [_P, _I]),
    "sty_model_prepare": (C.c_int, [_P, _P]),
    "sty_model_invalidate": (C.c_int, [_P]),
    "sty_vocoder_workspace_bytes": (C.c_int, [_P, _I, _I, _SZP]),
    "sty_vocoder_fwd": (C.c_int, [_P, C.POINTER(VocoderIO), _P, C.c_size_t, _P]),
    "sty_speech_workspace_bytes": (C.c_int, [_P, _I, _I, _I, _SZP]),
    "sty_speech_fwd": (C.c_int, [_P, C.POINTER(SpeechIO), _P, C.c_size_t, _P]),
    "sty_style_workspace_bytes": (C.c_int, [_P, _I, _I, _SZP]),
    "sty_style_fwd": (C.c_int, [_P, _I, _I, _P, _P, _P, C.c_size_t, _P]),
    "sty_mel_workspace_bytes": (C.c_int, [_I, _I, _I, _I, _SZP]),
    "sty_mel_fwd": (C.c_int, [_I, _I, _P, _I, _I, _I, C.c_float, C.c_float, _P, _P, _P, C.c_size_t, _P]),
    "sty_multispec_workspace_bytes": (C.c_int, [_I, _I, _SZP]),
    "sty_multispec_fwd": (C.c_int, [_I, _I, _P, C.POINTER(_P), C.POINTER(_P), C.POINTER(_P), _P, C.c_size_t, _P]),
    "sty_alignment_fwd": (C.c_int, [_I, _I, _I, _P, _P, _P]),
    "sty_convnext_fwd": (C.c_int, [_P, C.c_char_p, _I, _I, _I, _P, _P, _P, _P, C.c_size_t, _P]),
    "sty_resblock_fwd": (C.c_int, [_P, C.c_char_p, _I, _I, _P, _P, _P, _P, C.c_size_t, _P]),
    "sty_block_train_workspace_bytes": (C.c_int, [_P, C.c_char_p, C.c_char_p, _I, _I, _I, _SZP]),
    "sty_block_fwd_bwd": (C.c_int, [_P, C.c_char_p, C.c_char_p, _I, _I, _I, _P, _P, _P, _P, _P, _P, _P, C.c_size_t, _P]),
    "sty_attention_workspace_bytes": (C.c_int, [_I, _I, _I, _SZP]),
    "sty_attention_fwd_bwd": (C.c_int, [_I, _I, _I, _I, _P, _P, _P, _P, _P, _P, _P, _P, _P, _P, C.c_size_t, _P]),
    "sty_stft64_fwd": (C.c_int, [_I, _I, _P, _P, _P, _P]),
    "sty_istft64_fwd": (C.c_int, [_I, _I, _P, _P, _P, _P, _P]),
    "sty_source_fwd": (C.c_int, [_I, _I, _P, _P, _P, C.c_uint64, _P, _P, _P, _P, C.c_size_t, _P]),
    "sty_source_workspace_bytes": (C.c_int, [_I, _I, _SZP]),
    "sty_model_enable_training": (C.c_int, [_P]),
    "sty_model_bind_grad": (C.c_int, [_P, C.c_char_p, _P]),
    "sty_model_set_train_opts": (C.c_int, [_P, C.POINTER(TrainOpts)]),
    "sty_vocoder_train_workspace_bytes": (C.c_int, [_P, _I, _I, _SZP]),
    "sty_vocoder_fwd_train": (C.c_int, [_P, C.POINTER(VocoderIO), _P, C.c_size_t, _P]),
    "sty_vocoder_bwd": (C.c_int, [_P, _P, _P, _P, _P]),
    "sty_speech_train_workspace_bytes": (C.c_int, [_P, _I, _I, _I, _SZP]),
    "sty_speech_fwd_train": (C.c_int, [_P, C.POINTER(SpeechIO), _P, C.c_size_t, _P]),
    "sty_speech_bwd": (C.c_int, [_P, _P, _P, _P, _P]),
    "sty_speech_prepare_train": (C.c_int, [_P, _P]),
    "sty_speech_bwd_pe": (C.c_int, [_P, _P, _P, _P, _P, _P]),
    "sty_speech_d_style_ready": (C.c_int, [_P, _P]),
    "sty_speech_branch_stream": (C.c_int, [_P, C.POINTER(C.c_void_p)]),
    "sty_style_train_workspace_bytes": (C.c_int, [_P, _I, _I, _SZP]),
    "sty_style_fwd_train": (C.c_int, [_P, _I, _I, _P, _P, _P, C.c_size_t, _P]),
    "sty_style_prepare_train": (C.c_int, [_P, _P]),
    "sty_style_bwd": (C.c_int, [_P, _P, _P]),
    "sty_style_tap": (C.c_int, [_P, _I, _I, _P, C.POINTER(C.c_int), C.POINTER(C.c_int), C.POINTER(C.c_int), _P]),
    "sty_duration_workspace_bytes": (C.c_int, [_P, _I, _I, _SZP]),
    "sty_duration_fwd": (C.c_int, [_P, _I, _I, _P, _P, _P, _P, _P, C.c_size_t, _P]),
    "sty_pitch_energy_workspace_bytes": (C.c_int, [_P, _I, _I, _I, _SZP]),
    "sty_pitch_energy_fwd": (C.c_int, [_P, _I, _I, _I, _P, _P, _P, _P, _P, _P, _P, C.c_size_t, _P]),
    "sty_pitch_style_workspace_bytes": (C.c_int, [_P, _I, _I, _SZP]),
    "sty_pitch_style_fwd": (C.c_int, [_P, _I, _I, _P, _P, _P, _P, _P, C.c_size_t, _P]),
    "sty_conv1d_workspace_bytes": (C.c_int, [_I, _I, _I, _SZP]),
    "sty_conv1d_fwd": (C.c_int, [_I, _I, _I, _I, _I, _I, _P, _P, _P, _P, _P, C.c_size_t, _I, _P]),
    "sty_conv1d_fwd_ex": (C.c_int, [_I, _I, _I, _I, _I, _I, _P, _P, _P, _P, _P, _P, _I, _I, _P, _P, C.c_size_t, _I, _P]),
    "sty_conv1d_route": (C.c_int, [_I, _I, _I, _I, _I, _I, _I, _I, C.POINTER(C.c_int)]),
    "sty_conv1d_bwd_workspace_bytes": (C.c_int, [_I, _I, _I, _I, _I, _SZP]),
    "sty_conv1d_bwd": (C.c_int, [_I, _I, _I, _I, _I, _I, _P, _P, _P, _P, _P, _P, _P, C.c_size_t, _I, _P]),
    "sty_partial_sum": (C.c_int, [_I, _P, _I, _I, _I, _P, _P, _P]),
    "sty_grn_bwd_workspace_bytes": (C.c_int, [_I, _I, _I, _SZP]),
    "sty_grn_bwd": (C.c_int, [_I, _I, _I, _P, _P, _P, _I, _P, _P, _P, C.c_size_t, _P]),
    "sty_act_bwd": (C.c_int, [_I, _I, _I, _I, _P, _P, _P, _P, _P, _I, _P, _I, _P, _P]),
    "sty_adain_finalize": (C.c_int, [_I, _I, _I, _I, _P, _P, C.c_float, _P, _P, _P, _P, _P]),
    "sty_adamw_step": (C.c_int, [C.c_size_t, _P, _P, _P, _P, C.c_float, C.c_float, C.c_float, C.c_float, C.c_float,
                                 _I, C.c_float, _P]),
    "sty_adamw_step_scaled": (C.c_int, [C.c_size_t, _P, _P, _P, _P, C.c_double, _P, C.c_float, C.c_float, C.c_float,
                                        C.c_float, _I, C.c_float, _P]),
    "sty_disc_lr_track": (C.c_int, [_P, _P, C.c_double, C.c_double, C.c_double, C.c_double, C.c_double, _P]),
    "sty_model_set_grad_hook": (C.c_int, [_P, _P, _P]),
    "sty_acoustic_loss_workspace_bytes": (C.c_int, [_I, _I, _SZP]),
    "sty_acoustic_loss_target": (C.c_int, [_I, _I, _P, _P, C.c_size_t, _P]),
    "sty_acoustic_loss_fwd_bwd": (C.c_int, [_I, _I, _P, _P, C.c_float, C.c_float, _P, _P, _P, C.c_size_t, _P]),
    "sty_specdisc_workspace_bytes": (C.c_int, [_I, _I, _I, _I, _SZP]),
    "sty_specdisc_forward": (C.c_int, [_P, _I, _I, _I, _P, _P, _I, _P, C.c_size_t, _P]),
    "sty_specdisc_losses": (C.c_int, [_P, _I, _I, _I, _P, _P, C.c_float, _P, _P, C.c_float, _P, _P, _I, _P, C.c_size_t,
                                      _P]),
    "sty_prediction_to_duration": (C.c_int, [_I, _I, _I, _P, _P, _P, _P, _P]),
    "sty_duration_loss_fwd_bwd": (C.c_int, [_I, _I, _I, _P, _P, _P, _P, _P, _P, C.c_float, C.c_float, _P, _P, _P, _P,
                                            C.c_size_t, _P]),
    "sty_duration_train_workspace_bytes": (C.c_int, [_P, _I, _I, _SZP]),
    "sty_duration_fwd_train": (C.c_int, [_P, _I, _I, _P, _P, _P, _P, _P, C.c_size_t, _P]),
    "sty_duration_bwd": (C.c_int, [_P, _P, _P, _P]),
    "sty_pitch_loss_fwd_bwd": (C.c_int, [_I, _I, _P, _P, C.c_float, _I, _P, _P, _P, C.c_size_t, _P]),
    "sty_pitch_energy_train_workspace_bytes": (C.c_int, [_P, _I, _I, _I, _SZP]),
    "sty_pitch_energy_fwd_train": (C.c_int, [_P, _I, _I, _I, _P, _P, _P, _P, _P, _P, _P, C.c_size_t, _P]),
    "sty_pitch_energy_bwd": (C.c_int, [_P, _P, _P, _P, _P]),
    "sty_pitch_style_train_workspace_bytes": (C.c_int, [_P, _I, _I, _SZP]),
    "sty_pitch_style_fwd_train": (C.c_int, [_P, _I, _I, _P, _P, _P, _P, _P, C.c_size_t, _P]),
    "sty_pitchdisc_workspace_bytes": (C.c_int, [_I, _I, _I, _I, _I, _SZP]),
    "sty_pitchdisc_forward": (C.c_int, [_P, _I, _I, _I, _I, _P, _P, _P, C.c_size_t, _P]),
    "sty_pitchdisc_losses": (C.c_int, [_P, _I, _I, _I, _I, _P, _P, C.c_float, _P, _P, C.c_float, _P, _P, _P, C.c_size_t,
                                       _P]),
    "sty_cfdisc_workspace_bytes": (C.c_int, [_I, _I, _I, _SZP]),
    "sty_cfdisc_forward": (C.c_int, [_P, _I, _I, _P, _P, C.c_float, _I, _P, C.c_size_t, _P]),
    "sty_cfdisc_losses": (C.c_int, [_P, _I, _I, _P, _P, C.c_float, _P, _P, C.c_float, _P, _P, C.c_float, _I, _P,
                                    C.c_size_t, _P]),
    "sty_acoustic_gan_workspace_bytes": (C.c_int, [_I, _I, _I, _SZP]),
    "sty_acoustic_gan_loss_fwd_bwd": (C.c_int, [_I, _I, _P, _P, C.c_float, C.c_float, C.c_float, _P, C.c_float, _P, _I, _P,
                                                _P, _P, _P, C.c_size_t, _P, C.c_size_t, _I, _P]),
    "sty_comm_unique_id": (C.c_int, [_P]),
    "sty_comm_init": (C.c_int, [_P, _I, _I, _I, C.POINTER(C.c_void_p)]),
    "sty_comm_allreduce_bucket": (C.c_int, [_P, _P, C.c_size_t, _P]),
    "sty_comm_wait": (C.c_int, [_P, _P]),
    "sty_comm_set_stream": (C.c_int, [_P, _P]),
    "sty_comm_stats": (C.c_int, [_P, C.POINTER(C.c_uint64), C.POINTER(C.c_uint64), C.POINTER(C.c_double)]),
    "sty_comm_destroy": (C.c_int, [_P]),
    "sty_pack_accumulate": (C.c_int, [_I, _I, _I, _P, _P, _P, _P, _P]),
    "sty_pack_finalize": (C.c_int, [_I, _I, _P, _P, _P, _P, _P, _P]),
    "sty_aligner_workspace_bytes": (C.c_int, [_P, _I, _I, _SZP]),
    "sty_aligner_fwd": (C.c_int, [_P, _I, _I, _P, _P, _P, _P, C.c_size_t, _P]),
    "sty_forced_align_workspace_bytes": (C.c_int, [_I, _I, _I, _SZP]),
    "sty_forced_align": (C.c_int, [_I, _I, _I, _I, _P, _P, _P, _P, _I, _P, _P, _P, _P, C.c_size_t, _P]),
    "sty_rmvpe_resample_kernel_host": (None, [_P]),
    "sty_rmvpe_mel_basis_host": (None, [_P]),
    "sty_rmvpe_mel_workspace_bytes": (C.c_int, [_I, _I, _SZP]),
    "sty_rmvpe_mel_fwd": (C.c_int, [_I, _I, _P, _P, _P, C.c_size_t, _P]),
    "sty_rmvpe_workspace_bytes": (C.c_int, [_P, _I, _I, _SZP]),
    "sty_rmvpe_fwd": (C.c_int, [_P, _I, _I, _P, _P, _P, C.c_size_t, _P]),
    "sty_rmvpe_decode": (C.c_int, [_I, _I, _P, C.c_float, _P, _P]),
    "sty_aligner_train_workspace_bytes": (C.c_int, [_P, _I, _I, _SZP]),
    "sty_aligner_fwd_train": (C.c_int, [_P, _I, _I, _P, _P, C.c_float, C.c_uint, _P, _P, C.c_size_t, _P]),
    "sty_aligner_bwd": (C.c_int, [_P, _P, _P]),
    "sty_ctc_loss_workspace_bytes": (C.c_int, [_I, _I, _I, _I, _SZP]),
    "sty_ctc_loss_fwd_bwd": (C.c_int, [_I, _I, _I, _I, _P, _P, C.c_float, _P, _P, _P, _I, C.c_float, _P, _P, _P, _P, _P,
                                       C.c_size_t, _P]),
    "sty_prof_enable": (C.c_int, [_I]),
    "sty_prof_only": (C.c_int, [C.c_char_p]),
    "sty_set_single_stream": (C.c_int, [_I]),
    "sty_prof_report": (C.c_int, [_P, _I]),
}


class ProfRow(C.Structure):
    _fields_ = [("name", C.c_char * 48), ("inst", C.c_char * 144), ("launches", C.c_uint64), ("ms", C.c_double),
                ("flops", C.c_double), ("bytes", C.c_double)]


def prof_report(cap=64, by_inst=False):
    cap = max(cap, 4096)
    rows = (ProfRow * cap)()
    n = LIB.sty_prof_report(C.cast(rows, C.c_void_p), cap)
    if n < 0:
        check(n)
    raw = [dict(name=r.name.decode(), inst=r.inst.decode(), launches=int(r.launches), ms=r.ms, flops=r.flops, bytes=r.bytes)
           for r in rows[:min(n, cap)]]
    return raw if by_inst else group_families(raw)


def group_families(raw):
    fam = {}
    for r in raw:
        f = fam.setdefault(r["name"], dict(name=r["name"], launches=0, ms=0.0, flops=0.0, bytes=0.0, insts={}))
        for k in ("launches", "ms", "flops", "bytes"):
            f[k] += r[k]
        if r["inst"]:
            f["insts"][r["inst"]] = f["insts"].get(r["inst"], 0) + r["launches"]
    return list(fam.values())

GRAD_HOOK = C.CFUNCTYPE(None, C.c_void_p, C.c_int)

LIB = None


def load():
    global LIB
    if LIB is not None:
        return LIB
    if not os.path.exists(LIB_PATH):
        raise StyError(f"{LIB_PATH} not found: build it with `python __graft_entry__.py` (hipcc, gfx950). "
                       "There is no CPU fallback.")
    lib = C.CDLL(LIB_PATH)
    for name, (res, args) in SYMBOLS.items():
        fn = getattr(lib, name)
        fn.restype = res
        fn.argtypes = args
    LIB = lib
    return lib


def check(rc):
    if rc != 0:
        raise StyError(f"libstylish_hip: status {rc}: {LIB.sty_last_error().decode()}")


def ptr(t):
    return None if t is None else C.c_void_p(t.data_ptr())
```

Baseline: 404,700 frames/s.

## Fuse GELU/snake activation and GRN stats into convk1 epilogue; fuse scale-backward

Adds output stages to the pointwise (K=1) conv kernel. In the forward pass it writes both the pre-activation and the GELU/snake-activated output and accumulates per-row sum and sum-of-squares partials, so the separate activation and row-stats kernels of the ConvNeXt GRN path are skipped. In the backward pass it folds the PRO_SCALE backward (applying the scale, accumulating the residual, and the dscale partial reductions) into the conv epilogue, so the temporary U buffer and the pro_bwd kernel are no longer needed. This costs a more complex epilogue with extra register pressure and per-tile double-precision DPP reductions. It also adds C API entry points for testing the fused against the unfused paths.

```diff
diff --git a/include/stylish_hip.h b/include/stylish_hip.h
--- a/include/stylish_hip.h
+++ b/include/stylish_hip.h
@@ -206,9 +206,17 @@
                       const float *in_mask, const float *residual, const float *out_mask, int out_mask_post, int relu,
                       float *y, void *workspace, size_t ws_bytes, int compute_bf16, void *stream);
 enum { STY_ROUTE_IN_MASK = 1, STY_ROUTE_RESIDUAL = 2, STY_ROUTE_OUT_MASK = 4, STY_ROUTE_RELU = 8, STY_ROUTE_TWO_BYTE_X = 16,
-       STY_ROUTE_STATS = 32, STY_ROUTE_Y16 = 64, STY_ROUTE_X16 = 128 };
+       STY_ROUTE_STATS = 32, STY_ROUTE_Y16 = 64, STY_ROUTE_X16 = 128,
+       STY_ROUTE_ACT_TWIN = 256, STY_ROUTE_SCALE_BWD = 512 };
 enum { STY_CONV_STEM2D = 0, STY_CONV_32P, STY_CONV_SC, STY_CONV_K1, STY_CONV_Q, STY_CONV_P16, STY_CONV_TILED };
 int sty_conv1d_route(int B, int Cin, int Cout, int K, int dil, int T, int compute_bf16, int flags, int *kernel);
+int sty_conv1d_glue_workspace_bytes(int B, int Cin, int Cout, int T, size_t *bytes);
+int sty_conv1d_fwd_act_stats(int B, int Cin, int Cout, int T, const float *x, const float *w, const float *bias, int kind,
+                             const float *alpha, int fused, float *y, float *y_act, double *sums, void *workspace,
+                             size_t ws_bytes, int compute_bf16, void *stream);
+int sty_conv1d_scale_bwd(int B, int Cin, int Cout, int T, const float *gy, const float *wt, const float *h,
+                         const float *scale, const float *gh_old, int fused, float *gh, float *dscale, void *workspace,
+                         size_t ws_bytes, int compute_bf16, void *stream);
 int sty_conv1d_bwd_workspace_bytes(int B, int Cin, int Cout, int K, int T, size_t *bytes);
 int sty_conv1d_bwd(int B, int Cin, int Cout, int K, int dil, int T, const float *x, const float *w, const float *gy,
                    float *dw, float *dbias, float *dx, void *workspace, size_t ws_bytes, int compute_bf16,
diff --git a/stylish_tts_amd/csrc/api.hip b/stylish_tts_amd/csrc/api.hip
--- a/stylish_tts_amd/csrc/api.hip
+++ b/stylish_tts_amd/csrc/api.hip
@@ -2842,9 +2842,110 @@
   if (flags & STY_ROUTE_STATS) a.stat_part = dummy_d;
   if (flags & STY_ROUTE_Y16) a.y16 = dummy_h;
   if (flags & STY_ROUTE_X16) a.x16 = dummy_h;
+  if (flags & STY_ROUTE_ACT_TWIN) {
+    a.act = ACT_GELU;
+    a.y_act = dummy_f;
+  }
+  if (flags & STY_ROUTE_SCALE_BWD) {
+    a.sb_h = a.sb_scale = dummy_f;
+    a.sb_part = dummy_d;
+  }
   const ConvRoute r = conv1d_route(a);
   *kernel = r.refusal == CONV_OK ? (int)r.kernel : -1;
   return STY_OK;
+}
+static int glue_nseg_max(int T) { return std::max(convk1_stat_nseg(T), row_stats_nseg(T)); }
+int sty_conv1d_glue_workspace_bytes(int B, int Cin, int Cout, int T, size_t* bytes) {
+  size_t need = 0;
+  if (!bytes || B <= 0 || T <= 0 || sty_conv1d_workspace_bytes(Cout, Cin, 1, &need)) {
+    set_error("sty_conv1d_glue_workspace_bytes: bad argument");
+    return STY_EINVAL;
+  }
+  *bytes = need + 512 + (size_t)B * Cout * glue_nseg_max(T) * 2 * sizeof(double) + (size_t)B * Cout * T * sizeof(float);
+  return STY_OK;
+}
+static int glue_unit_conv(int B, int Cin, int Cout, int T, const float* x, const float* w, const float* bias, void* workspace,
+                          size_t ws_bytes, int compute_bf16, hipStream_t st, ConvArgs& a, double** part, float** tmp) {
+  size_t need = 0, all = 0;
+  int rc = sty_conv1d_glue_workspace_bytes(B, Cin, Cout, T, &all);
+  if (rc) return rc;
+  if ((rc = sty_conv1d_workspace_bytes(Cout, Cin, 1, &need))) return rc;
+  if (!x || !w || !workspace || ws_bytes < all) {
+    set_error("conv1d glue entry: bad argument or workspace too small");
+    return STY_EINVAL;
+  }
+  PackedConv pc = unit_conv_dims(Cin, Cout, 1);
+  float* wp = reinterpret_cast<float*>(align_up(reinterpret_cast<size_t>(workspace), 256));
+  float* bp = wp + (size_t)pc.CinP * pc.CoutP;
+  STY_HIP(hipMemsetAsync(wp, 0, ((size_t)pc.CinP * pc.CoutP + pc.CoutP) * sizeof(float), st));
+  if ((rc = launch_pack_conv(w, nullptr, nullptr, bias, Cout, Cin, 1, wp, bp, pc.CinP, pc.CoutP, st))) return rc;
+  pc.wp = wp;
+  pc.bias = bias ? bp : nullptr;
+  *part = reinterpret_cast<double*>(align_up(reinterpret_cast<size_t>(static_cast<char*>(workspace) + need), 256));
+  *tmp = reinterpret_cast<float*>(*part + (size_t)B * Cout * glue_nseg_max(T) * 2);
+  a.x[0] = x;
+  a.xc[0] = Cin;
+  a.nsrc = 1;
+  a.B = B;
+  a.T = T;
+  a.w = pc;
+  a.bf16 = compute_bf16 != 0;
+  return STY_OK;
+}
+int sty_conv1d_fwd_act_stats(int B, int Cin, int Cout, int T, const float* x, const float* w, const float* bias, int kind,
+                             const float* alpha, int fused, float* y, float* y_act, double* sums, void* workspace,
+                             size_t ws_bytes, int compute_bf16, void* stream) {
+  if (!y || !y_act || !sums || !(kind == ACT_GELU || (kind == ACT_SNAKE && alpha))) {
+    set_error("sty_conv1d_fwd_act_stats: bad argument");
+    return STY_EINVAL;
+  }
+  hipStream_t st = S(stream);
+  ConvArgs a;
+  double* part = nullptr;
+  float* tmp = nullptr;
+  int rc = glue_unit_conv(B, Cin, Cout, T, x, w, bias, workspace, ws_bytes, compute_bf16, st, a, &part, &tmp);
+  if (rc) return rc;
+  a.y = y;
+  if (fused) {
+    a.act = kind;
+    a.act_alpha = alpha;
+    a.y_act = y_act;
+    a.stat_part = part;
+    if ((rc = launch_conv1d(a, st))) return rc;
+    return launch_stat_part_sum(part, B * Cout, convk1_stat_nseg(T), sums, st);
+  }
+  if ((rc = launch_conv1d(a, st))) return rc;
+  if ((rc = launch_act_fwd(kind, y, alpha, B, Cout, T, y_act, st))) return rc;
+  if ((rc = launch_row_stats(y_act, B * Cout, T, part, st))) return rc;
+  return launch_stat_part_sum(part, B * Cout, row_stats_nseg(T), sums, st);
+}
+int sty_conv1d_scale_bwd(int B, int Cin, int Cout, int T, const float* gy, const float* wt, const float* h, const float* scale,
+                         const float* gh_old, int fused, float* gh, float* dscale, void* workspace, size_t ws_bytes,
+                         int compute_bf16, void* stream) {
+  if (!h || !scale || !gh || !dscale) {
+    set_error("sty_conv1d_scale_bwd: bad argument");
+    return STY_EINVAL;
+  }
+  hipStream_t st = S(stream);
+  ConvArgs d;
+  double* part = nullptr;
+  float* U = nullptr;
+  int rc = glue_unit_conv(B, Cin, Cout, T, gy, wt, nullptr, workspace, ws_bytes, compute_bf16, st, d, &part, &U);
+  if (rc) return rc;
+  if (gh_old) STY_HIP(hipMemcpyAsync(gh, gh_old, (size_t)B * Cout * T * sizeof(float), hipMemcpyDeviceToDevice, st));
+  if (fused) {
+    d.y = gh;
+    d.residual = gh_old ? gh : nullptr;
+    d.sb_h = h;
+    d.sb_scale = scale;
+    d.sb_part = part;
+    if ((rc = launch_conv1d(d, st))) return rc;
+    return launch_convk1_sb_sum(part, B * Cout, T, dscale, st);
+  }
+  d.y = U;
+  if ((rc = launch_conv1d(d, st))) return rc;
+  return launch_pro_bwd(PRO_SCALE | (d.bf16 ? 0x100 : 0), U, Cout, 0, h, B, Cout, T, scale, nullptr, Cout, 0, nullptr, nullptr, gh,
+                        gh_old ? 1 : 0, dscale, nullptr, nullptr, st);
 }
 int sty_conv1d_bwd_workspace_bytes(int B, int Cin, int Cout, int K, int T, size_t* bytes) {
   if (!bytes || B <= 0 || Cin <= 0 || Cout <= 0 || K <= 0 || T <= 0) {
diff --git a/stylish_tts_amd/csrc/bwd.hip b/stylish_tts_amd/csrc/bwd.hip
--- a/stylish_tts_amd/csrc/bwd.hip
+++ b/stylish_tts_amd/csrc/bwd.hip
@@ -768,6 +768,9 @@
 }
 int launch_act_fwd(int kind, const float* x, const float* alpha, int B, int C, int T, float* y, hipStream_t st) {
   const size_t n4 = (size_t)B * C * (T / 4);
+  char detail[40];
+  snprintf(detail, sizeof(detail), "k%d C%d T%d", kind, C, T);
+  ProfScope prof("act_fwd_kernel", 0.0, 8.0 * B * C * T, st, detail);
   if (kind != ACT_GLU && T % 4 == 0 && n4 < ((size_t)1 << 31) && ((((size_t)x | (size_t)y) & 15) == 0)) {
     hipLaunchKernelGGL(act_fwd4_kernel, dim3((unsigned)((n4 + 255) / 256)), dim3(256), 0, st, kind, x, alpha, (unsigned)C,
                        (unsigned)(T / 4), (unsigned)n4, y);
diff --git a/stylish_tts_amd/csrc/conv1d.hip b/stylish_tts_amd/csrc/conv1d.hip
--- a/stylish_tts_amd/csrc/conv1d.hip
+++ b/stylish_tts_amd/csrc/conv1d.hip
@@ -389,6 +389,7 @@
 bool conv32p_eligible(const ConvArgs& a);
 bool convsc_eligible(const ConvArgs& a);
 bool convk1_eligible(const ConvArgs& a);
+int convk1_stages(const ConvArgs& a);
 bool convp16_eligible(const ConvArgs& a);
 bool convq_eligible(const ConvArgs& a);
 int launch_stem2d(const ConvArgs& a, hipStream_t st);
@@ -406,7 +407,7 @@
     r.kernel = CONV_32P;
   else if (a.xh || a.yh || a.rh)
     r.refusal = CONV_NO_TWO_BYTE;
-  else if (a.stat_part)
+  else if (a.stat_part && !(a.y_act && convk1_eligible(a) && (convk1_stages(a) & 1)))
     r.refusal = CONV_NO_STATS;
   else if (convsc_eligible(a))
     r.kernel = CONV_SC;
@@ -419,6 +420,9 @@
                !(a.up_g && (!a.up_gate16 || !a.up_mask || a.up_H <= 0 || a.up_H * a.flatW != a.T)) &&
                (long)a.w.Cout * a.T < (1l << 26);
   if (a.up_g && !r.up_stage) r.refusal = CONV_NO_UP_STAGE;
+  if (r.kernel == CONV_K1 && r.refusal == CONV_OK) r.k1_stages = convk1_stages(a);
+  if ((a.y_act && !r.act_twin()) || ((a.sb_h || a.sb_scale || a.sb_part) && !(r.scale_bwd() && a.sb_h && a.sb_scale)))
+    r.refusal = CONV_NO_CNX_STAGE;
   return r;
 }
 
@@ -449,7 +453,11 @@
     return STY_EINVAL;
   }
   if (r.refusal == CONV_NO_STATS) {
-    set_error("conv1d: output statistics requested for a conv the persistent 32-channel kernel does not take");
+    set_error("conv1d: output statistics requested for a conv neither the persistent 32-channel kernel nor convk1_kernel takes");
+    return STY_EINVAL;
+  }
+  if (r.refusal == CONV_NO_CNX_STAGE) {
+    set_error("conv1d: activation twin or scale-backward operands on a conv that does not run on convk1_kernel's output stages");
     return STY_EINVAL;
   }
   int rc = STY_OK;
diff --git a/stylish_tts_amd/csrc/convk1.hip b/stylish_tts_amd/csrc/convk1.hip
--- a/stylish_tts_amd/csrc/convk1.hip
+++ b/stylish_tts_amd/csrc/convk1.hip
@@ -18,9 +18,26 @@
   return __builtin_bit_cast(unsigned, r);
 }
 
-template <int PRO, int RELU>
-__global__ __launch_bounds__(256, 2) void convk1_kernel(ConvArgs a, int tiles_per_row, int ncot, int ntiles, int per_xcd) {
-  extern __shared__ __attribute__((aligned(16))) __bf16 g_lds[];
+__host__ __device__ constexpr int g_nseg(int T) { return T / 64 + 2; }
+
+template <int CTRL>
+__device__ __forceinline__ double g_dpp(double v) {
+  const int2 x = __builtin_bit_cast(int2, v);
+  int2 y;
+  y.x = __builtin_amdgcn_update_dpp(0, x.x, CTRL, 0xf, 0xf, false);
+  y.y = __builtin_amdgcn_update_dpp(0, x.y, CTRL, 0xf, 0xf, false);
+  return __builtin_bit_cast(double, y);
+}
+__device__ __forceinline__ double g_sum16(double v) {
+  v += g_dpp<0x128>(v);
+  v += g_dpp<0x124>(v);
+  v += g_dpp<0x4E>(v);
+  v += g_dpp<0xB1>(v);
+  return v;
+}
+
+template <int PRO, int RELU, int STAGE>
+__device__ __forceinline__ void convk1_body(const ConvArgs& a, int ncot, int ntiles, int per_xcd, __bf16* g_lds) {
   const int tid = threadIdx.x, lane = tid & 63, wave = __builtin_amdgcn_readfirstlane(tid >> 6), l31 = lane & 31, hi = lane >> 5;
   const int wm = wave >> 1, wn = wave & 1;
   const int tile = ((int)blockIdx.x & 7) * per_xcd + ((int)blockIdx.x >> 3);
@@ -155,18 +172,106 @@
 #pragma unroll
     for (int e = 0; e < 4; ++e) om[e] = a.out_mask[(size_t)nq + e];
   }
+  const int s0 = n0 + wn * 64, nseg = g_nseg(T);
+  const bool sp_on = STAGE != 0 && s0 < NT && (STAGE == 2 ? a.sb_part != nullptr : a.stat_part != nullptr);
+  const int bA = sp_on ? s0 / T : 0, endA = (bA + 1) * T;
+  const bool two = sp_on && endA < s0 + 64 && endA < NT;
+  const int slotA = (s0 >> 6) - ((bA * T) >> 6);
+  const bool lastA = ((endA - 1) >> 6) == (s0 >> 6);
+  const bool inA = bq == bA;
+  const __amdgpu_buffer_rsrc_t rya = __builtin_amdgcn_make_buffer_rsrc(STAGE == 1 ? a.y_act : a.y, 0, ybytes, 0x00020000);
+  const __amdgpu_buffer_rsrc_t rsh = __builtin_amdgcn_make_buffer_rsrc(
+      const_cast<float*>(STAGE == 2 ? a.sb_h : a.y), 0, STAGE == 2 ? ybytes : 0, 0x00020000);
 #pragma unroll
   for (int m = 0; m < 2; ++m) {
+    const int cobase = cot * 128 + (wm * 2 + m) * 32;
+    float4 hv[8], gv[8];
+    if constexpr (STAGE == 2) {
+#pragma unroll
+      for (int i = 0; i < 8; ++i) {
+        const int co = cobase + rq + 4 * i;
+        const int yo = co < Cout && qin ? ((bq * Cout + co) * T + tq) * 4 : 0x7FFFFF00;
+        hv[i] = __builtin_bit_cast(float4, __builtin_amdgcn_raw_buffer_load_b128(rsh, yo, 0, 0));
+        gv[i] = __builtin_bit_cast(float4, __builtin_amdgcn_raw_buffer_load_b128(rres, yo, 0, 0));
+      }
+    }
 #pragma unroll
     for (int n = 0; n < 2; ++n)
 #pragma unroll
       for (int r = 0; r < 16; ++r) stg[((r & 3) + 8 * (r >> 2) + 4 * hi) * 68 + n * 32 + l31] = acc[m][n][r];
     __syncthreads();
-    const int cobase = cot * 128 + (wm * 2 + m) * 32;
 #pragma unroll
     for (int i = 0; i < 8; ++i) {
       const int row = rq + 4 * i, co = cobase + row;
-      if (co < Cout && qin) {
+      if constexpr (STAGE != 0) {
+        double s1 = 0.0, s2 = 0.0;
+        if (co < Cout && qin) {
+          const int yo = ((bq * Cout + co) * T + tq) * 4;
+          const float4 sv = *reinterpret_cast<const float4*>(stg + row * 68 + 4 * c4);
+          const float bi = a.w.bias ? a.w.bias[co] : 0.f;
+          float v[4] = {sv.x + bi, sv.y + bi, sv.z + bi, sv.w + bi};
+          if constexpr (STAGE == 1) {
+            float al = 1.f, ral = 1.f;
+            if (RELU == 2) {
+              al = a.act_alpha[co];
+              ral = 1.0f / al;
+            }
+            float ac[4];
+#pragma unroll
+            for (int e = 0; e < 4; ++e) {
+              ac[e] = RELU == 2 ? sty_snake(v[e], al, ral) : 0.5f * v[e] * (1.0f + erff(v[e] * 0.70710678118654752f));
+              const double d = (double)ac[e];
+              s1 += d;
+              s2 += d * d;
+            }
+            __builtin_amdgcn_raw_buffer_store_b128(
+                  __builtin_bit_cast(__attribute__((__vector_size__(4 * sizeof(unsigned)))) unsigned,
+                                     make_float4(v[0], v[1], v[2], v[3])), ry, yo, 0, 0);
+            __builtin_amdgcn_raw_buffer_store_b128(
+                __builtin_bit_cast(__attribute__((__vector_size__(4 * sizeof(unsigned)))) unsigned,
+                                   make_float4(ac[0], ac[1], ac[2], ac[3])), rya, yo, 0, 0);
+          } else {
+            const float sc = a.sb_scale[(size_t)bq * Cout + co];
+            const float hh[4] = {hv[i].x, hv[i].y, hv[i].z, hv[i].w}, gg[4] = {gv[i].x, gv[i].y, gv[i].z, gv[i].w};
+#pragma unroll
+            for (int e = 0; e < 4; ++e) {
+              const float u = v[e] * a.out_scale;
+              const float p = u * hh[e];
+              s1 += (double)p;
+              v[e] = gg[e] + u * sc;
+            }
+            __builtin_amdgcn_raw_buffer_store_b128(
+                __builtin_bit_cast(__attribute__((__vector_size__(4 * sizeof(unsigned)))) unsigned,
+                                   make_float4(v[0], v[1], v[2], v[3])), ry, yo, 0, 0);
+          }
+        }
+        if (sp_on) {
+          double a1 = s1, a2 = s2, b1 = 0.0, b2 = 0.0;
+          if (two) {
+            b1 = inA ? 0.0 : s1;
+            b2 = inA ? 0.0 : s2;
+            a1 = inA ? s1 : 0.0;
+            a2 = inA ? s2 : 0.0;
+            b1 = g_sum16(b1);
+            if (STAGE == 1) b2 = g_sum16(b2);
+          }
+          a1 = g_sum16(a1);
+          if (STAGE == 1) a2 = g_sum16(a2);
+          if (c4 == 0 && co < Cout) {
+            constexpr int W = STAGE == 1 ? 2 : 1;
+            double* pp = (STAGE == 1 ? a.stat_part : a.sb_part) + (((size_t)bA * Cout + co) * nseg + slotA) * W;
+            pp[0] = a1;
+            if (STAGE == 1) pp[1] = a2;
+            if (lastA)
+              for (int k = W; k < (nseg - slotA) * W; ++k) pp[k] = 0.0;
+            if (two) {
+              double* pb = (STAGE == 1 ? a.stat_part : a.sb_part) + ((size_t)(bA + 1) * Cout + co) * nseg * W;
+              pb[0] = b1;
+              if (STAGE == 1) pb[1] = b2;
+            }
+          }
+        }
+      } else if (co < Cout && qin) {
         const int yo = ((bq * Cout + co) * T + tq) * 4;
         const float4 sv = *reinterpret_cast<const float4*>(stg + row * 68 + 4 * c4);
         const float bi = a.w.bias ? a.w.bias[co] : 0.f;
@@ -198,6 +303,60 @@
   }
 }
 
+template <int PRO, int RELU>
+__global__ __launch_bounds__(256, 2) void convk1_kernel(ConvArgs a, int tiles_per_row, int ncot, int ntiles, int per_xcd) {
+  extern __shared__ __attribute__((aligned(16))) __bf16 g_lds[];
+  convk1_body<PRO, RELU, 0>(a, ncot, ntiles, per_xcd, g_lds);
+}
+template <int RELU, int STAGE>
+__global__ __launch_bounds__(256, 2) void convk1_glue_kernel(ConvArgs a, int ncot, int ntiles, int per_xcd) {
+  extern __shared__ __attribute__((aligned(16))) __bf16 g_lds[];
+  convk1_body<PRO_NONE, RELU, STAGE>(a, ncot, ntiles, per_xcd, g_lds);
+}
+
+__global__ __launch_bounds__(256) void convk1_sb_sum_kernel(const double* __restrict__ part, int nseg, int rows,
+                                                            float* __restrict__ dpa) {
+  const int i = blockIdx.x * 4 + (threadIdx.x >> 6), lane = threadIdx.x & 63;
+  if (i >= rows) return;
+  double s = 0.0;
+  for (int k = lane; k < nseg; k += 64) s += part[(size_t)i * nseg + k];
+  for (int o = 32; o > 0; o >>= 1) s += __shfl_xor(s, o);
+  if (lane == 0) dpa[i] = (float)s;
+}
+
+__global__ __launch_bounds__(256) void stat_part_sum_kernel(const double* __restrict__ part, int nseg, int rows,
+                                                            double* __restrict__ out) {
+  const int i = blockIdx.x * 4 + (threadIdx.x >> 6), lane = threadIdx.x & 63;
+  if (i >= rows) return;
+  double s = 0.0, q = 0.0;
+  for (int k = lane; k < nseg; k += 64) {
+    s += part[((size_t)i * nseg + k) * 2];
+    q += part[((size_t)i * nseg + k) * 2 + 1];
+  }
+  for (int o = 32; o > 0; o >>= 1) {
+    s += __shfl_xor(s, o);
+    q += __shfl_xor(q, o);
+  }
+  if (lane == 0) {
+    out[(size_t)i * 2] = s;
+    out[(size_t)i * 2 + 1] = q;
+  }
+}
+int launch_stat_part_sum(const double* part, int rows, int nseg, double* out, hipStream_t st) {
+  hipLaunchKernelGGL(stat_part_sum_kernel, dim3(cdiv(rows, 4)), dim3(256), 0, st, part, nseg, rows, out);
+  STY_LAUNCH_CHECK();
+  return STY_OK;
+}
+
+int convk1_stat_nseg(int T) { return g_nseg(T); }
+
+int launch_convk1_sb_sum(const double* part, int rows, int T, float* dpa, hipStream_t st) {
+  ProfScope prof("convk1_sb_sum_kernel", 0.0, 8.0 * rows * convk1_stat_nseg(T), st);
+  hipLaunchKernelGGL(convk1_sb_sum_kernel, dim3(cdiv(rows, 4)), dim3(256), 0, st, part, convk1_stat_nseg(T), rows, dpa);
+  STY_LAUNCH_CHECK();
+  return STY_OK;
+}
+
 int convp16_frags(const ConvArgs& a, hipStream_t st, const void** out);
 
 bool convk1_eligible(const ConvArgs& a) {
@@ -209,6 +368,14 @@
   if ((size_t)a.B * a.w.CinP * a.T * 4 >= (size_t)1 << 31 || (size_t)a.B * a.w.CoutP * a.T * 4 >= (size_t)1 << 31) return false;
   const char* mt = getenv("STY_CONVK1_MIN_TILES");
   return (long)cdiv(a.B * a.T, 128) * cdiv(a.w.CoutP, 128) >= (mt ? atoi(mt) : 24);
+}
+
+int convk1_stages(const ConvArgs& a) {
+  if (getenv("STY_NO_CNX_GLUE") || a.T < 64 || a.pro != PRO_NONE || a.out_mask || a.y16) return 0;
+  int s = 0;
+  if (a.act == ACT_NONE) s |= 4;
+  if ((a.act == ACT_SNAKE || a.act == ACT_GELU) && !a.residual && a.out_scale == 1.f) s |= 3;
+  return s;
 }
 
 template <int PRO>
@@ -234,8 +401,18 @@
   char detail[40];
   snprintf(detail, sizeof(detail), "ci%d co%d k1 T%d", a.w.Cin, a.w.Cout, a.T);
   ProfScope prof("convk1_kernel<true>", 2.0 * a.w.Cin * outs,
-                 4.0 * ((double)a.B * a.w.Cin * a.T + outs * (a.residual ? 2.0 : 1.0)) + 2.0 * a.w.Cout * a.w.Cin, st, detail);
+                 4.0 * ((double)a.B * a.w.Cin * a.T + outs * ((a.residual ? 2.0 : 1.0) + (a.y_act ? 1.0 : 0.0) + (a.sb_h ? 1.0 : 0.0))) + 2.0 * a.w.Cout * a.w.Cin, st, detail);
   const dim3 grid(per * 8);
+  if (a.sb_h || a.y_act) {
+    if (a.sb_h)
+      hipLaunchKernelGGL((convk1_glue_kernel<0, 2>), grid, dim3(256), lds, st, a, ncot, ntiles, per);
+    else if (a.act == ACT_SNAKE)
+      hipLaunchKernelGGL((convk1_glue_kernel<2, 1>), grid, dim3(256), lds, st, a, ncot, ntiles, per);
+    else
+      hipLaunchKernelGGL((convk1_glue_kernel<3, 1>), grid, dim3(256), lds, st, a, ncot, ntiles, per);
+    STY_LAUNCH_CHECK();
+    return STY_OK;
+  }
   switch (a.pro) {
     case PRO_MASK: g_launch<PRO_MASK>(a, grid, lds, tpr, ncot, ntiles, per, st); break;
     case PRO_SCALE: g_launch<PRO_SCALE>(a, grid, lds, tpr, ncot, ntiles, per, st); break;
diff --git a/stylish_tts_amd/csrc/norms.hip b/stylish_tts_amd/csrc/norms.hip
--- a/stylish_tts_amd/csrc/norms.hip
+++ b/stylish_tts_amd/csrc/norms.hip
@@ -63,6 +63,9 @@
 
 int launch_row_stats(const float* x, int rows, int T, double* part, hipStream_t st) {
   const int nseg = row_stats_nseg(T);
+  char detail[40];
+  snprintf(detail, sizeof(detail), "rows%d T%d", rows, T);
+  ProfScope prof("row_stats_kernel", 0.0, 4.0 * rows * T, st, detail);
   hipLaunchKernelGGL(row_stats_kernel, dim3(nseg, rows), dim3(256), 0, st, x, T, nseg, part);
   STY_LAUNCH_CHECK();
   return STY_OK;
@@ -109,7 +112,7 @@
 
 __global__ __launch_bounds__(1024) void grn_finalize_kernel(const double* __restrict__ part, int nseg, int G,
                                                             const float* __restrict__ gamma, int C4,
-                                                            float* __restrict__ scale, float* __restrict__ gx_out) {
+                                                            float* __restrict__ scale, float* __restrict__ gx_out, int flat) {
   __shared__ float red[16];
   __shared__ float gxs[1024];
   const int b = blockIdx.x, wave = threadIdx.x >> 6, lane = threadIdx.x & 63;
@@ -130,6 +133,10 @@
       loc += gx;
     }
   }
+  if (flat) {
+    __syncthreads();
+    loc = (int)threadIdx.x < C4 ? gxs[threadIdx.x] : 0.f;
+  }
   for (int o = 32; o > 0; o >>= 1) loc += __shfl_xor(loc, o);
   if (lane == 0) red[wave] = loc;
   __syncthreads();
@@ -141,14 +148,14 @@
 }
 
 int launch_grn_finalize(const double* part, int nseg, const float* gamma, int B, int C4, float* scale,
-                        hipStream_t st, float* gx) {
+                        hipStream_t st, float* gx, bool flat_mean) {
   if (C4 > 1024) {
     set_error("grn_finalize: 4C = %d > 1024", C4);
     return STY_EINVAL;
   }
   int G = 1;
   while (G < 64 && G < nseg) G <<= 1;
-  hipLaunchKernelGGL(grn_finalize_kernel, dim3(B), dim3(1024), 0, st, part, nseg, G, gamma, C4, scale, gx);
+  hipLaunchKernelGGL(grn_finalize_kernel, dim3(B), dim3(1024), 0, st, part, nseg, G, gamma, C4, scale, gx, flat_mean ? 1 : 0);
   STY_LAUNCH_CHECK();
   return STY_OK;
 }
diff --git a/stylish_tts_amd/csrc/sty_common.h b/stylish_tts_amd/csrc/sty_common.h
--- a/stylish_tts_amd/csrc/sty_common.h
+++ b/stylish_tts_amd/csrc/sty_common.h
@@ -172,6 +172,10 @@
   float* y = nullptr;
   float* y_split = nullptr;
   double* stat_part = nullptr;
+  float* y_act = nullptr;
+  const float* sb_h = nullptr;
+  const float* sb_scale = nullptr;
+  double* sb_part = nullptr;
   const __bf16* x16 = nullptr;
   const __bf16* g16 = nullptr;
   __bf16* y16 = nullptr;
@@ -196,19 +200,25 @@
   CONV_P16,
   CONV_TILED,
 };
-enum ConvRefusal : int { CONV_OK = 0, CONV_NO_UP_STAGE, CONV_NO_TWO_BYTE, CONV_NO_STATS };
+enum ConvRefusal : int { CONV_OK = 0, CONV_NO_UP_STAGE, CONV_NO_TWO_BYTE, CONV_NO_STATS, CONV_NO_CNX_STAGE };
 struct ConvRoute {
   ConvKernel kernel = CONV_TILED;
   ConvRefusal refusal = CONV_OK;
   bool x16_only = false;
   bool up_stage = false;
   bool writes_y16() const { return kernel == CONV_STEM2D || kernel == CONV_Q || kernel == CONV_P16; }
-  bool stats() const { return kernel == CONV_32P; }
+  int k1_stages = 0;
+  bool stats() const { return kernel == CONV_32P || (k1_stages & 1); }
+  bool act_twin() const { return (k1_stages & 2) != 0; }
+  bool scale_bwd() const { return (k1_stages & 4) != 0; }
   bool two_byte() const { return kernel == CONV_32P; }
 };
 ConvRoute conv1d_route(const ConvArgs& a);
 int launch_conv1d(const ConvArgs& a, hipStream_t st);
 int conv32p_stat_nseg(int T);
+int convk1_stat_nseg(int T);
+int launch_convk1_sb_sum(const double* part, int rows, int T, float* dpa, hipStream_t st);
+int launch_stat_part_sum(const double* part, int rows, int nseg, double* out, hipStream_t st);
 inline int num_cus() {
   static int n = 0;
   if (!n) {
@@ -276,7 +286,7 @@
 int launch_adain_finalize(const double* part, int nseg, const float* gb, int B, int C, int T, float eps, float* a,
                           float* s, hipStream_t st, float* mean = nullptr, float* rstd = nullptr);
 int launch_grn_finalize(const double* part, int nseg, const float* gamma, int B, int C4, float* scale, hipStream_t st,
-                        float* gx = nullptr);
+                        float* gx = nullptr, bool flat_mean = false);
 int launch_chan_layernorm(const float* x, float* y, int B, int C, int T, float eps, int ada, const float* w,
                           const float* bvec, const float* gb, int relu, const float* out_mask, hipStream_t st);
 int launch_embedding(const int64_t* tokens, const float* emb, int B, int L, int H, int ntok, float scale, float* y,
diff --git a/stylish_tts_amd/csrc/train.hip b/stylish_tts_amd/csrc/train.hip
--- a/stylish_tts_amd/csrc/train.hip
+++ b/stylish_tts_amd/csrc/train.hip
@@ -479,6 +479,12 @@
     bias_pass_sizing(a);
     if (live()) chk(launch_conv1d(a, st));
     ConvArgs f = a;
+    if (f.y_act) {
+      f.y_act = nullptr;
+      f.stat_part = nullptr;
+      f.act = ACT_NONE;
+      f.act_alpha = nullptr;
+    }
     tape.push_back([this, f]() { conv_bwd(f); });
   }
   void bias_pass_sizing(const ConvArgs& a) {
@@ -594,16 +600,6 @@
         return;
       }
       const bool u16 = f.xh && f.nsrc == 1 && act16_on();
-      float* U = take_act((size_t)B * w.Cin * Tt, u16);
-      struct UGuard {
-        Trainer* t;
-        float* U;
-        size_t mark;
-        ~UGuard() {
-          t->half_.erase(U);
-          t->release(mark);
-        }
-      } u_guard{this, U, mark};
       ConvArgs d;
       d.x[0] = gY;
       d.xc[0] = w.Cout;
@@ -620,9 +616,36 @@
         d.pro = PRO_MASK;
         d.mask = gmask;
       }
-      d.y = U;
       d.yh = u16;
       d.xh = is16(gY);
+      if (f.nsrc == 1 && f.pro == PRO_SCALE && dpa && gX[0] != gY && !u16 && !f.xh && !d.xh && !is16(gX[0])) {
+        ConvArgs s = d;
+        s.y = gX[0];
+        s.residual = accX[0] ? gX[0] : nullptr;
+        if (conv1d_route(s).scale_bwd()) {
+          double* sp = take<double>((size_t)B * w.Cin * convk1_stat_nseg(Tt));
+          s.sb_h = f.x[0];
+          s.sb_scale = f.pa;
+          s.sb_part = sp;
+          if (live()) {
+            chk(launch_conv1d(s, st));
+            chk(launch_convk1_sb_sum(sp, B * w.Cin, Tt, dpa, st));
+          }
+          release(mark);
+          return;
+        }
+      }
+      float* U = take_act((size_t)B * w.Cin * Tt, u16);
+      struct UGuard {
+        Trainer* t;
+        float* U;
+        size_t mark;
+        ~UGuard() {
+          t->half_.erase(U);
+          t->release(mark);
+        }
+      } u_guard{this, U, mark};
+      d.y = U;
       if (f.nsrc == 1 && (f.pro == PRO_NONE || f.pro == PRO_MASK) && gX[0] != gY) {
         d.y = gX[0];
         d.yh = is16(gX[0]);
@@ -671,6 +694,10 @@
   float* act(int kind, const float* x, const float* alpha, int C, int Tt) {
     float* y = take<float>((size_t)B * C * Tt);
     if (live()) chk(launch_act_fwd(kind, x, alpha, B, C, Tt, y, st));
+    act_tape(kind, x, alpha, C, Tt, y);
+    return y;
+  }
+  void act_tape(int kind, const float* x, const float* alpha, int C, int Tt, float* y) {
     tape.push_back([=]() {
       const int Cin = kind == ACT_GLU ? 2 * C : C;
       float* gY = G(y, (size_t)B * C * Tt, false, false, kind != ACT_GLU);
@@ -680,7 +707,6 @@
       float* dal = kind == ACT_SNAKE ? PG(alpha, C) : nullptr;
       if (live()) chk(launch_act_bwd(kind, x, gY, alpha, B, C, Tt, gX, acc, dal, st, row ? y : nullptr, row));
     });
-    return y;
   }
 
   unsigned drop_site = 0;
@@ -1038,16 +1064,34 @@
     float* u = dwconv(x, c.dw_w, c.dw_b, C, Tt, 7, 3);
     float* xn = layernorm(u, C, Tt, 1e-6f, &c.norm, nullptr, nullptr);
     float* h0 = take<float>((size_t)B * 4 * C * Tt);
-    conv(base(c.pw1, xn, Tt, h0));
-    float* h = c.alpha ? act(ACT_SNAKE, h0, c.alpha, 4 * C, Tt)
-                       : act(ACT_GELU, h0, nullptr, 4 * C, Tt);
-    const int nseg = row_stats_nseg(Tt);
-    double* part = take<double>((size_t)B * 4 * C * nseg * 2);
+    const int kind = c.alpha ? ACT_SNAKE : ACT_GELU;
+    ConvArgs a1 = base(c.pw1, xn, Tt, h0);
+    ConvArgs probe = a1;
+    probe.act = kind;
+    probe.act_alpha = c.alpha;
+    const ConvRoute r1 = plan_route(m, probe);
+    const bool glue = r1.act_twin() && r1.stats();
+    const int nseg = glue ? convk1_stat_nseg(Tt) : row_stats_nseg(Tt);
+    float* h;
+    double* part;
+    if (glue) {
+      h = take<float>((size_t)B * 4 * C * Tt);
+      part = take<double>((size_t)B * 4 * C * nseg * 2);
+      a1 = probe;
+      a1.y_act = h;
+      a1.stat_part = part;
+      conv(a1);
+      act_tape(kind, h0, c.alpha, 4 * C, Tt, h);
+    } else {
+      conv(a1);
+      h = act(kind, h0, c.alpha, 4 * C, Tt);
+      part = take<double>((size_t)B * 4 * C * nseg * 2);
+    }
     float* scale = take<float>((size_t)B * 4 * C);
     float* gxn = take<float>((size_t)B * 4 * C);
     if (live()) {
-      chk(launch_row_stats(h, B * 4 * C, Tt, part, st));
-      chk(launch_grn_finalize(part, nseg, c.grn_gamma, B, 4 * C, scale, st, gxn));
+      if (!glue) chk(launch_row_stats(h, B * 4 * C, Tt, part, st));
+      chk(launch_grn_finalize(part, nseg, c.grn_gamma, B, 4 * C, scale, st, gxn, glue));
     }
     const float* gamma = c.grn_gamma;
     tape.push_back([=]() {
diff --git a/stylish_tts_amd/lib.py b/stylish_tts_amd/lib.py
--- a/stylish_tts_amd/lib.py
+++ b/stylish_tts_amd/lib.py
@@ -110,6 +110,9 @@
     "sty_conv1d_fwd": (C.c_int, [_I, _I, _I, _I, _I, _I, _P, _P, _P, _P, _P, C.c_size_t, _I, _P]),
     "sty_conv1d_fwd_ex": (C.c_int, [_I, _I, _I, _I, _I, _I, _P, _P, _P, _P, _P, _P, _I, _I, _P, _P, C.c_size_t, _I, _P]),
     "sty_conv1d_route": (C.c_int, [_I, _I, _I, _I, _I, _I, _I, _I, C.POINTER(C.c_int)]),
+    "sty_conv1d_glue_workspace_bytes": (C.c_int, [_I, _I, _I, _I, _SZP]),
+    "sty_conv1d_fwd_act_stats": (C.c_int, [_I, _I, _I, _I, _P, _P, _P, _I, _P, _I, _P, _P, _P, _P, C.c_size_t, _I, _P]),
+    "sty_conv1d_scale_bwd": (C.c_int, [_I, _I, _I, _I, _P, _P, _P, _P, _P, _I, _P, _P, _P, C.c_size_t, _I, _P]),
     "sty_conv1d_bwd_workspace_bytes": (C.c_int, [_I, _I, _I, _I, _I, _SZP]),
     "sty_conv1d_bwd": (C.c_int, [_I, _I, _I, _I, _I, _I, _P, _P, _P, _P, _P, _P, _P, C.c_size_t, _I, _P]),
     "sty_partial_sum": (C.c_int, [_I, _P, _I, _I, _I, _P, _P, _P]),
```

Result: no change. 408,100 frames/s, median of 6 (+0.9%).
